# arturxe2/T-DEED

Hardware: AMD Instinct MI355X
Metric: clips/sec (L=100, 224^2, bf16) forward, per-frame logits (higher is better)
Workload: dtype bf16; 1 GPU; rny002_b8: rny002_gsf + ed_sgp_mixer n_layers=2 ks=7, L=100, 224x224, batch 8/GPU, inference forward, random-init weights; clips_per_gpu=8, parallelism=dp1 (clip-sharded, no collective), hip_graph=True, batches_in_flight=3, sub_batches_per_batch=1, dist_backend=none, dist_ranks=1, self_launched=False

## Files before the change

### include/tdeed_hip.h

```cpp
#ifndef TDEED_HIP_H
#define TDEED_HIP_H
#include <stdint.h>
#ifdef __cplusplus
extern "C" {
#endif

enum { TDEED_F32 = 0, TDEED_BF16 = 1 };
enum { TDEED_ACT_NONE = 0, TDEED_ACT_RELU = 1, TDEED_ACT_GELU = 2 };
enum { TDEED_OK = 0, TDEED_ERR_ARG = -1, TDEED_ERR_LAUNCH = -2, TDEED_ERR_RUNTIME = -3 };

const char* tdeed_last_error(void);
int tdeed_abi_version(void);
int tdeed_device_info(int dev, char* name64, int* n_cu, int* is_gfx950);

int tdeed_stem_fwd(const void* frames , int frames_f32,
                   int N, int H, int W, int crop_top, int crop_left,
                   int crop_h, int crop_w, int flip ,
                   const unsigned char* flip_mask ,
                   const float* w ,
                   const float* scale , const float* shift , void* out,
                   int relu , int dtype, void* stream);

int tdeed_stem_mfma_parts(int crop_h, int crop_w);
int tdeed_stem_mfma_fwd(const void* frames, int frames_f32, int N, int H, int W, int crop_top, int crop_left, int crop_h,
                        int crop_w, int flip, const unsigned char* flip_mask, const void* wfrag, void* z, float* colpart,
                        void* stream);
int tdeed_stem_mfma_eval_fwd(const void* frames, int frames_f32, int N, int H, int W, int crop_top, int crop_left, int crop_h,
                             int crop_w, int flip, const unsigned char* flip_mask, const void* wfrag, const float* scale,
                             const float* shift, void* out, void* stream);

int tdeed_s1_front_parts(int crop_h, int crop_w, int C1);
int tdeed_s1_front_fwd(const uint8_t* frames, int N, int H, int W, int crop_top, int crop_left, int crop_h,
                       int crop_w, int flip, const void* stem_wf, const float* stem_sc, const float* stem_sh,
                       int C1, const void* w1f, const float* sc1, const float* sh1, const void* wdf,
                       const float* scd, const float* shd, const void* w2f, const float* sc2,
                       const float* sh2, void* y2, void* shortcut, float* pooled, void* stream);

int tdeed_gemm_fwd(const void* A, long lda, const void* A0, long lda0, int k0,
                   const float* a_scale, int a_scale_rows, int M, int K, int N, const void* W,
                   long ldw, const float* scale, const float* shift, const void* R, long ldr,
                   int act, void* C, long ldc, int gather_stride, int gather_hi, int gather_wi,
                   int gather_ho, int gather_wo, float* colpart, void* C2, long ldc2, int n2, int c2_pre, int dtype,
                   void* stream);

int tdeed_gemm_ws_fits(int K, int N, int dtype);
int tdeed_gemm_ws_fwd(const void* A, long lda, const void* A0, long lda0, int k0,
                      const float* a_scale, int a_scale_rows, int M, int K, int N, const void* Wfrag,
                      const float* scale, const float* shift, const void* R, long ldr, int act,
                      void* C, long ldc, int gather_stride, int gather_hi, int gather_wi,
                      int gather_ho, int gather_wo, void* C2, long ldc2, int n2, int dtype, void* stream);

int tdeed_gemm_ws_sc_fits(int K, int Ks, int N, int dtype);
int tdeed_gemm_ws_sc_fwd(const void* A, long lda, const void* A0, long lda0, int k0, const float* a_scale,
                         int a_scale_rows, int M, int K, int N, const void* Wfrag, const float* scale,
                         const float* shift, const void* As, long ldas, int Ks, const void* Wsfrag,
                         const float* sscale, const float* sshift, int act, void* C, long ldc, int gather_stride,
                         int gather_hi, int gather_wi, int gather_ho, int gather_wo, void* C2, long ldc2, int n2,
                         int dtype, void* stream);

int tdeed_gconv3x3_parts(int Hi, int Wi, int C, int stride, int dtype);
int tdeed_gconv3x3_mfma_fits(int Hi, int Wi, int C, int stride);
int tdeed_gconv3x3_fwd(const void* x, int N, int Hi, int Wi, int C, int gw, int stride,
                       const float* w, const void* wfrag, const float* scale, const float* shift,
                       void* y, float* pooled, float* pooled_sq, const float* in_a, const float* in_b,
                       int relu , int dtype,
                       void* stream);

int tdeed_gemm_splitk_splits(int K);
int tdeed_gemm_splitk_partials(const void* A, long lda, int M, int K, int N, const void* W, long ldw, float* workspace,
                               void* stream);
int tdeed_gemm_splitk_fwd(const void* A, long lda, int M, int K, int N, const void* W, long ldw, const float* scale,
                          const float* shift, const void* R, long ldr, int act, void* C, long ldc,
                          float* workspace, void* stream);

int tdeed_se_gate_mfma_fits(int C, int R);
int tdeed_se_gate_mfma_fwd(const float* pooled, int n_parts, float inv_cnt, int N, int C, int R, const void* w1f,
                           const float* b1, const void* w2f, const float* b2, float* gate, void* stream);

int tdeed_gemm_rs_fits(int M, int K, int N);
int tdeed_gemm_rs_fwd(const void* A, long lda, const void* A0, long lda0, int k0, const float* a_scale, int a_scale_rows,
                      int M, int K, int N, const void* Wfrag, const float* scale, const float* shift, const void* R, long ldr,
                      int act, void* C, long ldc, void* C2, long ldc2, int n2, void* stream);

int tdeed_gemm_rs_grid(int M);
int tdeed_gemm_rs_stats_fwd(const void* A, long lda, const void* A0, long lda0, int k0, int M, int K, int N, const void* Wfrag,
                            void* C, long ldc, float* colpart, void* stream);

int tdeed_c1_gconv_set_debug(void* buf);
int tdeed_c1_gconv_fits(int Hi, int Wi, int Cin, int C, int stride);
int tdeed_c1_gconv_slab_tiles(int Hi, int Wi, int C, int stride);
int tdeed_c1_gconv_fwd(const void* x, const void* G, int Fp, int N, int Hi, int Wi, int Cin, int C, int gw, int stride,
                       const void* w1f, const float* s1, const float* h1, const void* wfrag, const float* scale,
                       const float* shift, void* y, float* pooled, void* stream);
int tdeed_c1_gconv_set_form(int form);
int tdeed_c1_gconv_slab_loop_fits(int Hi, int Wi, int Cin, int C, int stride);
int tdeed_c1_gconv_workgroups(int N, int Hi, int Wi, int Cin, int C, int stride);

int tdeed_c1_gconv_c3in_fits(int Hi, int Wi, int Cp, int C);
int tdeed_c1_gconv_c3in_fwd(const void* y2p, const void* scp, const float* gate, const void* w3f, const float* s3,
                            const float* h3, void* xs2, int N, int Hi, int Wi, int Cp, int C, int gw, const void* w1f,
                            const float* s1, const float* h1, const void* wfrag, const float* scale, const float* shift,
                            void* y, float* pooled, void* stream);
int tdeed_c1_gconv_c3in_set_walk(int walk);
int tdeed_c1_gconv_c3in_walk(int Hi, int Wi, int Cp, int C);
int tdeed_c1_gconv_c3in_workgroups(int N, int Hi, int Wi, int Cp, int C);

int tdeed_bneck_fits(int h, int w, int C, int R);
int tdeed_bneck_set_debug(void* buf);
int tdeed_bneck_fwd(const void* x, const void* G, int Fp, int N, int h, int w, int C, const void* w1f, const float* s1,
                    const float* h1, const void* w2f, const float* s2, const float* h2, const void* se_w1f,
                    const float* se_b1, const void* se_w2f, const float* se_b2, int R, const void* w3f, const float* s3,
                    const float* h3, void* out, void* out2, int n2,
                    int w2_tap_major ,
                    void* stream);
int tdeed_bneck_qtail_fits(int h, int w, int C, int F);
int tdeed_bneck_gs_fwd(const void* x, const void* gx, int ldx, const float* gate, const float* ysum, const float* xsum,
                       const float* cw1, const float* cb1, const float* cw2, const float* cb2, int T, int F, int Fp, int N,
                       int h, int w, int C, const void* w1f, const float* s1, const float* h1, const void* w2f,
                       const float* s2, const float* h2, const void* se_w1f, const float* se_b1, const void* se_w2f,
                       const float* se_b2, int R, const void* w3f, const float* s3, const float* h3, void* out, void* out2,
                       int n2, int w2_tap_major, const void* q_wqf, const float* q_bn, int q_F, float* Q, void* stream);


int tdeed_se_gate_fwd(const float* pooled, int n_parts, float inv_cnt, int N, int C, int R,
                      const float* w1t, const float* b1, const float* w2t, const float* b2,
                      float* gate, void* stream);

int tdeed_se_gate_bf16_fwd(const float* pooled, int n_parts, float inv_cnt, int N, int C, int R,
                           const void* w1p, const float* b1, const void* w2p, const float* b2,
                           float* gate, void* stream);

int tdeed_gsf_gate_fwd(const void* x, int B, int T, int h, int w, int C, int F,
                       const float* bn_scale, const float* bn_shift,
                       const float* wq ,
                       const void* wqf ,
                       const float* b3d ,
                       float* Q , float* gate, float* ysum, float* xsum,
                       int dtype, void* stream);
int tdeed_gsf_gate_sums_fwd(const void* x, int B, int T, int h, int w, int C, int F, const float* b3d, const float* Q,
                            float* gate, float* ysum, float* xsum, void* stream);
int tdeed_gsf_weight_fwd(const float* ysum, const float* xsum, int B, int T, int F, int hw,
                         const float* cw1 , const float* cb1, const float* cw2,
                         const float* cb2, float* fw , void* stream);
int tdeed_gsf_apply_fwd(const void* x, const float* gate, const float* fw , int B,
                        int T, int h, int w, int C, int F, int Fp, void* out, int dtype,
                        void* stream);

int tdeed_gsf_apply_fused_fwd(const void* x, const float* gate, const float* ysum, const float* xsum,
                              const float* cw1, const float* cb1, const float* cw2, const float* cb2, int B,
                              int T, int h, int w, int C, int F, int Fp, void* out, int dtype, void* stream);
int tdeed_gsf_blend_src_fwd(const void* x, const float* gate, const float* ysum, const float* xsum,
                            const float* cw1, const float* cb1, const float* cw2, const float* cb2, int B,
                            int T, int h, int w, int C, int F, int Fp, void* out, int dtype, void* stream);

int tdeed_avgpool_posenc_fwd(const void* x, int B, int T, int hw, int C, const float* temp_enc,
                             void* feat, float* rowstat, int dtype, int dtype_out , void* stream);

int tdeed_layernorm_fwd(const void* x, long ldx, int rows, int C, const float* w, const float* b,
                        float eps, void* y, long ldy, int dtype, void* stream);
int tdeed_sgp_branch_fwd(const void* o, const void* x, int B, int T, int C, int ks, int up,
                         const float* dw, const float* db, void* y, int dtype, void* stream);
int tdeed_mixer_branch_fwd(const void* xn, int B, int T_hi, int T_lo, int C, int ks, int up,
                           const float* dw1, const float* db1, const float* dw2,
                           const float* db2, void* cat, int dtype, void* stream);
int tdeed_sgp_front_set_debug(void* buf);
int tdeed_sgp_front_fwd(const void* x, int B, int T, int C, int ks, int up, const float* ln_w, const float* ln_b, float eps,
                        const float* dw, const float* db, void* y, float* chsum, const float* rowstat, int rowstat_parts,
                        void* y16 ,
                        int dtype, void* stream);
int tdeed_mixer_front_fwd(const void* z, const void* xlo, int B, int T_hi, int T_lo, int C, int ks, int up,
                          const float* ln1_w, const float* ln1_b, const float* ln2_w, const float* ln2_b, float eps,
                          const float* dw1, const float* db1, const float* dw2, const float* db2, void* cat,
                          const float* rowstat_z, int rowstat_z_parts, const float* rowstat_x, int rowstat_x_parts,
                          int dtype, int dtype_cat, void* stream);
int tdeed_groupnorm_fwd(const void* x, int B, int T, int C, int G, const float* w, const float* b,
                        float eps, void* y, int dtype, void* stream);
int tdeed_maxpool_fwd(const void* x, int B, int T_in, int T_out, int C, void* y, int dtype,
                      void* stream);
int tdeed_maxpool_rowstat_fwd(const void* x, int B, int T_in, int T_out, int C, void* y, float* rowstat, float eps, int dtype,
                              void* stream);

int tdeed_heads_fwd(const void* x, int rows, int C, const float* w, const float* b, int n_out,
                    float* out, int dtype, void* stream);

int tdeed_loss_fwd(const float* logits, int rows, int ld, int K1, const int64_t* hard,
                   const float* soft, const float* cls_w, int displ_col, const float* labelD,
                   float* out, void* stream);

int tdeed_loss_bwd(const float* head_out, int rows, int ld, int K1, const int64_t* hard, const float* soft,
                   const float* cls_w, int displ_col, const float* labelD, float grad_scale, float* dhead,
                   void* stream);
int tdeed_loss2(const float* head_out, int B, int T, int ld, int K1a, int K1b, const int64_t* dataset, const int64_t* hard,
                const float* soft, const float* cls_w, int displ_col, const float* labelD, float grad_scale, float* out,
                float* dhead, void* stream);
long tdeed_heads_bwd_workspace(int rows, int C, int n_out);
int tdeed_heads_bwd(const float* dout, const void* x, int rows, int C, const float* w, int n_out, void* dx,
                    float* dw, float* db, void* workspace, int dtype, void* stream);
int tdeed_adamw_step(float* param, const float* grad, float* exp_avg, float* exp_avg_sq, long n, float lr,
                     float beta1, float beta2, float eps, float weight_decay, int step, float grad_scale,
                     void* stream);

long tdeed_grad_guard_ws_bytes(long n);
int tdeed_grad_guard(const float* grad, long n, int skip_nonfinite, void* guard, void* ws, void* stream);
int tdeed_adamw_step_guarded(float* param, const float* grad, float* exp_avg, float* exp_avg_sq, long n, float lr,
                             float beta1, float beta2, float eps, float weight_decay, int step, float grad_scale,
                             const void* guard, int skip_nonfinite, float max_grad_norm, void* stream);

int tdeed_adamw_step_groups(float* param, const float* grad, float* exp_avg, float* exp_avg_sq, long n, float lr,
                            float beta1, float beta2, float eps, float weight_decay, int step, float grad_scale,
                            const void* guard, int skip_nonfinite, float max_grad_norm, const void* runs, int nruns,
                            void* stream);

int tdeed_process_prediction(const float* head_out, int B, int T, int ld, int K1, int displ_col,
                             float* scores, int64_t* cls, void* stream);

int tdeed_cast_f32_to_bf16(const float* src, void* dst, long n, void* stream);
int tdeed_multi_cast_transpose(const void* tab, int n, long tiles, int dtype, void* stream);
int tdeed_gather_cast(const float* src, const int* idx, long n, void* out, int dtype, void* stream);
int tdeed_fill_u8_hash(uint8_t* dst, long n, uint64_t seed, void* stream);

int tdeed_clip_gather_u8(const uint8_t* video, int L, long frame_bytes, const int* starts, int B, int T,
                         uint8_t* clips_out, void* stream);

int tdeed_clip_gather_seg_u8(const uint8_t* video, int L_total, long frame_bytes, const int* starts, const int* clip_base,
                             const int* clip_len_v, int B, int T, uint8_t* clips_out, void* stream);
int tdeed_clip_gather_ring_u8(const uint8_t* ring, int ring_frames, int L_total, long frame_bytes, const int* starts,
                              const int* clip_base, const int* clip_len_v, int B, int T, uint8_t* clips_out, void* stream);
int tdeed_rows_gather(const void* maps, int rows, long row_bytes, int L, int pad_row, const int* starts, int B, int T, void* out,
                      void* stream);
int tdeed_rows_gather_seg(const void* maps, int rows, long row_bytes, int L_total, int pad_row, const int* starts,
                          const int* clip_base, const int* clip_len_v, int B, int T, void* out, void* stream);
int tdeed_stitch_scores_seg(const float* clip_scores, int V, int n, int T, int K1, const int* starts, const int* seg_off,
                            const int* clip_off, int nv, int count_all, int L_total, float* track_sum, int* support,
                            float* mean_out, void* stream);
int tdeed_frame_events_seg(const float* mean, const int* seg_off, int nv, int L_total, int max_len, int K1, float hr_threshold,
                           int* pred, unsigned char* pred_u8, float* pred_score, int* first_frame, int* count, void* stream);
int tdeed_frame_stats_seg(const float* mean, const unsigned char* labels, int L_total, int K1, long* stats, void* stream);
long tdeed_nms_track_seg_workspace(int L_total, int max_len, int K1);
int tdeed_nms_track_seg_threads(int max_len);
int tdeed_nms_track_seg(const float* mean, const int* seg_off, int nv, int L_total, int max_len, int K1, float hr_threshold,
                        double threshold, int soft, const int* windows, int n_windows, const int* first_frame, void* workspace,
                        unsigned char* emitted, double* kept_score, int* st_frame, unsigned char* st_class_u8, double* st_score,
                        int* st_count, int* out_frame, unsigned char* out_class_u8, double* out_score, int* event_off, int* rounds,
                        void* stream);

int tdeed_ap_lds_frames(void);
int tdeed_ap_max_tolerances(void);
int tdeed_ap_max_truth(int n_tol);
int tdeed_ap_match_seg(const float* mean, const unsigned char* emitted, const double* kept_score, const int* seg_off, int nv,
// ... 218 lines not shown
```

### t-deed_amd/_lib.py

```python
import ctypes
import os
from ctypes import c_int, c_long, c_float, c_double, c_void_p, c_char_p, c_uint64, POINTER

import torch

CSRC = os.path.join(os.path.dirname(os.path.abspath(__file__)), "csrc")
LIB_PATH = os.path.join(CSRC, "libtdeed_hip.so")

F32, BF16 = 0, 1
ACT_NONE, ACT_RELU, ACT_GELU = 0, 1, 2


class HipLibraryMissing(RuntimeError):
    pass


class HipCallError(RuntimeError):
    pass


P = c_void_p
_SIGS = {
    "tdeed_abi_version": ([], c_int),
    "tdeed_device_info": ([c_int, c_char_p, POINTER(c_int), POINTER(c_int)], c_int),
    "tdeed_stem_fwd": ([P, c_int, c_int, c_int, c_int, c_int, c_int, c_int, c_int, c_int, P, P, P, P, P, c_int, c_int, P], c_int),
    "tdeed_augment_scratch_floats": ([c_int], c_long),
    "tdeed_augment_clips": ([P, c_int, c_int, c_int, c_int, c_int, c_int, c_int, c_int, c_int, P, P, P, P, P], c_int),
    "tdeed_mix_frames": ([P, P, P, c_int, c_long, P, P], c_int),
    "tdeed_avgpool_posenc_bwd": ([P, c_int, c_int, c_int, c_int, P, P, c_int, P], c_int),
    "tdeed_stem_mfma_parts": ([c_int, c_int], c_int),
    "tdeed_stem_mfma_fwd": ([P, c_int, c_int, c_int, c_int, c_int, c_int, c_int, c_int, c_int, P, P, P, P, P], c_int),
    "tdeed_stem_mfma_eval_fwd": ([P, c_int, c_int, c_int, c_int, c_int, c_int, c_int, c_int, c_int, P, P, P, P, P, P], c_int),
    "tdeed_stem_wgrad": ([P, c_int, c_int, c_int, c_int, c_int, c_int, c_int, c_int, c_int, P, P, P, P, c_int, P], c_int),
    "tdeed_stem_wgrad_bn_fits": ([c_int, c_int, c_int, c_int], c_int),
    "tdeed_stem_wgrad_bn": ([P, c_int, c_int, c_int, c_int, c_int, c_int, c_int, c_int, c_int, P, P, P, P, P, P, P, P, P, P], c_int),
    "tdeed_s1_front_parts": ([c_int, c_int, c_int], c_int),
    "tdeed_s1_front_fwd": ([P, c_int, c_int, c_int, c_int, c_int, c_int, c_int, c_int, P, P, P, c_int, P, P, P, P, P, P,
                            P, P, P, P, P, P, P], c_int),
    "tdeed_gemm_fwd": ([P, c_long, P, c_long, c_int, P, c_int, c_int, c_int, c_int, P, c_long, P, P, P, c_long,
                        c_int, P, c_long, c_int, c_int, c_int, c_int, c_int, P, P, c_long, c_int, c_int, c_int, P], c_int),
    "tdeed_gemm_ws_fits": ([c_int, c_int, c_int], c_int),
    "tdeed_gemm_ws_fwd": ([P, c_long, P, c_long, c_int, P, c_int, c_int, c_int, c_int, P, P, P, P, c_long,
                           c_int, P, c_long, c_int, c_int, c_int, c_int, c_int, P, c_long, c_int, c_int, P], c_int),
    "tdeed_gemm_ws_sc_fits": ([c_int, c_int, c_int, c_int], c_int),
    "tdeed_gemm_ws_sc_fwd": ([P, c_long, P, c_long, c_int, P, c_int, c_int, c_int, c_int, P, P, P, P, c_long, c_int, P, P, P,
                              c_int, P, c_long, c_int, c_int, c_int, c_int, c_int, P, c_long, c_int, c_int, P], c_int),
    "tdeed_gconv3x3_parts": ([c_int, c_int, c_int, c_int, c_int], c_int),
    "tdeed_gconv3x3_mfma_fits": ([c_int, c_int, c_int, c_int], c_int),
    "tdeed_gconv3x3_fwd": ([P, c_int, c_int, c_int, c_int, c_int, c_int, P, P, P, P, P, P, P, P, P, c_int, c_int, P], c_int),
    "tdeed_gemm_splitk_splits": ([c_int], c_int),
    "tdeed_gemm_splitk_fwd": ([P, c_long, c_int, c_int, c_int, P, c_long, P, P, P, c_long, c_int, P, c_long, P, P], c_int),
    "tdeed_se_gate_mfma_fits": ([c_int, c_int], c_int),
    "tdeed_se_gate_mfma_fwd": ([P, c_int, c_float, c_int, c_int, c_int, P, P, P, P, P, P], c_int),
    "tdeed_gemm_rs_fits": ([c_int, c_int, c_int], c_int),
    "tdeed_gemm_rs_grid": ([c_int], c_int),
    "tdeed_gemm_rs_stats_fwd": ([P, c_long, P, c_long, c_int, c_int, c_int, c_int, P, P, c_long, P, P], c_int),
    "tdeed_gemm_rs_fwd": ([P, c_long, P, c_long, c_int, P, c_int, c_int, c_int, c_int, P, P, P, P, c_long, c_int, P, c_long, P,
                           c_long, c_int, P], c_int),
    "tdeed_c1_gconv_set_debug": ([P], c_int),
    "tdeed_c1_gconv_fits": ([c_int, c_int, c_int, c_int, c_int], c_int),
    "tdeed_c1_gconv_slab_tiles": ([c_int, c_int, c_int, c_int], c_int),
    "tdeed_c1_gconv_fwd": ([P, P, c_int, c_int, c_int, c_int, c_int, c_int, c_int, c_int, P, P, P, P, P, P, P, P,
                            P], c_int),
    "tdeed_c1_gconv_set_form": ([c_int], c_int),
    "tdeed_c1_gconv_slab_loop_fits": ([c_int, c_int, c_int, c_int, c_int], c_int),
    "tdeed_c1_gconv_workgroups": ([c_int, c_int, c_int, c_int, c_int, c_int], c_int),
    "tdeed_c1_gconv_c3in_fits": ([c_int, c_int, c_int, c_int], c_int),
    "tdeed_c1_gconv_c3in_fwd": ([P, P, P, P, P, P, P, c_int, c_int, c_int, c_int, c_int, c_int, P, P, P, P, P, P, P, P,
                                 P], c_int),
    "tdeed_c1_gconv_c3in_set_walk": ([c_int], c_int),
    "tdeed_c1_gconv_c3in_walk": ([c_int, c_int, c_int, c_int], c_int),
    "tdeed_c1_gconv_c3in_workgroups": ([c_int, c_int, c_int, c_int, c_int], c_int),
    "tdeed_bneck_fits": ([c_int, c_int, c_int, c_int], c_int),
    "tdeed_bneck_set_debug": ([P], c_int),
    "tdeed_bneck_fwd": ([P, P, c_int, c_int, c_int, c_int, c_int, P, P, P, P, P, P, P, P, P, P, c_int, P, P, P, P, P, c_int,
                         c_int, P], c_int),
    "tdeed_bneck_gs_fwd": ([P, P, c_int, P, P, P, P, P, P, P, c_int, c_int, c_int, c_int, c_int, c_int, c_int, P, P, P, P, P, P, P,
                            P, P, P, c_int, P, P, P, P, P, c_int, c_int, P, P, c_int, P, P], c_int),
    "tdeed_bneck_qtail_fits": ([c_int, c_int, c_int, c_int], c_int),
    "tdeed_gsf_gate_sums_fwd": ([P, c_int, c_int, c_int, c_int, c_int, c_int, P, P, P, P, P, P], c_int),
    "tdeed_bn_slabs": ([c_long], c_int),
    "tdeed_bn_train_stats": ([P, c_long, c_int, P, P, c_float, c_float, P, P, P, P, P, P, P, c_int, P], c_int),
    "tdeed_bn_apply": ([P, c_long, c_int, P, P, P, c_int, P, c_int, P], c_int),
    "tdeed_bn_apply_slice": ([P, c_long, c_int, P, P, P, P, P, c_int, P, P, c_int, c_int, c_int, P], c_int),
    "tdeed_bn_apply2": ([P, c_long, c_int, P, P, P, P, P, c_int, P, c_int, P], c_int),
    "tdeed_bn_train_bwd": ([P, P, P, c_int, c_long, c_int, P, P, P, P, P, P, P, P, P, P, P, c_int, P], c_int),
    "tdeed_fold_rows": ([P, c_long, c_int, c_int, c_int, P, c_long, P], c_int),
    "tdeed_bn_finalize": ([P, P, c_long, c_int, c_long, c_int, P, P, c_float, c_float, P, P, P, P, P, P, P], c_int),
    "tdeed_pool_rows": ([P, P, c_int, c_int, c_int, P, P, c_int, P, c_int, P], c_int),
    "tdeed_se_train_fwd": ([P, c_int, c_int, c_int, P, P, P, P, P, P, P], c_int),
    "tdeed_se_train_bwd": ([P, P, P, c_int, c_int, c_int, P, P, P, P, P, P], c_int),
    "tdeed_scale_rows": ([P, P, P, c_float, c_int, c_int, c_int, P, P, P, c_int, P], c_int),
    "tdeed_gconv3x3_dgrad_stats": ([P, c_int, c_int, c_int, c_int, c_int, P, P, P, P, P, P, P, P, P, P, P], c_int),
    "tdeed_gconv3x3_bwd_stats_bands": ([c_int], c_int),
    "tdeed_gconv3x3_bwd_stats_fits": ([c_int, c_int, c_int, c_int, c_int], c_int),
    "tdeed_gconv3x3_bwd_stats": ([P, P, c_int, c_int, c_int, c_int, c_int, P, P, P, P, P, P, P, P, P, P, P, P, P], c_int),
    "tdeed_bn_bwd_masked_from_parts": ([P, P, c_long, c_int, P, P, P, P, P, P, P, c_long, c_int, P, P, c_int, P], c_int),
    "tdeed_narrow_conv1_bwd_fits": ([c_int, c_int], c_int),
    "tdeed_narrow_conv1_bwd_grid": ([c_long, c_int, c_int], c_int),
    "tdeed_narrow_conv1_bwd": ([P, P, c_long, c_int, c_int, P, P, P, P, P, P, P, P, P, c_long, c_int, c_int, P, c_int, P, P, P, P,
                                P, P, P], c_int),
    "tdeed_bn_sums_from_parts": ([P, P, c_long, c_int, c_int, P, P, P], c_int),
    "tdeed_se_bn_bwd_sums": ([P, P, c_int, c_int, c_int, P, P, P, P, c_int, P], c_int),
    "tdeed_se_bn_bwd_finalize": ([P, P, P, c_int, c_int, c_int, P, P, P], c_int),
    "tdeed_se_bn_bwd_apply": ([P, P, P, P, c_int, c_int, c_int, P, P, P, P, P, P, P, c_int, P], c_int),
    "tdeed_gemm_dgrad": ([P, c_long, c_int, c_int, c_int, P, c_long, P, c_long, c_int, c_int, P, c_long, P, c_long, c_int, P,
                          c_long, P, c_long, P, P, c_long, P, P, c_int, P], c_int),
    "tdeed_gemm_dgrad_rs": ([P, c_long, c_int, c_int, c_int, P, P, c_long, P, c_long, P, c_long, c_int, P, c_long, P, c_long, P, P,
                             P], c_int),
    "tdeed_gsf_add_cols_sink_parts": ([c_long, c_int, c_int], c_int),
    "tdeed_gsf_add_cols_sink": ([P, P, c_long, c_int, c_int, P, P, c_long, P, c_long, P, P, c_long, P, P, c_int, P], c_int),
    "tdeed_bn_bwd_from_parts": ([P, P, c_long, c_int, P, P, P, P, c_int, P, c_int, c_int, c_int, P, P, P, c_int, P], c_int),
    "tdeed_gconv_wgrad_slabs": ([c_long], c_int),
    "tdeed_gconv3x3_bwd": ([P, P, c_int, c_int, c_int, c_int, c_int, c_int, P, P, P, P, P, P, c_int, P], c_int),
    "tdeed_stride2_rows": ([P, P, c_int, c_int, c_int, c_int, c_int, c_int, P], c_int),
    "tdeed_loss2": ([P, c_int, c_int, c_int, c_int, c_int, P, P, P, P, c_int, P, c_float, P, P, P], c_int),
    "tdeed_reduce_strided": ([P, c_int, c_long, c_long, P, P], c_int),
    "tdeed_gsf_slice": ([P, c_long, c_int, c_int, c_int, P, c_int, P], c_int),
    "tdeed_gsf_bwd_scratch_floats": ([c_int, c_int, c_int, c_int], c_long),
    "tdeed_gsf_bwd_part_layout": ([c_int, c_int, c_int, c_int, P], c_int),
    "tdeed_sgp_gemm_ksteps": ([c_int], c_int),
    "tdeed_sgp_gemm_row_tiles": ([c_int, c_int], c_int),
    "tdeed_sgp_gemm_col_tiles": ([c_int, c_int], c_int),
    "tdeed_sgp_gemm_form": ([c_int, c_int, c_int, c_int, c_int], c_int),
    "tdeed_sgp_gemm_gn_gelu": ([P, c_int, c_int, c_int, P, c_int, P, P, c_int, c_float, P, P, c_int, P, c_int, c_int, P], c_int),
    "tdeed_sgp_gemm_residual": ([P, c_int, c_int, c_int, P, P, c_int, P, P, P, P, P, c_int, c_int, c_int, P], c_int),
    "tdeed_sgp_gemm_gelu_chsum": ([P, c_int, c_int, c_int, P, P, c_int, P, P, P, c_int, c_int, P], c_int),
    "tdeed_gsf_bwd": ([P, P, P, P, P, P, c_int, c_int, c_int, c_int, c_int, c_int, c_int, P, P, P, P, P, P, P, P, P, P, P, P,
                       c_int, P], c_int),
    "tdeed_gsf_add_cols": ([P, P, c_long, c_int, c_int, P, c_int, P], c_int),
    "tdeed_gsf_bwd_bn_parts": ([c_int, c_int, c_int, c_int, c_int, c_int], c_int),
    "tdeed_gsf_bwd_stats": ([P, P, P, P, P, P, c_int, c_int, c_int, c_int, c_int, c_int, c_int, P, P, P, P, P, P, P, P, P, P, P, P,
                             P, P, c_int, P], c_int),
    "tdeed_gsf_add_cols_sink_bn": ([P, P, c_long, c_int, c_int, P, P, c_long, P, c_long, P, P, c_long, P, P, P, P, P, P, P, c_int,
                                    P], c_int),
    "tdeed_multi_fold_cw": ([c_int, c_long], c_int),
    "tdeed_multi_fold": ([P, c_int, c_long, P, c_float, c_int, P], c_int),
    "tdeed_multi_copy": ([P, c_int, c_long, P, c_float, c_int, P], c_int),
    "tdeed_reduce_partials": ([P, c_int, c_long, P, c_int, P], c_int),
    "tdeed_eltwise": ([P, P, P, c_long, c_int, c_int, P], c_int),
    "tdeed_transpose": ([P, c_int, c_int, P, c_int, P], c_int),
    "tdeed_wgrad_slices": ([c_int, c_int, c_int], c_int),
    "tdeed_wgrad": ([P, c_long, P, c_long, P, c_long, c_int, c_int, c_int, c_int, P, P, P, P, c_int, c_int, P], c_int),
    "tdeed_layernorm_bwd_blocks": ([c_int], c_int),
    "tdeed_layernorm_bwd": ([P, c_long, P, c_long, c_int, c_int, P, c_float, P, c_int, P, P, P, c_int, P], c_int),
    "tdeed_groupnorm_bwd": ([P, P, c_int, c_int, c_int, c_int, P, c_float, P, c_int, P, P, P, c_int, P], c_int),
    "tdeed_sgp_branch_bwd": ([P, c_long, P, P, P, c_long, c_int, c_int, c_int, c_int, c_int, P, P, P, c_long, P, P, P, P,
                              c_int, P], c_int),
    "tdeed_upsample_bwd": ([P, c_long, c_int, c_int, c_int, c_int, P, c_int, P], c_int),
    "tdeed_maxpool_bwd": ([P, P, c_int, c_int, c_int, c_int, P, c_int, P], c_int),
    "tdeed_se_gate_fwd": ([P, c_int, c_float, c_int, c_int, c_int, P, P, P, P, P, P], c_int),
    "tdeed_se_gate_bf16_fwd": ([P, c_int, c_float, c_int, c_int, c_int, P, P, P, P, P, P], c_int),
    "tdeed_gsf_gate_fwd": ([P, c_int, c_int, c_int, c_int, c_int, c_int, P, P, P, P, P, P, P, P, P, c_int, P], c_int),
    "tdeed_gsf_weight_fwd": ([P, P, c_int, c_int, c_int, c_int, P, P, P, P, P, P], c_int),
    "tdeed_gsf_apply_fwd": ([P, P, P, c_int, c_int, c_int, c_int, c_int, c_int, c_int, P, c_int, P], c_int),
    "tdeed_gsf_apply_fused_fwd": ([P, P, P, P, P, P, P, P, c_int, c_int, c_int, c_int, c_int, c_int, c_int, P, c_int, P], c_int),
    "tdeed_gsf_blend_src_fwd": ([P, P, P, P, P, P, P, P, c_int, c_int, c_int, c_int, c_int, c_int, c_int, P, c_int, P], c_int),
    "tdeed_avgpool_posenc_fwd": ([P, c_int, c_int, c_int, c_int, P, P, P, c_int, c_int, P], c_int),
    "tdeed_layernorm_fwd": ([P, c_long, c_int, c_int, P, P, c_float, P, c_long, c_int, P], c_int),
    "tdeed_sgp_branch_fwd": ([P, P, c_int, c_int, c_int, c_int, c_int, P, P, P, c_int, P], c_int),
    "tdeed_mixer_branch_fwd": ([P, c_int, c_int, c_int, c_int, c_int, c_int, P, P, P, P, P, c_int, P], c_int),
    "tdeed_sgp_front_set_debug": ([P], c_int),
    "tdeed_sgp_front_fwd": ([P, c_int, c_int, c_int, c_int, c_int, P, P, c_float, P, P, P, P, P, c_int, P, c_int, P], c_int),
    "tdeed_mixer_front_fwd": ([P, P, c_int, c_int, c_int, c_int, c_int, c_int, P, P, P, P, c_float, P, P, P, P, P, P, c_int, P,
                               c_int, c_int, c_int, P], c_int),
    "tdeed_gemm_splitk_partials": ([P, c_long, c_int, c_int, c_int, P, c_long, P, P], c_int),
    "tdeed_groupnorm_fwd": ([P, c_int, c_int, c_int, c_int, P, P, c_float, P, c_int, P], c_int),
    "tdeed_maxpool_fwd": ([P, c_int, c_int, c_int, c_int, P, c_int, P], c_int),
    "tdeed_maxpool_rowstat_fwd": ([P, c_int, c_int, c_int, c_int, P, P, c_float, c_int, P], c_int),
    "tdeed_heads_fwd": ([P, c_int, c_int, P, P, c_int, P, c_int, P], c_int),
    "tdeed_loss_fwd": ([P, c_int, c_int, c_int, P, P, P, c_int, P, P, P], c_int),
    "tdeed_loss_bwd": ([P, c_int, c_int, c_int, P, P, P, c_int, P, c_float, P, P], c_int),
    "tdeed_heads_bwd_workspace": ([c_int, c_int, c_int], c_long),
    "tdeed_heads_bwd": ([P, P, c_int, c_int, P, c_int, P, P, P, P, c_int, P], c_int),
    "tdeed_adamw_step": ([P, P, P, P, c_long, c_float, c_float, c_float, c_float, c_float, c_int, c_float, P], c_int),
    "tdeed_grad_guard_ws_bytes": ([c_long], c_long),
    "tdeed_grad_guard": ([P, c_long, c_int, P, P, P], c_int),
    "tdeed_adamw_step_guarded": ([P, P, P, P, c_long, c_float, c_float, c_float, c_float, c_float, c_int, c_float, P, c_int,
                                  c_float, P], c_int),
    "tdeed_adamw_step_groups": ([P, P, P, P, c_long, c_float, c_float, c_float, c_float, c_float, c_int, c_float, P, c_int,
                                 c_float, P, c_int, P], c_int),
    "tdeed_process_prediction": ([P, c_int, c_int, c_int, c_int, c_int, P, P, P], c_int),
    "tdeed_gather_cast": ([P, P, c_long, P, c_int, P], c_int),
    "tdeed_cast_f32_to_bf16": ([P, P, c_long, P], c_int),
    "tdeed_multi_cast_transpose": ([P, c_int, c_long, c_int, P], c_int),
    "tdeed_fill_u8_hash": ([P, c_long, c_uint64, P], c_int),
    "tdeed_clip_gather_u8": ([P, c_int, c_long, P, c_int, c_int, P, P], c_int),
    "tdeed_clip_gather_seg_u8": ([P, c_int, c_long, P, P, P, c_int, c_int, P, P], c_int),
    "tdeed_clip_gather_ring_u8": ([P, c_int, c_int, c_long, P, P, P, c_int, c_int, P, P], c_int),
    "tdeed_rows_gather": ([P, c_int, c_long, c_int, c_int, P, c_int, c_int, P, P], c_int),
    "tdeed_rows_gather_seg": ([P, c_int, c_long, c_int, c_int, P, P, P, c_int, c_int, P, P], c_int),
    "tdeed_stitch_scores_seg": ([P, c_int, c_int, c_int, c_int, P, P, P, c_int, c_int, c_int, P, P, P, P], c_int),
    "tdeed_frame_events_seg": ([P, P, c_int, c_int, c_int, c_int, c_float, P, P, P, P, P, P], c_int),
    "tdeed_nms_track_seg_workspace": ([c_int, c_int, c_int], c_long),
    "tdeed_nms_track_seg_threads": ([c_int], c_int),
    "tdeed_nms_track_seg": ([P, P, c_int, c_int, c_int, c_int, c_float, c_double, c_int, P, c_int, P, P, P, P, P, P, P, P, P, P, P,
                             P, P, P], c_int),
    "tdeed_ap_lds_frames": ([], c_int),
    "tdeed_ap_max_tolerances": ([], c_int),
    "tdeed_ap_max_truth": ([c_int], c_int),
    "tdeed_ap_match_seg": ([P, P, P, P, c_int, c_int, c_int, c_int, c_float, P, c_int, P, c_long, P, P, c_int, c_int, P, c_int, P, P,
                            P, P, P, P], c_int),
    "tdeed_ap_rank": ([P, P, P, c_int, c_long, P, c_int, c_int, c_int, c_int, P, P, P, P, P, P, P, P], c_int),
    "tdeed_ap_state_pack": ([P, P, P, P, P, P, c_long, c_long, P, P, P, c_int, c_int, c_int, c_int, c_long, c_int, P], c_int),
    "tdeed_ap_state_unpack": ([P, P, P, P, P, P, c_long, c_long, P, P, P, c_int, c_int, c_int, c_int, c_long, c_int, P], c_int),
    "tdeed_frame_stats_seg": ([P, P, c_int, c_int, P, P], c_int),
    "tdeed_train_clip_gather_u8": ([P, c_long, c_long, P, P, P, c_int, c_int, c_int, P, P], c_int),
    "tdeed_train_clip_gather_mix_f32": ([P, c_long, c_long, P, P, P, P, P, P, P, c_int, c_int, c_int, P, P], c_int),
    "tdeed_clip_labels": ([P, P, c_int, c_int, c_int, c_int, P, P, P, c_int, c_int, P, P, P], c_int),
    "tdeed_train_clip_gather_u8_ps": ([P, c_long, c_long, P, P, P, c_int, c_int, P, P, P], c_int),
    "tdeed_train_clip_gather_mix_f32_ps": ([P, c_long, c_long, P, P, P, P, P, P, P, c_int, c_int, P, P, P], c_int),
    "tdeed_clip_labels_ps": ([P, P, c_int, c_int, P, c_int, P, P, P, c_int, c_int, P, P, P], c_int),
    "tdeed_jpeg_frame_coeffs": ([c_int, c_int, c_int], c_long),
    "tdeed_jpeg_entropy": ([P, c_long, P, c_int, P, c_int, P, c_int, c_int, c_int, c_int, c_int, c_int, P, P, P], c_int),
    "tdeed_jpeg_pixels": ([P, P, P, c_int, P, c_int, c_int, c_int, c_int, c_int, P], c_int),
    "tdeed_jpeg_pixels_rows": ([P, P, P, c_int, P, c_long, P, c_int, c_int, c_int, c_int, c_int, P], c_int),
    "tdeed_jpeg_pixels_window": ([P, P, P, c_int, P, c_long, P, c_int, c_int, c_int, c_int, c_int, c_int, c_int, c_int, c_int, P],
                                 c_int),
    "tdeed_jpeg_window_blocks": ([c_int, c_int, c_int, c_int, c_int, c_int, c_int, P], c_int),
# ... 118 lines not shown
```

### t-deed_amd/build.py

```python
import os
import subprocess
import sys
from concurrent.futures import ThreadPoolExecutor

CSRC = os.path.join(os.path.dirname(os.path.abspath(__file__)), "csrc")
LIB = os.path.join(CSRC, "libtdeed_hip.so")
SOURCES = ["gemm.hip", "conv.hip", "front.hip", "gsf.hip", "sgp.hip", "sgp_fused.hip", "sgp_gemm.hip", "bneck.hip", "sgp_bwd.hip", "trunk_bwd.hip", "trunk_bwd2.hip", "trunk_bwd3.hip", "gsf_bwd.hip", "train.hip", "misc.hip", "augment.hip", "comm.hip", "video.hip", "spot.hip", "ap.hip", "trainclips.hip", "jpeg.hip"]
FLAGS = ["--offload-arch=gfx950", "-O3", "-fPIC", "-std=c++17", "-ffp-contract=fast", "-Wall",
         "-Wno-unused-function"]
VGPR_MFMA = set(filter(None, os.environ.get("TDEED_VGPR_MFMA", "front.hip").split(",")))
EXTRA = {s: ["-mllvm", "-amdgpu-mfma-vgpr-form"] for s in VGPR_MFMA}


def _hipcc():
    for p in ("/opt/rocm/bin/hipcc", "hipcc"):
        if os.path.exists(p) or p == "hipcc":
            return p


def _stale(obj, deps):
    if not os.path.exists(obj):
        return True
    t = os.path.getmtime(obj)
    return any(os.path.getmtime(d) > t for d in deps)


DEBUG_FLAGS = ["--offload-arch=gfx950", "-O1", "-g", "-DTDEED_DEBUG=1", "-fPIC", "-std=c++17", "-ffp-contract=fast", "-Wall",
               "-Wno-unused-function"]
LIB_DEBUG = os.path.join(CSRC, "libtdeed_hip_dbg.so")


def build(force=False, verbose=True, flavour="release", only=None):
    debug = flavour == "debug"
    flags, lib, osuf = (DEBUG_FLAGS, LIB_DEBUG, ".dbg.o") if debug else (FLAGS, LIB, ".o")
    hdrs = [os.path.join(CSRC, "common.h"), os.path.join(CSRC, "sgp_tile.h"), os.path.join(CSRC, "se_excite.h"), os.path.join(CSRC, "jpeg_core.h"),
            os.path.join(os.path.dirname(os.path.dirname(CSRC)), "include", "tdeed_hip.h")]
    jobs = []
    objs = []
    for s in (only or SOURCES):
        src = os.path.join(CSRC, s)
        obj = os.path.join(CSRC, s.replace(".hip", osuf))
        objs.append(obj)
        if force or _stale(obj, [src] + hdrs):
            jobs.append([_hipcc(), *flags, *([] if debug else EXTRA.get(s, [])), "-c", src, "-o", obj])

    def run(cmd):
        if verbose:
            print(" ".join(cmd), flush=True)
        r = subprocess.run(cmd, capture_output=True, text=True)
        if r.returncode != 0:
            raise RuntimeError(f"hipcc failed:\n{r.stdout}\n{r.stderr}")
        if verbose and r.stderr.strip():
            print(r.stderr, file=sys.stderr)
    with ThreadPoolExecutor(max_workers=4) as ex:
        list(ex.map(run, jobs))
    if only:
        return objs
    if jobs or not os.path.exists(lib):
        run([_hipcc(), "--offload-arch=gfx950", "-shared", "-fPIC", "-o", lib, *objs, "-ldl"])
    return lib


if __name__ == "__main__":
    print(build(force="--force" in sys.argv, flavour="debug" if "--debug" in sys.argv else "release"))
```

### t-deed_amd/csrc/conv.hip

```cpp
#include "common.h"

template <typename T, typename IN>
__global__ __launch_bounds__(256) void stem_kernel(const IN* __restrict__ frames, int H, int W,
                                                   int top, int left, int ch, int cw, int flip_all,
                                                   const unsigned char* __restrict__ flip_mask,
                                                   const float* __restrict__ w,
                                                   const float* __restrict__ scale,
                                                   const float* __restrict__ shift, T* __restrict__ out,
                                                   int Ho, int Wo, int relu) {
  __shared__ float tile[3][33][34];
  const int n = blockIdx.z;
  const int oy0 = blockIdx.y * 16, ox0 = blockIdx.x * 16;
  const int iy0 = oy0 * 2 - 1, ix0 = ox0 * 2 - 1;
  const float mean[3] = {0.485f, 0.456f, 0.406f};
  const float stdv[3] = {0.229f, 0.224f, 0.225f};
  const IN* src = frames + (long)n * 3 * H * W;
  const int flip = flip_mask ? (int)flip_mask[n] : flip_all;
  for (int i = threadIdx.x; i < 3 * 33 * 33; i += 256) {
    int c = i / (33 * 33);
    int r = i - c * 33 * 33;
    int y = r / 33, x = r - y * 33;
    int iy = iy0 + y, ix = ix0 + x;
    float v = 0.f;
    if (iy >= 0 && iy < ch && ix >= 0 && ix < cw) {
// ... 413 lines not shown
        o[r] = (bf16_t)v;
        if (zin) {
          const float zv = (float)z4[r];
          const float g = fmaf(zv, bfa[r], bfb[r]) > 0.f ? (float)o[r] : 0.f;
          psum[r] += g;
          psq[r] = fmaf(g, zv - bmu[r], psq[r]);
        } else {
          psum[r] += (float)o[r];
          psq[r] = fmaf((float)o[r], (float)o[r], psq[r]);
        }
      }
      *reinterpret_cast<bf16x4*>(yout + (long)pc * C + ch0) = o;
    }
  }
#pragma unroll
  for (int r = 0; r < 4; ++r) {
    const float v = td_row16_sum(psum[r]);
    if (pl == 0) red[wv][q * 4 + r] = v;
    if (pooled_sq) {
      const float w = td_row16_sum(psq[r]);
      if (pl == 0) redq[wv][q * 4 + r] = w;
    }
  }
  __syncthreads();
  if (threadIdx.x < units * 16) {
    const int u = threadIdx.x >> 4, cc = threadIdx.x & 15;
    float sres = 0.f, qres = 0.f;
    for (int w2 = u; w2 < 4; w2 += units) {
      sres += red[w2][cc];
      if (pooled_sq) qres += redq[w2][cc];
    }
    const int ch = cs0 + u * 16 + cc;
    if (ch < C) {
      pooled[((long)n * nbands + bnd) * C + ch] = sres;
      if (pooled_sq) pooled_sq[((long)n * nbands + bnd) * C + ch] = qres;
    }
  }
}

template <int STRIDE, bool AFF>
__global__ __launch_bounds__(256) void gconv3x3_mfma_kernel(const bf16_t* __restrict__ x, int Hi, int Wi, int C,
                                                            const float* __restrict__ in_a, const float* __restrict__ in_b,
                                                            const bf16x8* __restrict__ wfrag,
                                                            const float* __restrict__ scale,
                                                            const float* __restrict__ shift,
                                                            bf16_t* __restrict__ y, float* __restrict__ pooled,
                                                            float* __restrict__ pooled_sq,
                                                            int Ho, int Wo, int band, int nbands, int CSP, int PS,
                                                            int rows_in, int relu, const GcStat bst) {
  extern __shared__ __attribute__((aligned(16))) unsigned char tile[];
  __shared__ float red[4][32];
  __shared__ float redq[4][32];
  const long lid = xcd_logical_id(blockIdx.x, gridDim.x);
  const int nslabs_ = (C + CSP - 1) >> (CSP == 64 ? 6 : (CSP == 32 ? 5 : 4));
  int slab, bnd, n, t_;
  td_split(lid, nslabs_, t_, slab);
  td_split(t_, nbands, n, bnd);
  const int cs0 = slab * CSP;
  const GcW gw_ = gconv_load_w(wfrag, slab, CSP);
  const int oy0 = bnd * band;
  const int nrows_out = min(band, Ho - oy0);
  const int WP = Wi + 2;
  const int iy0 = oy0 * STRIDE - 1;
  const int cpp = CSP >> 3;
  const int nrow_used = (nrows_out - 1) * STRIDE + 3;
  const bf16_t* xin = x + (long)n * Hi * Wi * C;
  const int total = nrow_used * WP * cpp;
  const IDiv dcpp(cpp), dwp(WP);
  float ia[8], ib[8];
  if constexpr (AFF) {
    const int jt = threadIdx.x % cpp;
#pragma unroll
    for (int e = 0; e < 8; ++e) {
      const int c = min(cs0 + jt * 8 + e, C - 1);
      ia[e] = in_a[c];
      ib[e] = in_b[c];
    }
  }
  for (int i0 = threadIdx.x; i0 < total; i0 += 256 * 8) {
    u32x4 v[8];
    bool ok[8];
#pragma unroll
    for (int b8 = 0; b8 < 8; ++b8) {
      const int i = min(i0 + b8 * 256, total - 1);
      int j, pix, r, xx;
      dcpp.divmod(i, pix, j);
      dwp.divmod(pix, r, xx);
      const int iy = iy0 + r, ix = xx - 1, c = cs0 + j * 8;
      ok[b8] = iy >= 0 && iy < Hi && ix >= 0 && ix < Wi && c < C;
      v[b8] = *reinterpret_cast<const u32x4*>(ok[b8] ? xin + ((long)iy * Wi + ix) * C + c : xin);
    }
    TD_ISSUE_FENCE();
#pragma unroll
    for (int b8 = 0; b8 < 8; ++b8) {
      const int i = i0 + b8 * 256;
      if (i < total) {
        int j, pix;
        dcpp.divmod(i, pix, j);
        if constexpr (AFF) {
          const bf16x8 t8 = *reinterpret_cast<const bf16x8*>(&v[b8]);
          bf16x8 o8;
#pragma unroll
          for (int e = 0; e < 8; ++e) o8[e] = (bf16_t)fmaxf(fmaf((float)t8[e], ia[e], ib[e]), 0.f);
          v[b8] = *reinterpret_cast<const u32x4*>(&o8);
        }
        *reinterpret_cast<u32x4*>(tile + (long)pix * PS + j * 16) = ok[b8] ? v[b8] : (u32x4){0u, 0u, 0u, 0u};
      }
    }
  }
  __syncthreads();
  gconv_band_mma<STRIDE>(gw_, tile, red, redq, Wi, C, scale, shift, y, pooled, pooled_sq, Ho, Wo, nbands, CSP, PS, relu, n, bnd,
                         slab, oy0, nrows_out, bst);
}

__device__ __forceinline__ void c1g_zero_halo(unsigned char* tile, int nrow_used, int Hi, int Wi, int PS, int iy0) {
  const int tid = threadIdx.x, WP = Wi + 2;
  const int cpp = PS >> 4;
  for (int i = tid; i < nrow_used * 2 * cpp; i += 256) {
    const int j = i % cpp, rc = i / cpp;
    const int rr = rc >> 1, col = (rc & 1) ? (Wi + 1) : 0;
    *reinterpret_cast<u32x4*>(tile + ((long)rr * WP + col) * PS + j * 16) = (u32x4){0u, 0u, 0u, 0u};
  }
  for (int rr = 0; rr < nrow_used; ++rr) {
    const int r = iy0 + rr;
    if (r >= 0 && r < Hi) continue;
    for (int i = tid; i < WP * cpp; i += 256)
      *reinterpret_cast<u32x4*>(tile + (long)rr * WP * PS + (long)i * 16) = (u32x4){0u, 0u, 0u, 0u};
  }
}
__device__ __forceinline__ bool c1g_tile_px(int ntl, int npx, IDiv dwi, int t0, int pl, int& rr, int& cc) {
  const int p = t0 * 16 + pl;
  const bool ok = t0 < ntl && p < npx;
  dwi.divmod(ok ? p : 0, rr, cc);
  return ok;
}
template <int KS1, typename F4>
__device__ __forceinline__ void c1g_conv1_tile(const bf16x8 (&w1r)[4][KS1], const bf16x8 (&xf)[KS1], const F4 (&a1)[4],
                                               const F4 (&b1)[4], int nts, bool pok, unsigned char* dst) {
#pragma unroll
  for (int t = 0; t < 4; ++t) {
    if (t < nts) {
      f32x4 acc = {0.f, 0.f, 0.f, 0.f};
#pragma unroll
      for (int ks = 0; ks < KS1; ++ks) acc = __builtin_amdgcn_mfma_f32_16x16x32_bf16(w1r[t][ks], xf[ks], acc, 0, 0, 0);
      if (pok) {
        bf16x4 o;
#pragma unroll
        for (int e = 0; e < 4; ++e) o[e] = (bf16_t)fmaxf(acc[e] * a1[t][e] + b1[t][e], 0.f);
        *reinterpret_cast<bf16x4*>(dst + t * 32) = o;
      }
    }
  }
}
template <int STRIDE, int KS1>
__global__ __launch_bounds__(256, KS1 == 4 ? 3 : 1) void c1_gconv_mfma_kernel(const bf16_t* __restrict__ x, const bf16_t* __restrict__ G, int Fp,
                                                            int Hi, int Wi, int Cin, int C, const bf16x8* __restrict__ w1f,
                                                            const float* __restrict__ s1, const float* __restrict__ h1,
                                                            const bf16x8* __restrict__ wfrag, const float* __restrict__ scale,
                                                            const float* __restrict__ shift, bf16_t* __restrict__ y,
                                                            float* __restrict__ pooled, int Ho, int Wo, int band, int nbands,
                                                            int CSP, int PS, int rows_in, int relu, long long* dbg) {
  extern __shared__ __attribute__((aligned(16))) unsigned char tile[];
  __shared__ float red[4][32];
  __shared__ float redq[4][32];
  GC_STAMP(0);
  const long lid = xcd_logical_id(blockIdx.x, gridDim.x);
  const int nslabs_ = (C + CSP - 1) >> (CSP == 64 ? 6 : (CSP == 32 ? 5 : 4));
  int slab, bnd, n, t_;
  td_split(lid, nslabs_, t_, slab);
  td_split(t_, nbands, n, bnd);
  const int oy0 = bnd * band;
  const int nrows_out = min(band, Ho - oy0);
  const int WP = Wi + 2;
  const int iy0 = oy0 * STRIDE - 1;
  const int nrow_used = (nrows_out - 1) * STRIDE + 3;
  const int tid = threadIdx.x, lane = tid & 63, wv = __builtin_amdgcn_readfirstlane(tid >> 6);
  const int pl = lane & 15, q = lane >> 4;
  const int nts = CSP >> 4;
  constexpr bool GW_EARLY = KS1 <= 2;
  GcW gw_;
  if constexpr (GW_EARLY) gw_ = gconv_load_w(wfrag, slab, CSP);
  bf16x8 w1r[4][KS1];
  float a1[4][4], b1[4][4];
#pragma unroll
  for (int t = 0; t < 4; ++t) {
    const int tt = slab * nts + min(t, nts - 1);
#pragma unroll
    for (int ks = 0; ks < KS1; ++ks) w1r[t][ks] = w1f[((long)tt * KS1 + ks) * 64 + lane];
    const int c4 = slab * CSP + t * 16 + 4 * q;
    const bool ok = t < nts && c4 < C;
    const int cc4 = min(c4, C - 4);
    const f32x4 av = *reinterpret_cast<const f32x4*>(s1 + cc4), bv = *reinterpret_cast<const f32x4*>(h1 + cc4);
#pragma unroll
    for (int e = 0; e < 4; ++e) {
      a1[t][e] = ok ? av[e] : 0.f;
      b1[t][e] = ok ? bv[e] : 0.f;
    }
  }
  c1g_zero_halo(tile, nrow_used, Hi, Wi, PS, iy0);
  GC_STAMP(1);
  {
    const int r_lo = max(iy0, 0), r_hi = min(iy0 + nrow_used, Hi);
    const int npx = (r_hi - r_lo) * Wi;
    const int ntl = (npx + 15) >> 4;
    const IDiv dwi(Wi);
    const bf16_t* xn = x + (long)n * Hi * Wi * Cin;
    const bf16_t* gn = G ? G + (long)n * Hi * Wi * Fp : nullptr;
    constexpr int NPF = KS1 <= 2 ? 4 : 1;
    if constexpr (KS1 == 4) {
      auto tile_px = [&](int t0, int& rr, int& cc) {
        const int p = min(t0, ntl - 1) * 16 + pl;
        const bool ok = t0 < ntl && p < npx;
        dwi.divmod(p < npx ? p : 0, rr, cc);
        return ok;
      };
      auto tile_load = [&](int rr, int cc, bf16x8 (&xfo)[KS1]) {
        const long pix = (long)(r_lo + rr) * Wi + cc;
#pragma unroll
        for (int ks = 0; ks < KS1; ++ks) {
          const int k = 32 * ks + 8 * q;
          const bf16_t* src = (gn && k < Fp) ? gn + pix * Fp + k : xn + pix * Cin + k;
          xfo[ks] = *reinterpret_cast<const bf16x8*>(src);
        }
      };
      auto tile_mma = [&](bool pok_, int rr, int cc, const bf16x8 (&xfi)[KS1]) {
        unsigned char* dst = tile + ((long)(r_lo + rr - iy0) * WP + cc + 1) * PS + 8 * q;
        c1g_conv1_tile(w1r, xfi, a1, b1, nts, pok_, dst);
      };
      bf16x8 xa[KS1], xb[KS1];
      int ra, ca, rb, cb;
      bool pa = tile_px(wv, ra, ca), pb;
      tile_load(ra, ca, xa);
      for (int tb = wv; tb < ntl; tb += 8) {
        pb = tile_px(tb + 4, rb, cb);
        tile_load(rb, cb, xb);
        tile_mma(pa, ra, ca, xa);
        pa = tile_px(tb + 8, ra, ca);
        tile_load(ra, ca, xa);
        tile_mma(pb, rb, cb, xb);
      }
    } else
    for (int tb = wv; tb < ntl; tb += 4 * NPF) {
      bf16x8 xf[NPF][KS1];
      int rrs[NPF], ccs[NPF];
      bool poks[NPF];
#pragma unroll
      for (int g = 0; g < NPF; ++g) {
        poks[g] = c1g_tile_px(ntl, npx, dwi, tb + 4 * g, pl, rrs[g], ccs[g]);
        const long pix = (long)(r_lo + rrs[g]) * Wi + ccs[g];
#pragma unroll
        for (int ks = 0; ks < KS1; ++ks) {
          const int k = 32 * ks + 8 * q;
          const bool ok = poks[g] && k < Cin;
          const bf16_t* src = (gn && k < Fp) ? gn + pix * Fp + k : xn + pix * Cin + k;
          const u32x4 v = *reinterpret_cast<const u32x4*>(ok ? src : xn);
          const u32x4 z = {0u, 0u, 0u, 0u};
          const u32x4 w = ok ? v : z;
          xf[g][ks] = *reinterpret_cast<const bf16x8*>(&w);
        }
      }
#pragma unroll
      for (int g = 0; g < NPF; ++g) {
        if (tb + 4 * g >= ntl) break;
        unsigned char* dst = tile + ((long)(r_lo + rrs[g] - iy0) * WP + ccs[g] + 1) * PS + 8 * q;
        c1g_conv1_tile(w1r, xf[g], a1, b1, nts, poks[g], dst);
      }
    }
  }
  GC_STAMP(2);
  if constexpr (!GW_EARLY) gw_ = gconv_load_w(wfrag, slab, CSP);
  __syncthreads();
  GC_STAMP(3);
  gconv_band_mma<STRIDE>(gw_, tile, red, redq, Wi, C, scale, shift, y, pooled, nullptr, Ho, Wo, nbands, CSP, PS, relu, n, bnd,
                         slab, oy0, nrows_out, GcStat{nullptr, nullptr, nullptr, nullptr}, dbg);
}

#define C1G_SLAB_TILES(KS1v) ((KS1v) <= 2 ? 5 : 4)
#define C1G_SLAB_MAXC 512
template <int STRIDE, int KS1>
__global__ __launch_bounds__(256, KS1 == 2 ? 3 : 2) void c1_gconv_slab_loop_kernel(const bf16_t* __restrict__ x, const bf16_t* __restrict__ G, int Fp,
                                                            int Hi, int Wi, int Cin, int C, const bf16x8* __restrict__ w1f,
                                                            const float* __restrict__ s1, const float* __restrict__ h1,
                                                            const bf16x8* __restrict__ wfrag, const float* __restrict__ scale,
                                                            const float* __restrict__ shift, bf16_t* __restrict__ y,
                                                            float* __restrict__ pooled, int Ho, int Wo, int band, int nbands,
                                                            int CSP, int PS, int rows_in, int relu, long long* dbg) {
  extern __shared__ __attribute__((aligned(16))) unsigned char tile[];
  __shared__ float red[4][32];
  __shared__ float redq[4][32];
  GC_STAMP(0);
  const long lid = xcd_logical_id(blockIdx.x, gridDim.x);
  const int nslabs_ = (C + CSP - 1) >> 6;
  int bnd, n;
  td_split(lid, nbands, n, bnd);
  const int oy0 = bnd * band;
  const int nrows_out = min(band, Ho - oy0);
  const int WP = Wi + 2;
  const int iy0 = oy0 * STRIDE - 1;
  const int nrow_used = (nrows_out - 1) * STRIDE + 3;
  const int tid = threadIdx.x, lane = tid & 63, wv = __builtin_amdgcn_readfirstlane(tid >> 6);
  const int pl = lane & 15, q = lane >> 4;
  static_assert(STRIDE == 2 && (KS1 == 2 || KS1 == 5), "the slab loop exists for the stride-2 multi-slab blocks");
  constexpr int NT = C1G_SLAB_TILES(KS1);
  constexpr int SCSP = 64;
  const int r_lo = max(iy0, 0), r_hi = min(iy0 + nrow_used, Hi);
  const int npx = (r_hi - r_lo) * Wi;
  const int ntl = (npx + 15) >> 4;
  const IDiv dwi(Wi);
  const bf16_t* xn = x + (long)n * Hi * Wi * Cin;
  const bf16_t* gn = G ? G + (long)n * Hi * Wi * Fp : nullptr;
  __shared__ __attribute__((aligned(16))) float fold[2][C1G_SLAB_MAXC];
  float fa[C1G_SLAB_MAXC / 256], fb[C1G_SLAB_MAXC / 256];
#pragma unroll
  for (int j = 0; j < C1G_SLAB_MAXC / 256; ++j) {
    const int c = min(tid + 256 * j, C - 1);
    fa[j] = s1[c];
    fb[j] = h1[c];
  }
  u32x4 xv[NT][KS1];
  int dsto[NT];
  bool poks[NT];
#pragma unroll
  for (int g = 0; g < NT; ++g) {
    int rr, cc;
    poks[g] = c1g_tile_px(ntl, npx, dwi, wv + 4 * g, pl, rr, cc);
    const long pix = (long)(r_lo + rr) * Wi + cc;
    dsto[g] = ((r_lo + rr - iy0) * WP + cc + 1) * PS + 8 * q;
#pragma unroll
    for (int ks = 0; ks < KS1; ++ks) {
      const int k = 32 * ks + 8 * q;
      const bool ok = poks[g] && k < Cin;
      const bf16_t* src = (gn && k < Fp) ? gn + pix * Fp + k : xn + pix * Cin + k;
      xv[g][ks] = *reinterpret_cast<const u32x4*>(ok ? src : xn);
    }
  }
  bf16x8 w1r[4][KS1];
  auto load_w1 = [&](int sl, int tlo) {
#pragma unroll
    for (int t = tlo; t < tlo + 2; ++t)
#pragma unroll
      for (int ks = 0; ks < KS1; ++ks) w1r[t][ks] = w1f[((long)(sl * 4 + t) * KS1 + ks) * 64 + lane];
  };
  load_w1(0, 0);
  load_w1(0, 2);
  GcW gw_ = gconv_load_w(wfrag, 0, SCSP);
  c1g_zero_halo(tile, nrow_used, Hi, Wi, PS, iy0);
#pragma unroll
  for (int j = 0; j < C1G_SLAB_MAXC / 256; ++j) {
    const int c = tid + 256 * j;
    fold[0][c] = c < C ? fa[j] : 0.f;
    fold[1][c] = c < C ? fb[j] : 0.f;
  }
  __syncthreads();
  GC_STAMP(1);
  bf16x8 xf[NT][KS1];
#pragma unroll
  for (int g = 0; g < NT; ++g)
#pragma unroll
    for (int ks = 0; ks < KS1; ++ks) {
      const u32x4 z = {0u, 0u, 0u, 0u};
      const u32x4 w = (poks[g] && 32 * ks + 8 * q < Cin) ? xv[g][ks] : z;
      xf[g][ks] = *reinterpret_cast<const bf16x8*>(&w);
    }
  auto conv1_pair = [&](int sl, int tlo) {
#pragma unroll
    for (int t = tlo; t < tlo + 2; ++t) {
      const f32x4 av = *reinterpret_cast<const f32x4*>(&fold[0][sl * 64 + t * 16 + 4 * q]);
      const f32x4 bv = *reinterpret_cast<const f32x4*>(&fold[1][sl * 64 + t * 16 + 4 * q]);
#pragma unroll
      for (int g = 0; g < NT; ++g) {
        if (wv + 4 * g >= ntl) break;
        f32x4 acc = {0.f, 0.f, 0.f, 0.f};
#pragma unroll
        for (int ks = 0; ks < KS1; ++ks) acc = __builtin_amdgcn_mfma_f32_16x16x32_bf16(w1r[t][ks], xf[g][ks], acc, 0, 0, 0);
        if (poks[g]) {
          bf16x4 o;
#pragma unroll
          for (int e = 0; e < 4; ++e) o[e] = (bf16_t)fmaxf(acc[e] * av[e] + bv[e], 0.f);
          *reinterpret_cast<bf16x4*>(tile + dsto[g] + t * 32) = o;
        }
      }
    }
  };
  for (int s = 0; s < nslabs_; ++s) {
    const int sn = min(s + 1, nslabs_ - 1);
    conv1_pair(s, 0);
    load_w1(sn, 0);
    conv1_pair(s, 2);
    if (s == 0) GC_STAMP(2);
    __syncthreads();
    if (s == 0) GC_STAMP(3);
    gconv_band_mma<STRIDE>(gw_, tile, red, redq, Wi, C, scale, shift, y, pooled, nullptr, Ho, Wo, nbands, SCSP, PS, relu, n,
                           bnd, s, oy0, nrows_out);
    if (s == 0) GC_STAMP(4);
    load_w1(sn, 2);
    gw_ = gconv_load_w(wfrag, sn, SCSP);
    __syncthreads();
  }
  GC_STAMP(5);
  GC_STAMP(6);
}

struct C3In {
  const bf16_t* y2p; const bf16_t* scp; const float* gate;
  const bf16x8* w3f; const float* s3; const float* h3;
  bf16_t* xs2;
};
#define C3W_NPF 4
template <int CSP>
__global__ __launch_bounds__(256, 3) void c1_gconv_c3in_walk_kernel(int Hi, int Wi, int Cin, int C, const bf16x8* __restrict__ w1f,
                                                            const float* __restrict__ s1, const float* __restrict__ h1,
                                                            const bf16x8* __restrict__ wfrag, const float* __restrict__ scale,
                                                            const float* __restrict__ shift, bf16_t* __restrict__ y,
                                                            float* __restrict__ pooled, int Ho, int Wo, int band, int nbands,
                                                            int walk, long long* dbg, const C3In c3) {
  constexpr int PS = CSP * 2 + 16;
  extern __shared__ __attribute__((aligned(16))) unsigned char tile[];
  __shared__ float red[4][32];
  __shared__ float redq[4][32];
  __shared__ __attribute__((aligned(16))) float f1[2][64];
  __shared__ __attribute__((aligned(16))) float f2[2][64];
  __shared__ __attribute__((aligned(16))) float f3[3][32];
  __shared__ __attribute__((aligned(16))) bf16x8 wl[6][64];
  GC_STAMP(0);
  const long lid = xcd_logical_id(blockIdx.x, gridDim.x);
  const int nruns = (nbands + walk - 1) / walk;
  int n, run;
  td_split(lid, nruns, n, run);
  const int b0 = run * walk, b1 = min(b0 + walk, nbands);
  const int WP = Wi + 2;
  const int tid = threadIdx.x, lane = tid & 63, wv = __builtin_amdgcn_readfirstlane(tid >> 6);
  const int pl = lane & 15, q = lane >> 4;
  const int nts = CSP >> 4;
  const int k8 = 8 * q;
  const bool kok = k8 < Cin;
  const int kc = min(k8, Cin - 8);
  const bf16_t* yn = c3.y2p + (long)n * Hi * Wi * Cin;
  const bf16_t* rn = c3.scp + (long)n * Hi * Wi * Cin;
  bf16_t* xsn = c3.xs2 ? c3.xs2 + (long)n * Ho * Wo * Cin : nullptr;
  const IDiv dwi(Wi);
  struct Bg { int oy0, nrows_out, iy0, nrow_used, r_lo, npx, ntl; };
  auto geom = [&](int b, bool first) {
    Bg g;
    g.oy0 = b * band;
    g.nrows_out = min(band, Ho - g.oy0);
    g.iy0 = g.oy0 * 2 - 1;
    g.nrow_used = (g.nrows_out - 1) * 2 + 3;
    g.r_lo = first ? max(g.iy0, 0) : g.iy0 + 1;
    g.npx = (min(g.iy0 + g.nrow_used, Hi) - g.r_lo) * Wi;
    g.ntl = (g.npx + 15) >> 4;
    return g;
  };
  auto request = [&](const Bg& g, int tb, u32x4 (&yf)[C3W_NPF], u32x4 (&rf)[C3W_NPF]) {
#pragma unroll
    for (int i = 0; i < C3W_NPF; ++i) {
      const int t0 = tb + 4 * i;
      const int p = t0 * 16 + pl;
      int rr, cc;
      dwi.divmod((t0 < g.ntl && p < g.npx) ? p : 0, rr, cc);
      const unsigned o = (unsigned)(((g.r_lo + rr) * Wi + cc) * Cin + kc) * 2u;
      yf[i] = *reinterpret_cast<const u32x4*>(reinterpret_cast<const unsigned char*>(yn) + o);
      rf[i] = *reinterpret_cast<const u32x4*>(reinterpret_cast<const unsigned char*>(rn) + o);
    }
  };
  Bg cur = geom(b0, true);
  u32x4 yf[C3W_NPF], rf[C3W_NPF];
  request(cur, wv, yf, rf);
  auto load_gw = [&]() {
    constexpr int pairs = CSP >= 32 ? CSP >> 5 : 1;
    const unsigned char* wu = reinterpret_cast<const unsigned char*>(wfrag + (CSP >= 32 ? (wv % pairs) * 2 * 5 * 64 : 0));
    unsigned lo = (unsigned)lane * 16u;
    asm volatile("" : "+v"(lo));
    GcW w;
#pragma unroll
    for (int ks = 0; ks < 5; ++ks) {
      w.a[ks] = *reinterpret_cast<const bf16x8*>(wu + ks * 1024 + lo);
      w.b[ks] = CSP >= 32 ? *reinterpret_cast<const bf16x8*>(wu + (5 + ks) * 1024 + lo) : w.a[ks];
    }
    return w;
  };
  GcW gw_;
  {
    const int i0 = tid, i1 = min(tid + 256, 6 * 64 - 1);
    const bf16x8 wv0 = w1f[(long)min(i0 >> 6, nts - 1) * 64 + (i0 & 63)];
    const bf16x8 wv1 = c3.w3f[i1 - 256];
    const int c = tid & 63, cc = min(c, C - 1), c3c = min(tid & 31, Cin - 1);
    const bool ok = c < C, ok3 = (tid & 31) < Cin;
    const float v1a = s1[cc], v1b = h1[cc], v2a = scale[cc], v2b = shift[cc];
    const float v3g = c3.gate[(long)n * Cin + c3c], v3a = c3.s3[c3c], v3b = c3.h3[c3c];
    c1g_zero_halo(tile, cur.nrow_used, Hi, Wi, PS, cur.iy0);
    if (tid < 64) {
      f1[0][c] = ok ? v1a : 0.f;
      f1[1][c] = ok ? v1b : 0.f;
      f2[0][c] = ok ? v2a : 0.f;
      f2[1][c] = ok ? v2b : 0.f;
    } else if (tid < 96) {
      f3[0][tid & 31] = v3g;
      f3[1][tid & 31] = ok3 ? v3a : 1.f;
      f3[2][tid & 31] = ok3 ? v3b : 0.f;
    }
    wl[i0 >> 6][i0 & 63] = wv0;
    if (tid < 128) wl[4 + (tid >> 6)][tid & 63] = wv1;
  }
  __syncthreads();
  GC_STAMP(1);
  auto compute = [&](const Bg& g, int tb, const u32x4 (&yfi)[C3W_NPF], const u32x4 (&rfi)[C3W_NPF]) {
    float g8[8], sc3[8], sh3[8];
#pragma unroll
    for (int e4 = 0; e4 < 8; e4 += 4) {
      const f32x4 gv = *reinterpret_cast<const f32x4*>(&f3[0][kc + e4]);
      const f32x4 sv = *reinterpret_cast<const f32x4*>(&f3[1][k8 + e4]), hv = *reinterpret_cast<const f32x4*>(&f3[2][k8 + e4]);
#pragma unroll
      for (int e = 0; e < 4; ++e) {
        g8[e4 + e] = gv[e];
        sc3[e4 + e] = sv[e];
        sh3[e4 + e] = hv[e];
      }
    }
    f32x4 a1[4], b1[4];
    bf16x8 w1r[4][1];
    const bf16x8 w3a = wl[4][lane], w3b = wl[5][lane];
#pragma unroll
    for (int t = 0; t < 4; ++t) {
      w1r[t][0] = wl[t][lane];
      a1[t] = *reinterpret_cast<const f32x4*>(&f1[0][t * 16 + 4 * q]);
      b1[t] = *reinterpret_cast<const f32x4*>(&f1[1][t * 16 + 4 * q]);
    }
#pragma unroll
    for (int i = 0; i < C3W_NPF; ++i) {
      const int t0 = tb + 4 * i;
      if (t0 >= g.ntl) break;
      int rr, col;
      const bool pok = c1g_tile_px(g.ntl, g.npx, dwi, t0, pl, rr, col);
      const bf16x8 y8 = *reinterpret_cast<const bf16x8*>(&yfi[i]), r8 = *reinterpret_cast<const bf16x8*>(&rfi[i]);
      bf16x8 a8;
#pragma unroll
      for (int e = 0; e < 8; ++e) {
        float f = (float)y8[e];
        f *= g8[e];
        a8[e] = (bf16_t)f;
      }
      const u32x4 zero4 = {0u, 0u, 0u, 0u};
      const u32x4 am = (pok && kok) ? *reinterpret_cast<const u32x4*>(&a8) : zero4;
      const f32x4 z4 = {0.f, 0.f, 0.f, 0.f};
      const f32x4 c0 = __builtin_amdgcn_mfma_f32_16x16x32_bf16(w3a, *reinterpret_cast<const bf16x8*>(&am), z4, 0, 0, 0);
      const f32x4 c1 = __builtin_amdgcn_mfma_f32_16x16x32_bf16(w3b, *reinterpret_cast<const bf16x8*>(&am), z4, 0, 0, 0);
      float v[8];
#pragma unroll
      for (int r = 0; r < 4; ++r) {
        v[r] = c0[r] * sc3[r] + sh3[r];
        v[4 + r] = c1[r] * sc3[4 + r] + sh3[4 + r];
      }
      bf16x8 o8;
#pragma unroll
      for (int e = 0; e < 8; ++e) {
        v[e] += (float)r8[e];
        v[e] = fmaxf(v[e], 0.f);
        o8[e] = (bf16_t)v[e];
      }
      const u32x4 xm = kok ? *reinterpret_cast<const u32x4*>(&o8) : zero4;
      const bf16x8 xf[1] = {*reinterpret_cast<const bf16x8*>(&xm)};
      const int row = g.r_lo + rr;
      if (xsn && pok && kok && !((row | col) & 1) && (row >> 1) >= g.oy0 && (row >> 1) < g.oy0 + g.nrows_out)
        *reinterpret_cast<u32x4*>(xsn + ((long)(row >> 1) * Wo + (col >> 1)) * Cin + k8) = xm;
      unsigned char* dst = tile + ((long)(row - g.iy0) * WP + col + 1) * PS + 8 * q;
      c1g_conv1_tile(w1r, xf, a1, b1, nts, pok, dst);
    }
  };
  const int rowchunks = (WP * PS) >> 4;
  for (int b = b0; b < b1; ++b) {
    TD_ISSUE_FENCE();
    const int rz = Hi - cur.iy0;
    if (b != b0 && rz < cur.nrow_used)
      for (int i = tid; i < rowchunks; i += 256)
        *reinterpret_cast<u32x4*>(tile + rz * (WP * PS) + i * 16) = (u32x4){0u, 0u, 0u, 0u};
    compute(cur, wv, yf, rf);
    for (int tb = wv + 4 * C3W_NPF; tb < cur.ntl; tb += 4 * C3W_NPF) {
      request(cur, tb, yf, rf);
      compute(cur, tb, yf, rf);
    }
    const Bg nxt = geom(min(b + 1, b1 - 1), false);
    gw_ = load_gw();
    request(nxt, wv, yf, rf);
    if (b == b0) GC_STAMP(2);
    if (b == b0 + 1) GC_STAMP(4);
    __syncthreads();
    __builtin_amdgcn_s_waitcnt(0x0F70 | (2 * C3W_NPF));
    gconv_band_mma<2>(gw_, tile, red, redq, Wi, C, f2[0], f2[1], y, pooled, nullptr, Ho, Wo, nbands, CSP, PS, 1, n, b, 0,
                      cur.oy0, cur.nrows_out);
    for (int i = tid; i < rowchunks; i += 256)
      *reinterpret_cast<u32x4*>(tile + i * 16) = *reinterpret_cast<const u32x4*>(tile + (cur.nrow_used - 1) * (WP * PS) + i * 16);
    __syncthreads();
    if (b == b0) GC_STAMP(3);
    if (b == b0 + 1) GC_STAMP(5);
    cur = nxt;
  }
  GC_STAMP(6);
}

static long long* g_c1g_dbg = nullptr;
extern "C" int tdeed_c1_gconv_set_debug(void* buf) { g_c1g_dbg = (long long*)buf; return TDEED_OK; }

extern "C" int tdeed_gconv3x3_mfma_fits(int Hi, int Wi, int C, int stride) {
  return gc_geom(Hi, Wi, C, stride).band > 0 ? 1 : 0;
}

extern "C" int tdeed_gconv3x3_parts(int Hi, int Wi, int C, int stride, int dtype) {
  if (dtype != TDEED_BF16) return 1;
  GcGeom g = gc_geom(Hi, Wi, C, stride);
  return g.band > 0 ? g.nbands : 1;
}

static int gconv3x3_launch(const void* x, int N, int Hi, int Wi, int C, int gw, int stride, const float* w, const void* wfrag,
                           const float* scale, const float* shift, void* y, float* pooled, float* pooled_sq, const float* in_a,
                           const float* in_b, int relu, int dtype, void* stream, const GcStat bst);
extern "C" int tdeed_gconv3x3_fwd(const void* x, int N, int Hi, int Wi, int C, int gw, int stride,
                                  const float* w, const void* wfrag, const float* scale, const float* shift,
                                  void* y, float* pooled, float* pooled_sq, const float* in_a, const float* in_b, int relu,
                                  int dtype, void* stream) {
  return gconv3x3_launch(x, N, Hi, Wi, C, gw, stride, w, wfrag, scale, shift, y, pooled, pooled_sq, in_a, in_b, relu, dtype,
                         stream, GcStat{nullptr, nullptr, nullptr, nullptr});
}
extern "C" int tdeed_gconv3x3_dgrad_stats(const void* dy, int N, int Hi, int Wi, int C, int gw, const void* wfrag_t,
                                          const float* one, const float* zero, void* dx, const void* bz, const float* bfa,
                                          const float* bfb, const float* bmean, float* part_s, float* part_q, void* stream) {
  TD_CHECK(bz && bfa && bfb && bmean && part_s && part_q && wfrag_t && one && zero, "gconv3x3_dgrad_stats: null pointer");
  TD_CHECK(tdeed_gconv3x3_mfma_fits(Hi, Wi, C, 1), "gconv3x3_dgrad_stats: %dx%dx%d is not served by the MFMA kernel", Hi, Wi, C);
  return gconv3x3_launch(dy, N, Hi, Wi, C, gw, 1, nullptr, wfrag_t, one, zero, dx, part_s, part_q, nullptr, nullptr, 0,
                         TDEED_BF16, stream, GcStat{(const bf16_t*)bz, bfa, bfb, bmean});
}
static int gconv3x3_launch(const void* x, int N, int Hi, int Wi, int C, int gw, int stride, const float* w, const void* wfrag,
                           const float* scale, const float* shift, void* y, float* pooled, float* pooled_sq, const float* in_a,
                           const float* in_b, int relu, int dtype, void* stream, const GcStat bst) {
  TD_CHECK(x && scale && shift && y && pooled, "gconv3x3: null pointer");
  TD_CHECK(!in_a == !in_b, "gconv3x3: in_a and in_b come together");
  TD_CHECK(!in_a || (dtype == TDEED_BF16 && wfrag), "gconv3x3: the on-load input affine exists in the bf16 MFMA kernel only");
  TD_CHECK(!pooled_sq || (dtype == TDEED_BF16 && wfrag), "gconv3x3: sums of squares come from the bf16 MFMA kernel only");
  TD_CHECK((gw == 8 || gw == 16) && C % gw == 0, "gconv3x3: group width %d / C %d unsupported", gw, C);
  TD_CHECK(stride == 1 || stride == 2, "gconv3x3: stride %d", stride);
  TD_CHECK(N > 0 && N <= 65535 && Hi > 0 && Wi > 0, "gconv3x3: bad sizes");
  hipStream_t st = (hipStream_t)stream;
  if (dtype == TDEED_F32) {
    TD_CHECK(w, "gconv3x3: fp32 path needs the packed fp32 weights");
    return gw == 8 ? launch_gconv<float, 8>(x, N, Hi, Wi, C, stride, w, scale, shift, y, pooled, relu, st)
                   : launch_gconv<float, 16>(x, N, Hi, Wi, C, stride, w, scale, shift, y, pooled, relu, st);
  }
  if (dtype == TDEED_BF16) {
    GcGeom g = gc_geom(Hi, Wi, C, stride);
    if (!wfrag || g.band <= 0) {
      TD_CHECK(w, "gconv3x3: no weights");
      TD_CHECK(!in_a, "gconv3x3: a row of %d px x %d ch does not fit LDS; no on-load input affine on the VALU path", Wi, C);
      return gw == 8 ? launch_gconv<bf16_t, 8>(x, N, Hi, Wi, C, stride, w, scale, shift, y, pooled, relu, st)
                     : launch_gconv<bf16_t, 16>(x, N, Hi, Wi, C, stride, w, scale, shift, y, pooled, relu, st);
    }
    const int Ho = (Hi - 1) / stride + 1, Wo = (Wi - 1) / stride + 1;
    dim3 grid((unsigned)((long)g.nbands * g.nslabs * N));
    size_t smem = (size_t)g.rows_in * (Wi + 2) * g.PS;
#define TD_GCF(Sv, Av)                                                                                                   \
  hipLaunchKernelGGL((gconv3x3_mfma_kernel<Sv, Av>), grid, dim3(256), smem, st, (const bf16_t*)x, Hi, Wi, C, in_a, in_b,      \
                     (const bf16x8*)wfrag, scale, shift, (bf16_t*)y, pooled, pooled_sq, Ho, Wo, g.band, g.nbands, g.CSP, g.PS, \
                     g.rows_in, relu, bst)
    if (stride == 1) { if (in_a) TD_GCF(1, true); else TD_GCF(1, false); }
    else { if (in_a) TD_GCF(2, true); else TD_GCF(2, false); }
#undef TD_GCF
    TD_LAUNCH_CHECK("gconv3x3_mfma");
    return TDEED_OK;
  }
  tdeed_set_error("gconv3x3: bad dtype %d", dtype);
  return TDEED_ERR_ARG;
}

extern "C" int tdeed_c1_gconv_fits(int Hi, int Wi, int Cin, int C, int stride) {
  const int ks1 = (Cin + 31) / 32;
  if (Cin % 8 != 0 || Cin < 8 || !(ks1 == 1 || ks1 == 2 || ks1 == 4 || ks1 == 5) || C % 8 != 0) return 0;
  return gc_geom(Hi, Wi, C, stride).band > 0 ? 1 : 0;
}
extern "C" int tdeed_c1_gconv_slab_tiles(int Hi, int Wi, int C, int stride) {
  const GcGeom g = gc_geom(Hi, Wi, C, stride);
  return g.nslabs * (g.CSP >> 4);
}
static int g_c1g_form = -1;
extern "C" int tdeed_c1_gconv_set_form(int form) {
  TD_CHECK(form >= -1 && form <= 1, "c1_gconv_set_form: %d (-1 routed, 0 per slab, 1 slab loop)", form);
  g_c1g_form = form;
  return TDEED_OK;
}
extern "C" int tdeed_c1_gconv_slab_loop_fits(int Hi, int Wi, int Cin, int C, int stride) {
  if (stride != 2 || !tdeed_c1_gconv_fits(Hi, Wi, Cin, C, stride)) return 0;
  const int ks1 = (Cin + 31) / 32;
  if (ks1 != 2 && ks1 != 5) return 0;
  const GcGeom g = gc_geom(Hi, Wi, C, stride);
  if (g.nslabs < 2 || g.nslabs * g.CSP > C1G_SLAB_MAXC) return 0;
  const int rows = g.rows_in < Hi ? g.rows_in : Hi;
  const int tiles = (rows * Wi + 15) / 16;
  return (tiles + 3) / 4 <= C1G_SLAB_TILES(ks1) ? 1 : 0;
}
static bool c1g_slab_loop(int Hi, int Wi, int Cin, int C, int stride) {
  return g_c1g_form != 0 && tdeed_c1_gconv_slab_loop_fits(Hi, Wi, Cin, C, stride);
}
extern "C" int tdeed_c1_gconv_workgroups(int N, int Hi, int Wi, int Cin, int C, int stride) {
  if (N <= 0 || !tdeed_c1_gconv_fits(Hi, Wi, Cin, C, stride)) return 0;
  const GcGeom g = gc_geom(Hi, Wi, C, stride);
  return N * g.nbands * (c1g_slab_loop(Hi, Wi, Cin, C, stride) ? 1 : g.nslabs);
}
extern "C" int tdeed_c1_gconv_fwd(const void* x, const void* G, int Fp, int N, int Hi, int Wi, int Cin, int C, int gw,
                                  int stride, const void* w1f, const float* s1, const float* h1, const void* wfrag,
                                  const float* scale, const float* shift, void* y, float* pooled, void* stream) {
  TD_CHECK(x && w1f && s1 && h1 && wfrag && scale && shift && y && pooled, "c1_gconv: null pointer");
  TD_CHECK((gw == 8 || gw == 16) && C % gw == 0, "c1_gconv: group width %d / C %d unsupported", gw, C);
  TD_CHECK(stride == 1 || stride == 2, "c1_gconv: stride %d", stride);
  TD_CHECK(N > 0 && N <= 65535 && tdeed_c1_gconv_fits(Hi, Wi, Cin, C, stride), "c1_gconv: Hi=%d Wi=%d Cin=%d C=%d unsupported",
           Hi, Wi, Cin, C);
  TD_CHECK(!G || (Fp % 8 == 0 && Fp > 0 && Fp <= Cin), "c1_gconv: bad splice width %d", Fp);
  const GcGeom g = gc_geom(Hi, Wi, C, stride);
  const int Ho = (Hi - 1) / stride + 1, Wo = (Wi - 1) / stride + 1;
  const bool slabs = c1g_slab_loop(Hi, Wi, Cin, C, stride);
  dim3 grid((unsigned)((long)g.nbands * (slabs ? 1 : g.nslabs) * N));
  const size_t smem = (size_t)g.rows_in * (Wi + 2) * g.PS;
  hipStream_t st = (hipStream_t)stream;
  const int KS1 = (Cin + 31) / 32;
#define TD_C1G(Sv, Kv)                                                                                                       \
  hipLaunchKernelGGL((c1_gconv_mfma_kernel<Sv, Kv>), grid, dim3(256), smem, st, (const bf16_t*)x, (const bf16_t*)G,           \
                     G ? Fp : 0, Hi, Wi, Cin, C, (const bf16x8*)w1f, s1, h1, (const bf16x8*)wfrag, scale, shift, (bf16_t*)y,  \
                     pooled, Ho, Wo, g.band, g.nbands, g.CSP, g.PS, g.rows_in, 1, g_c1g_dbg)
#define TD_C1G_K(Sv)                                                                                                       \
  do {                                                                                                                     \
    if (KS1 == 1) TD_C1G(Sv, 1); else if (KS1 == 2) TD_C1G(Sv, 2); else if (KS1 == 4) TD_C1G(Sv, 4);                      \
    else TD_C1G(Sv, 5);                                                                                                    \
  } while (0)
  if (slabs) {
#define TD_C1G_SL(Kv)                                                                                                       \
  hipLaunchKernelGGL((c1_gconv_slab_loop_kernel<2, Kv>), grid, dim3(256), smem, st, (const bf16_t*)x, (const bf16_t*)G,        \
                     G ? Fp : 0, Hi, Wi, Cin, C, (const bf16x8*)w1f, s1, h1, (const bf16x8*)wfrag, scale, shift, (bf16_t*)y,  \
                     pooled, Ho, Wo, g.band, g.nbands, g.CSP, g.PS, g.rows_in, 1, g_c1g_dbg)
    if (KS1 == 2) TD_C1G_SL(2); else TD_C1G_SL(5);
#undef TD_C1G_SL
  } else if (stride == 2) TD_C1G_K(2); else TD_C1G_K(1);
#undef TD_C1G_K
#undef TD_C1G
  TD_LAUNCH_CHECK("c1_gconv");
  return TDEED_OK;
}

extern "C" int tdeed_c1_gconv_c3in_fits(int Hi, int Wi, int Cp, int C) {
  if (Cp < 8 || Cp > 32 || Cp % 8 != 0 || C > 64 || !tdeed_c1_gconv_fits(Hi, Wi, Cp, C, 2)) return 0;
  if ((long)Hi * Wi * Cp * 2 >= (1L << 31)) return 0;
  return gc_geom(Hi, Wi, C, 2).nslabs == 1 ? 1 : 0;
}
#define C3IN_WALK_ROUTED 5
static int g_c3in_walk = 0;
extern "C" int tdeed_c1_gconv_c3in_set_walk(int walk) {
  TD_CHECK(walk >= 0 && walk <= 65535, "c1_gconv_c3in_set_walk: %d (0 routed, k >= 1 runs of k bands)", walk);
  g_c3in_walk = walk;
  return TDEED_OK;
}
static int c3in_walk(int forced, int Hi, int Wi, int C) {
  const int nb = gc_geom(Hi, Wi, C, 2).nbands, walk = forced ? forced : C3IN_WALK_ROUTED;
  return walk < nb ? walk : nb;
}
extern "C" int tdeed_c1_gconv_c3in_walk(int Hi, int Wi, int Cp, int C) {
  return tdeed_c1_gconv_c3in_fits(Hi, Wi, Cp, C) ? c3in_walk(0, Hi, Wi, C) : 0;
}
extern "C" int tdeed_c1_gconv_c3in_workgroups(int N, int Hi, int Wi, int Cp, int C) {
  if (N <= 0 || !tdeed_c1_gconv_c3in_fits(Hi, Wi, Cp, C)) return 0;
  const int nb = gc_geom(Hi, Wi, C, 2).nbands, walk = c3in_walk(g_c3in_walk, Hi, Wi, C);
  return N * ((nb + walk - 1) / walk);
}
extern "C" int tdeed_c1_gconv_c3in_fwd(const void* y2p, const void* scp, const float* gate, const void* w3f, const float* s3,
                                       const float* h3, void* xs2, int N, int Hi, int Wi, int Cp, int C, int gw,
                                       const void* w1f, const float* s1, const float* h1, const void* wfrag,
                                       const float* scale, const float* shift, void* y, float* pooled, void* stream) {
  TD_CHECK(y2p && scp && gate && w3f && s3 && h3, "c1_gconv_c3in: null pointer (the producer's operands)");
  TD_CHECK(w1f && s1 && h1 && wfrag && scale && shift && y && pooled, "c1_gconv_c3in: null pointer");
  TD_CHECK((gw == 8 || gw == 16) && C % gw == 0, "c1_gconv_c3in: group width %d / C %d unsupported", gw, C);
  TD_CHECK(N > 0 && N <= 65535 && tdeed_c1_gconv_c3in_fits(Hi, Wi, Cp, C), "c1_gconv_c3in: Hi=%d Wi=%d Cp=%d C=%d unsupported",
           Hi, Wi, Cp, C);
  const GcGeom g = gc_geom(Hi, Wi, C, 2);
  const int Ho = (Hi - 1) / 2 + 1, Wo = (Wi - 1) / 2 + 1;
  const size_t smem = (size_t)g.rows_in * (Wi + 2) * g.PS;
  const C3In c3{(const bf16_t*)y2p, (const bf16_t*)scp, gate, (const bf16x8*)w3f, s3, h3, (bf16_t*)xs2};
  const int walk = c3in_walk(g_c3in_walk, Hi, Wi, C);
  dim3 grid((unsigned)((long)((g.nbands + walk - 1) / walk) * N));
#define TD_C3W(CSPv)                                                                                                        \
  hipLaunchKernelGGL((c1_gconv_c3in_walk_kernel<CSPv>), grid, dim3(256), smem, (hipStream_t)stream, Hi, Wi,  \
                     Cp, C, (const bf16x8*)w1f, s1, h1, (const bf16x8*)wfrag, scale, shift, (bf16_t*)y, pooled, Ho, Wo,       \
                     g.band, g.nbands, walk, g_c1g_dbg, c3)
  if (g.CSP == 64) TD_C3W(64); else if (g.CSP == 32) TD_C3W(32); else TD_C3W(16);
#undef TD_C3W
  TD_LAUNCH_CHECK("c1_gconv_c3in");
  return TDEED_OK;
}

#define SE_FPB 4
__global__ __launch_bounds__(256) void se_gate_kernel(const float* __restrict__ pooled, int n_parts, float inv_cnt,
                                                      int N, int C, int R, const float* __restrict__ w1t,
                                                      const float* __restrict__ b1,
                                                      const float* __restrict__ w2t,
                                                      const float* __restrict__ b2, float* __restrict__ gate) {
  extern __shared__ float sm[];
  float* sp = sm;
  float* shid = sm + SE_FPB * C;
  const int f0 = blockIdx.x * SE_FPB;
  for (int i = threadIdx.x; i < SE_FPB * C; i += 256) {
    const int f = i / C, c = i - f * C;
    float v = 0.f;
    if (f0 + f < N) {
      const float* src = pooled + ((long)(f0 + f) * n_parts) * C + c;
      for (int q = 0; q < n_parts; ++q) v += src[(long)q * C];
    }
    sp[i] = v * inv_cnt;
  }
  __syncthreads();
  {
    const int RP = R <= 32 ? 32 : (R <= 64 ? 64 : (R <= 128 ? 128 : 256));
    const int nsl = 256 / RP;
    const int j = threadIdx.x % RP, sl = threadIdx.x / RP;
    float a[SE_FPB];
#pragma unroll
    for (int f = 0; f < SE_FPB; ++f) a[f] = 0.f;
    if (j < R) {
      const int cper = (C + nsl - 1) / nsl;
      const int c0 = sl * cper, c1 = min(C, c0 + cper);
#pragma unroll 8
      for (int c = c0; c < c1; ++c) {
        const float wv_ = w1t[(long)c * R + j];
#pragma unroll
        for (int f = 0; f < SE_FPB; ++f) a[f] = fmaf(sp[f * C + c], wv_, a[f]);
      }
    }
    float* part = shid + SE_FPB * R;
    if (j < R) {
#pragma unroll
      for (int f = 0; f < SE_FPB; ++f) part[(sl * SE_FPB + f) * R + j] = a[f];
    }
    __syncthreads();
    for (int i = threadIdx.x; i < SE_FPB * R; i += 256) {
      float v = 0.f;
      for (int q = 0; q < nsl; ++q) v += part[q * SE_FPB * R + i];
      shid[i] = fmaxf(v + b1[i % R], 0.f);
    }
  }
  __syncthreads();
  for (int c = threadIdx.x; c < C; c += 256) {
    float a[SE_FPB];
#pragma unroll
    for (int f = 0; f < SE_FPB; ++f) a[f] = 0.f;
#pragma unroll 8
    for (int j = 0; j < R; ++j) {
      const float wv_ = w2t[(long)j * C + c];
#pragma unroll
      for (int f = 0; f < SE_FPB; ++f) a[f] = fmaf(shid[f * R + j], wv_, a[f]);
    }
#pragma unroll
    for (int f = 0; f < SE_FPB; ++f)
      if (f0 + f < N) gate[(long)(f0 + f) * C + c] = sigmoidf_(a[f] + b2[c]);
  }
}

extern "C" int tdeed_se_gate_fwd(const float* pooled, int n_parts, float inv_cnt, int N, int C, int R,
                                 const float* w1t, const float* b1, const float* w2t, const float* b2, float* gate,
                                 void* stream) {
  TD_CHECK(pooled && w1t && b1 && w2t && b2 && gate, "se_gate: null pointer");
  TD_CHECK(N > 0 && C > 0 && R > 0 && R <= 256 && n_parts > 0, "se_gate: bad sizes");
  const int RP = R <= 32 ? 32 : (R <= 64 ? 64 : (R <= 128 ? 128 : 256));
  size_t smem = (size_t)SE_FPB * (C + R + (256 / RP) * R) * sizeof(float);
  hipLaunchKernelGGL(se_gate_kernel, dim3(cdiv(N, SE_FPB)), dim3(256), smem, (hipStream_t)stream, pooled, n_parts,
                     inv_cnt, N, C, R, w1t, b1, w2t, b2, gate);
  TD_LAUNCH_CHECK("se_gate");
  return TDEED_OK;
}

__global__ __launch_bounds__(256) void se_gate_bf16_kernel(const float* __restrict__ pooled, int n_parts, float inv_cnt,
                                                           int N, int C, int R, const bf16_t* __restrict__ w1p,
// ... 447 lines not shown
```

### t-deed_amd/engine.py

```python
import os
from collections import namedtuple
from types import SimpleNamespace

import numpy as np
import torch

from . import ops, _lib
from .streams import new_stream
from .regnet_spec import regnet_spec, sgp_up_size, pyramid_lengths, first_site_block
from .packing import (_np, _f32, _dense, pack_ws_weights, pack_se_bf16, pack_mfma_frags, pack_se_mfma,
                      pack_front_weights, _stem_frags_np, gs_source_order_columns, _gsf_q_frags_np, pack_gsf_q_frags,
                      _gsf_p_frags_np, pack_gsf_p_frags, pack_gconv_frags, _gconv_frags_np, stem_frags_on_device,
                      gsf_q_frags_on_device, gconv_frag_index, gconv_frags_on_device)

BN_EPS = 1e-5


class _Pool:

    def __init__(self, device):
        self.device = device
        self.free = []
        self.all = []

    def take(self, shape, dtype):
        n = int(np.prod(shape)) * torch.empty((), dtype=dtype).element_size()
        n = (n + 255) // 256 * 256
        best = None
        for i, b in enumerate(self.free):
            if b.numel() >= n and (best is None or b.numel() < self.free[best].numel()):
                best = i
        if best is not None and self.free[best].numel() <= 2 * n + (1 << 20):
            raw = self.free.pop(best)
        else:
            raw = torch.empty(n, dtype=torch.uint8, device=self.device)
            self.all.append(raw)
        t = raw[:int(np.prod(shape)) * torch.empty((), dtype=dtype).element_size()].view(dtype).view(*shape)
        t._td_raw = raw
        return t

    def give(self, t):
        self.free.append(t._td_raw)

    def total_bytes(self):
        return sum(b.numel() for b in self.all)


def _dwpack(sd, pre, names, C, device):
    ws = [_np(sd[f"{pre}.{n}.weight"]).reshape(C, -1) for n in names]
    bs = [_np(sd[f"{pre}.{n}.bias"]).reshape(C) for n in names]
    return _f32(np.concatenate(ws, axis=1), device), _f32(np.stack(bs, axis=0), device)


SGP_GEMM = os.environ.get("TDEED_SGP_GEMM", "1") == "1"
SGP_F32_STREAM = os.environ.get("TDEED_SGP_F32_STREAM", "1") == "1"
SGP_BF16_OPERAND_MIN_C = int(os.environ.get("TDEED_SGP_BF16_OPERAND_MIN_C", "384"))


def sgp_stream_dtype(act_dtype, device):
    if SGP_GEMM and SGP_F32_STREAM and act_dtype == torch.bfloat16 and str(device) != "cpu":
        return torch.float32
    return act_dtype


def _pack_mlp(sd, pre, C, o, act_dtype, device):
    o.w_fc1 = _dense(_np(sd[pre + ".mlp.0.weight"]).reshape(4 * C, C), act_dtype, device)
    o.b_fc1 = _f32(_np(sd[pre + ".mlp.0.bias"]), device)
    o.w_fc2 = _dense(_np(sd[pre + ".mlp.2.weight"]).reshape(C, 4 * C), act_dtype, device)
    o.b_fc2 = _f32(_np(sd[pre + ".mlp.2.bias"]), device)
    o.gn_w, o.gn_b = _f32(_np(sd[pre + ".gn.weight"]), device), _f32(_np(sd[pre + ".gn.bias"]), device)
    o.w1g = o.w2g = None
    if act_dtype == torch.bfloat16 and str(device) != "cpu" and C % 16 == 0 and SGP_GEMM:
        o.w1g = pack_mfma_frags(_np(sd[pre + ".mlp.0.weight"]).reshape(4 * C, C), device, ks_mult=12)
        o.w2g = pack_mfma_frags(_np(sd[pre + ".mlp.2.weight"]).reshape(C, 4 * C), device, ks_mult=12)


GS_SRC_ORDER = os.environ.get("TDEED_GS_SRC_ORDER", "1") == "1"
WS_WIDE_MIN_ROWS = 250000
RS_MIN_ROWS = int(os.environ.get("TDEED_RS_MIN_ROWS", "60000"))


class DenseW:

    def __init__(self, W, act_dtype, device, gated=False):
        W = _np(W)
        self.N, self.K = W.shape
        mode = ops.gemm_ws_fits_mode(self.K, self.N, act_dtype) if str(device) != "cpu" else 0
        self.ws = mode == 1
        if self.ws and ((self.K == 64 and self.N == 64) or (gated and self.K >= 64 and self.K % 64 == 0)):
            self.ws = False
        self.w = pack_ws_weights(W, act_dtype, device) if self.ws else _dense(W, act_dtype, device)
        self.wide = (not self.ws) and mode == 2 and WS_WIDE_MIN_ROWS > 0
        self.w_wide = pack_ws_weights(W, act_dtype, device) if self.wide else None
        self.kernel = "gemm_ws" if self.ws else "gemm"

    def _use_wide(self, M):
        return self.wide and M is not None and M >= WS_WIDE_MIN_ROWS

    def _use_rs(self, M, kw):
        return (RS_MIN_ROWS > 0 and self.wide and M is not None and M >= RS_MIN_ROWS
                and (kw.get("a_scale") is None or kw.get("a_scale_rows", 0) >= 64)
                and kw.get("gather") is None and kw.get("lda") is None and kw.get("ldc") is None
                and ops.gemm_rs_fits(M, self.K, self.N))

    def kern(self, M):
        return "gemm_ws" if (self.ws or self._use_wide(M)) else "gemm"

    def run(self, A, scale, shift, act, **kw):
        if self.ws:
            return ops.gemm_ws(A, self.w, self.K, self.N, scale, shift, act, **kw)
        if act in (ops.ACT_NONE, ops.ACT_RELU) and self._use_rs(kw.get("M"), kw):
            return ops.gemm_rs(A, self.w_wide, self.K, self.N, scale, shift, act,
                               **{k: v for k, v in kw.items() if k in ("A0", "k0", "out", "M", "out2", "residual", "a_scale",
                                                                       "a_scale_rows")})
        if self._use_wide(kw.get("M")):
            return ops.gemm_ws(A, self.w_wide, self.K, self.N, scale, shift, act, **kw)
        return ops.gemm(A, self.w, scale, shift, act, **kw)


def pack_sgp_block(sd, pre, C, act_dtype, device):
    o = SimpleNamespace(C=C)
    o.ln_w = _f32(_np(sd[pre + ".ln.weight"]).reshape(C), device)
    o.ln_b = _f32(_np(sd[pre + ".ln.bias"]).reshape(C), device)
    o.dw, o.db = _dwpack(sd, pre, ["psi", "convw", "convkw", "fc", "global_fc"], C, device)
    o.ks = _np(sd[pre + ".psi.weight"]).shape[-1]
    o.up = _np(sd[pre + ".convkw.weight"]).shape[-1]
    _pack_mlp(sd, pre, C, o, act_dtype, device)
    return o


def pack_sgp_mixer(sd, pre, C, act_dtype, device):
    o = SimpleNamespace(C=C)
    for n in ("ln1", "ln2"):
        setattr(o, n + "_w", _f32(_np(sd[f"{pre}.{n}.weight"]).reshape(C), device))
        setattr(o, n + "_b", _f32(_np(sd[f"{pre}.{n}.bias"]).reshape(C), device))
    o.dw1, o.db1 = _dwpack(sd, pre, ["psi1", "convw1", "convkw1", "fc1", "global_fc1"], C, device)
    o.dw2, o.db2 = _dwpack(sd, pre, ["psi2", "convw2", "convkw2", "fc2", "global_fc2"], C, device)
    o.ks = _np(sd[pre + ".psi1.weight"]).shape[-1]
    o.up = _np(sd[pre + ".convkw1.weight"]).shape[-1]
    o.w_cat = _dense(_np(sd[pre + ".concat_fc.weight"]).reshape(C, 6 * C), act_dtype, device)
    o.b_cat = _f32(_np(sd[pre + ".concat_fc.bias"]), device)
    o.wcg = (pack_mfma_frags(_np(sd[pre + ".concat_fc.weight"]).reshape(C, 6 * C), device, ks_mult=12)
             if act_dtype == torch.bfloat16 and str(device) != "cpu" and C % 16 == 0 and SGP_GEMM else None)
    _pack_mlp(sd, pre, C, o, act_dtype, device)
    return o


def _se(pooled, inv_cnt, bw, gate):
    if bw.se_mf is not None:
        return ops.se_gate_mfma(pooled, inv_cnt, bw.se_mf.w1f, bw.se_b1, bw.se_mf.w2f, bw.se_b2, bw.spec.se_rd, out=gate)
    if bw.se_bf is not None:
        return ops.se_gate_bf16(pooled, inv_cnt, bw.se_bf.se_w1p, bw.se_b1, bw.se_bf.se_w2p, bw.se_b2, bw.spec.se_rd, out=gate)
    return ops.se_gate(pooled, inv_cnt, bw.se_w1t, bw.se_b1, bw.se_w2t, bw.se_b2, out=gate)


BNECK_ONE_LAUNCH = os.environ.get("TDEED_BNECK", "1") == "1"
BNECK_BLEND = True
BNECK_QTAIL = True
C1_GCONV = os.environ.get("TDEED_C1_GCONV", "1") == "1"
C1_GCONV_MAX_CIN = 160
SC_IN_CONV3 = True
S1_CONV3_IN_C1G = True


BlockForm = namedtuple("BlockForm",
                       "h w h2 w2 one_launch c1g site Fp slice_in q_given blend_in qtail slice_next sc_in_conv3 conv3_in")


def block_forms(blocks, h, w, act_dtype, taps, last_out_is_slice, pending=None):
    forms = []
    for bi, bw in enumerate(blocks):
        blk = bw.spec
        nbw = blocks[bi + 1] if bi + 1 < len(blocks) else None
        one_launch = bool(BNECK_ONE_LAUNCH and getattr(bw, "fused", None) is not None and bw.se_mf is not None
                          and blk.stride == 1 and not blk.has_downsample and blk.cin == blk.cout
                          and not (last_out_is_slice and nbw is None) and ops.bneck_fits(h, w, blk.cout, blk.se_rd))
        c1g = bool(C1_GCONV and not one_launch and act_dtype == torch.bfloat16 and bw.w2frag is not None
                   and blk.cin <= C1_GCONV_MAX_CIN and ops.c1_gconv_fits(h, w, blk.cin, blk.cout, blk.stride))
        site = blk.gsf_fold > 0
        Fp = (blk.gsf_fold + 7) // 8 * 8 if site else 0
        blend_in = bool(site and one_launch and BNECK_BLEND and bw.gs_src and bw.gs_cw1 is not None and h * w >= 14
                        and 2 * Fp <= blk.cin and ("_features." + blk.name + ".gs_out") not in taps)
        slice_next = (nbw.spec.gsf_fold + 7) // 8 * 8 if (nbw is not None and nbw.spec.gsf_fold) else 0
        qtail = bool(blend_in and BNECK_QTAIL and slice_next and getattr(nbw, "gs_wqf", None) is not None
                     and ops.bneck_qtail_fits(h, w, blk.cout, nbw.spec.gsf_fold))
        sc_in_conv3 = bool(SC_IN_CONV3 and blk.has_downsample and act_dtype == torch.bfloat16 and bw.w3.ws and bw.wd.ws
                           and ops.gemm_ws_sc_fits(blk.cout, blk.cin, blk.cout, act_dtype))
        h2, w2 = (h - 1) // blk.stride + 1, (w - 1) // blk.stride + 1
        slice_in, q_given = bool(site and forms and forms[-1].slice_next == Fp), bool(forms and forms[-1].qtail)
        conv3_in = bool(S1_CONV3_IN_C1G and pending is not None and bi == 0 and c1g and not site and blk.stride == 2
                        and blk.has_downsample and act_dtype == torch.bfloat16 and pending.w3.ws
                        and pending.spec.cout == blk.cin and ("_features." + pending.spec.name) not in taps
                        and ops.c1_gconv_c3in_fits(h, w, blk.cin, blk.cout))
        forms.append(BlockForm(h, w, h2, w2, one_launch, c1g, site, Fp, slice_in, q_given, blend_in, qtail, slice_next, sc_in_conv3,
                               conv3_in))
        h, w = h2, w2
    return forms


class Step:
    __slots__ = ("name", "kernel", "fn", "bytes", "flops")

    def __init__(self, name, kernel, fn, nbytes=0, flops=0):
        self.name, self.kernel, self.fn, self.bytes, self.flops = name, kernel, fn, int(nbytes), int(flops)


def _esz(dt):
    return 2 if dt == torch.bfloat16 else 4


def gemm_cost(M, K, N, es, residual=False, extra=0):
    return (M * K + N * K + M * N * (2 if residual else 1)) * es + extra, 2 * M * K * N


class SgpBuilder:

    def __init__(self, pool, steps, keep, taps, B, act_dtype):
        self.pool, self.steps, self.keep, self.taps, self.B, self.dt = pool, steps, keep, taps, B, act_dtype
        self.splitk_rows = 4096
        self.fused = os.environ.get("TDEED_SGP_FUSED", "1") == "1"
        self.gemm = SGP_GEMM and act_dtype == torch.bfloat16

    def _mlp_gemm(self, name, y, o, Tn, chsum, pool_to=None, y16=None):
        pool, steps, B, C = self.pool, self.steps, self.B, o.C
        R, adt = B * Tn, y.dtype
        es = _esz(adt)
        ya = y if y16 is None else y16
        f1 = ops.sgp_gemm_form(0 if ya.dtype == torch.bfloat16 else 3, B, Tn, 4 * C, C)
        f2 = ops.sgp_gemm_form(1, B, Tn, C, 4 * C)
        nct = ops.sgp_gemm_tiles(Tn, C, f2)[1]
        H = pool.take((B, Tn, 4 * C), torch.bfloat16)
        outb = pool.take((B, Tn, C), adt)
        rsp = torch.empty((nct, R, 2), dtype=torch.float32, device=y.device)
        pooled = rpp = None
        if pool_to is not None and 2 * pool_to == Tn:
            pooled = pool.take((B, pool_to, C), adt)
            rpp = torch.empty((nct, B * pool_to, 2), dtype=torch.float32, device=y.device)
            pooled._td_rowstat = rpp
        self.last_pooled = pooled
        steps.append(Step(name + ".fc1", "sgp_gemm", lambda: ops.sgp_gemm_gn_gelu(ya, chsum, o.gn_w, o.gn_b, o.w1g, o.b_fc1, 4 * C,
                                                                                out=H, form=f1),
                          R * C * _esz(ya.dtype) + 4 * C * C * 2 + R * 4 * C * 2, 2 * R * 4 * C * C))
        steps.append(Step(name + ".fc2", "sgp_gemm", lambda: ops.sgp_gemm_residual(H, o.w2g, o.b_fc2, y, out=outb, rowstat_part=rsp,
                                                                                 pooled=pooled, rowstat_pool_part=rpp, form=f2),
                          R * 4 * C * 2 + 4 * C * C * 2 + 2 * R * C * es + (0 if pooled is None else B * pool_to * C * es),
                          2 * R * 4 * C * C))
        pool.give(H)
        outb._td_rowstat = rsp
        return outb

    def dense(self, name, A, Wt, bias, act, out, R, residual=None):
        N, K = Wt.shape
        es = _esz(self.dt)
        if (self.dt == torch.bfloat16 and R <= self.splitk_rows
                and ops.gemm_splitk_splits(K) >= 4):
            ws = self.pool.take((ops.gemm_splitk_splits(K), R, N), torch.float32)
            self.steps.append(Step(name, "gemm_splitk", lambda: ops.gemm_splitk(A, Wt, None, bias, act, residual=residual,
                                                                                 out=out, M=R, workspace=ws),
                                   *gemm_cost(R, K, N, es, residual is not None)))
            self.pool.give(ws)
        else:
            self.steps.append(Step(name, "gemm", lambda: ops.gemm(A, Wt, None, bias, act, residual=residual, out=out, M=R),
                                   *gemm_cost(R, K, N, es, residual is not None)))

    def _mlp(self, name, y, o, outb, Tn):
        pool, steps, B, C, dt = self.pool, self.steps, self.B, o.C, self.dt
        es, R = _esz(dt), B * Tn
        self.last_pooled = None
        gn = pool.take((B, Tn, C), dt)
        hid = pool.take((B, Tn, 4 * C), dt)
        steps.append(Step(name + ".gn", "groupnorm", lambda: ops.groupnorm(y, 16, o.gn_w, o.gn_b, out=gn), 2 * R * C * es))
        self.dense(name + ".fc1", gn, o.w_fc1, o.b_fc1, ops.ACT_GELU, hid, R)
        self.dense(name + ".fc2", hid, o.w_fc2, o.b_fc2, ops.ACT_NONE, outb, R, residual=y)
        pool.give(gn)
        pool.give(hid)

    def _tap(self, name, outb):
        if name in self.taps:
            self.keep[name] = outb
        return outb

    def block(self, xin, Tn, o, name, pool_to=None):
        pool, steps, B, C, dt = self.pool, self.steps, self.B, o.C, self.dt
        self.last_pooled = None
        R, wl = B * Tn, 2 * o.ks + o.up + 2
        if self.fused:
            gemm = self.gemm and getattr(o, "w1g", None) is not None
            adt = xin.dtype if gemm else dt
            es = _esz(adt)
            y = pool.take((B, Tn, C), adt)
            y16 = pool.take((B, Tn, C), torch.bfloat16) if (gemm and adt == torch.float32 and C > SGP_BF16_OPERAND_MIN_C) else None
            chs = pool.take((B, C, 2), torch.float32) if gemm else None
            outb = None if gemm else pool.take((B, Tn, C), dt)
            rs_in = getattr(xin, "_td_rowstat", None)
            steps.append(Step(name + ".front", "sgp_front", lambda: ops.sgp_front(xin, o.ks, o.up, o.ln_w, o.ln_b, o.dw, o.db,
                                                                                 out=y, chsum=chs, rowstat=rs_in, out16=y16),
                              2 * R * C * es + C * (wl + 7) * 4 + (0 if y16 is None else R * C * 2), 2 * R * C * (wl + 3)))
            if gemm:
                outb = self._mlp_gemm(name, y, o, Tn, chs, pool_to=pool_to, y16=y16)
            else:
                self._mlp(name, y, o, outb, Tn)
            for t_ in (y, y16, chs):
                if t_ is not None:
                    pool.give(t_)
            return self._tap(name, outb)
        ln = pool.take((B, Tn, C), dt)
        y = pool.take((B, Tn, C), dt)
        gn = pool.take((B, Tn, C), dt)
        hid = pool.take((B, Tn, 4 * C), dt)
        outb = pool.take((B, Tn, C), dt)
        es = _esz(dt)
        steps.append(Step(name + ".ln", "layernorm", lambda: ops.layernorm(xin, o.ln_w, o.ln_b, out=ln), 2 * R * C * es))
        steps.append(Step(name + ".branch", "sgp_branch", lambda: ops.sgp_branch(ln, xin, o.ks, o.up, o.dw, o.db, out=y),
                          3 * R * C * es + C * (wl + 5) * 4, 2 * R * C * (wl + 3)))
        steps.append(Step(name + ".gn", "groupnorm", lambda: ops.groupnorm(y, 16, o.gn_w, o.gn_b, out=gn), 2 * R * C * es))
        self.dense(name + ".fc1", gn, o.w_fc1, o.b_fc1, ops.ACT_GELU, hid, R)
        self.dense(name + ".fc2", hid, o.w_fc2, o.b_fc2, ops.ACT_NONE, outb, R, residual=y)
        for t_ in (ln, y, gn, hid):
            pool.give(t_)
        return self._tap(name, outb)

    def mixer(self, xlo, T_lo, z, T_hi, o, name):
        pool, steps, B, C, dt = self.pool, self.steps, self.B, o.C, self.dt
        R, Rl, wl = B * T_hi, B * T_lo, 2 * o.ks + o.up + 2
        if self.fused:
            gemm = self.gemm and getattr(o, "wcg", None) is not None
            adt = z.dtype if gemm else dt
            if gemm and xlo.dtype != adt:
                raise TypeError("SgpBuilder.mixer: z and x_lo must share the residual stream's type")
            es = _esz(adt)
            cat = pool.take((B, T_hi, 6 * C), torch.bfloat16 if gemm else dt)
            if not gemm:
                mo = pool.take((B, T_hi, C), dt)
                outb = pool.take((B, T_hi, C), dt)
            rs_z, rs_x = getattr(z, "_td_rowstat", None), getattr(xlo, "_td_rowstat", None)
            steps.append(Step(name + ".front", "mixer_front",
                              lambda: ops.mixer_front(z, xlo, cat, o.ks, o.up, o.ln1_w, o.ln1_b, o.ln2_w, o.ln2_b, o.dw1,
                                                      o.db1, o.dw2, o.db2, rowstat_z=rs_z, rowstat_x=rs_x),
                              (R + Rl) * C * es + 6 * R * C * _esz(cat.dtype) + 2 * C * (wl + 7) * 4, 4 * R * C * (wl + 3)))
            if not gemm:
                self.dense(name + ".cat", cat, o.w_cat, o.b_cat, ops.ACT_GELU, mo, R)
                self._mlp(name, mo, o, outb, T_hi)
                pool.give(cat)
                pool.give(mo)
                return self._tap(name, outb)
            fc = ops.sgp_gemm_form(2, B, T_hi, C, 6 * C)
            NJ = ops.sgp_gemm_tiles(T_hi, C, fc)[0]
            mo = pool.take((B, T_hi, C), adt)
            mo16 = pool.take((B, T_hi, C), torch.bfloat16) if (adt == torch.float32 and C > SGP_BF16_OPERAND_MIN_C) else None
            chs = pool.take((NJ, B, C, 2), torch.float32)
            steps.append(Step(name + ".cat", "sgp_gemm", lambda: ops.sgp_gemm_gelu_chsum(cat, o.wcg, o.b_cat, C, mo, chs, form=fc,
                                                                                       out16=mo16),
                              R * 6 * C * 2 + 6 * C * C * 2 + R * C * es + (0 if mo16 is None else R * C * 2), 2 * R * 6 * C * C))
            pool.give(cat)
            outb = self._mlp_gemm(name, mo, o, T_hi, chs, y16=mo16)
            pool.give(mo)
            if mo16 is not None:
                pool.give(mo16)
            pool.give(chs)
            return self._tap(name, outb)
        cat = pool.take((B, T_hi, 6 * C), dt)
        xn = pool.take((B, T_lo, C), dt)
        mo = pool.take((B, T_hi, C), dt)
        gn = pool.take((B, T_hi, C), dt)
        hid = pool.take((B, T_hi, 4 * C), dt)
        outb = pool.take((B, T_hi, C), dt)
        zslab = cat.view(-1)[4 * C:]
        es = _esz(dt)
        steps.append(Step(name + ".ln1", "layernorm", lambda: ops.layernorm(z, o.ln1_w, o.ln1_b, out=zslab, ldy=6 * C,
                                                                            rows=R, C=C), 2 * R * C * es))
        steps.append(Step(name + ".ln2", "layernorm", lambda: ops.layernorm(xlo, o.ln2_w, o.ln2_b, out=xn), 2 * Rl * C * es))
        steps.append(Step(name + ".branch", "mixer_branch",
                          lambda: ops.mixer_branch(xn, cat, T_hi, o.ks, o.up, o.dw1, o.db1, o.dw2, o.db2),
                          (6 * R + Rl) * C * es + 2 * C * (wl + 5) * 4, 4 * R * C * (wl + 3)))
        self.dense(name + ".cat", cat, o.w_cat, o.b_cat, ops.ACT_GELU, mo, R)
        steps.append(Step(name + ".gn", "groupnorm", lambda: ops.groupnorm(mo, 16, o.gn_w, o.gn_b, out=gn), 2 * R * C * es))
        self.dense(name + ".fc1", gn, o.w_fc1, o.b_fc1, ops.ACT_GELU, hid, R)
        self.dense(name + ".fc2", hid, o.w_fc2, o.b_fc2, ops.ACT_NONE, outb, R, residual=mo)
        for t_ in (cat, xn, mo, gn, hid):
            pool.give(t_)
        return self._tap(name, outb)

    def pyramid(self, feat, T, n, sgp, mixers, pre="_temp_fine."):
        pool, steps, B, dt = self.pool, self.steps, self.B, self.dt
        C = sgp[0].C
        lens = pyramid_lengths(T, n)
        cur = feat
        stash = []
        for i in range(n):
            cur = self.block(cur, lens[i], sgp[i], f"{pre}_sgp.{i}", pool_to=lens[i + 1])
            stash.append(cur)
            pooled = self.last_pooled
            if pooled is None:
                pooled = pool.take((B, lens[i + 1], C), cur.dtype)
                if self.gemm and self.fused:
                    prs = torch.empty((B * lens[i + 1], 2), dtype=torch.float32, device=cur.device)
                    pooled._td_rowstat = prs
                    steps.append(Step(f"{pre}pool{i}", "maxpool", lambda a=cur, b=pooled, L=lens[i + 1], r=prs:
                                      ops.maxpool_rowstat(a, L, out=b, rowstat=r), B * (lens[i] + lens[i + 1]) * C * _esz(cur.dtype)))
                else:
                    steps.append(Step(f"{pre}pool{i}", "maxpool", lambda a=cur, b=pooled, L=lens[i + 1]: ops.maxpool(a, L, out=b),
                                      B * (lens[i] + lens[i + 1]) * C * _esz(cur.dtype)))
            cur = pooled
        cur = self.block(cur, lens[n], sgp[n], f"{pre}_sgp.{n}")
        for i in range(n):
            lvl = n - 1 - i
            cur = self.mixer(cur, lens[lvl + 1], stash[lvl], lens[lvl], mixers[lvl], f"{pre}_sgpMixer.{lvl}")
            cur = self.block(cur, lens[lvl], sgp[n + 1 + i], f"{pre}_sgp.{n + 1 + i}")
        return cur


TrunkGeometry = namedtuple("TrunkGeometry", "crop ch cw maps")


def centre_window(H, W, ch, cw):
    return (int(round((H - ch) / 2.0)), int(round((W - cw) / 2.0)), ch, cw)


def trunk_geometry(blocks, crop, H, W):
    ch, cw, rect = H, W, None
    if crop is not None and crop > 0 and (crop != H or crop != W):
        ch = cw = crop
        rect = centre_window(H, W, ch, cw)
    h, w = (ch + 1) // 2, (cw + 1) // 2
    maps = [(h, w, blocks[0].cin)]
    for blk in blocks:
        h, w = (h - 1) // blk.stride + 1, (w - 1) // blk.stride + 1
        maps.append((h, w, blk.cout))
    return TrunkGeometry(rect, ch, cw, maps)


class SubPlan:
    __slots__ = ("frames", "steps", "keep", "head_out", "pool_bytes", "B", "T", "h", "w", "sgp_out")

    def __init__(self, frames, steps, keep, head_out, pool_bytes, B, T, h=None, w=None):
        self.frames, self.steps, self.keep, self.head_out, self.pool_bytes = frames, steps, keep, head_out, pool_bytes
        self.B, self.T, self.h, self.w, self.sgp_out = B, T, h, w, keep.get("sgp_out")


class Plan:
    __slots__ = ("subs", "streams", "tail", "steps", "head_out", "keep", "graph", "pool_bytes", "B", "T", "trunk_map", "out", "h",
                 "w", "trunk_in", "flip_buf")

    def __init__(self, subs, head_out, B, T, streams=None, tail=None, trunk_map=None, out=None, h=None, w=None, trunk_in=None,
                 flip_buf=None):
        self.subs, self.streams, self.tail = subs, streams or [None] * len(subs), tail
        chains = subs + ([] if tail is None else [tail])
        self.steps = [st for c in chains for st in c.steps]
        self.pool_bytes = sum(c.pool_bytes for c in chains)
        self.head_out, self.keep, self.graph, self.B, self.T = head_out, (subs[0].keep if subs else {}), None, B, T
        self.trunk_map, self.out, self.h, self.w, self.trunk_in, self.flip_buf = trunk_map, out, h, w, trunk_in, flip_buf


_Front = namedtuple("_Front", "bw y2 sc pooled gate")


class TrunkBuilder:

    def __init__(self, pw, act_dtype, device, taps, B, fuse_front=True):
        self.pw, self.act_dtype, self.device, self.taps, self.B, self.fuse_front = pw, act_dtype, device, taps, B, fuse_front
        self.pool, self.steps, self.keep = _Pool(device), [], {}
        self.N = B * pw.clip_len
        self.frames = self.head_out = None
        self.front = None
        self.stem_wf = None

    def _se_conv3(self, bw, h2, w2, y2, pooled, gate, sc, out, out2=None, sc_from=None):
        blk, es, N, M2 = bw.spec, _esz(self.act_dtype), self.N, self.N * h2 * w2
        se = Step(blk.name + ".se", "se_gate", lambda: _se(pooled, 1.0 / (h2 * w2), bw, gate),
                  2 * N * blk.cout * 4 + 2 * blk.cout * blk.se_rd * 4, 4 * N * blk.cout * blk.se_rd)
        if sc_from is not None:
            x, gather = sc_from
            return (se, Step(blk.name + ".conv3", "gemm_ws", lambda: ops.gemm_ws_sc(
                y2, bw.w3.w, blk.cout, blk.cout, bw.s3, bw.h3, x, bw.wd.w, blk.cin, bw.sd, bw.hd, ops.ACT_RELU, a_scale=gate,
                a_scale_rows=h2 * w2, gather=gather, out=out, M=M2, out2=out2),
                (M2 * (2 * blk.cout + blk.cin) + blk.cout * (blk.cout + blk.cin)) * es,
                2 * M2 * blk.cout * (blk.cout + blk.cin)))
        return (se, Step(blk.name + ".conv3", bw.w3.kern(M2), lambda: bw.w3.run(
            y2, bw.s3, bw.h3, ops.ACT_RELU, residual=sc, a_scale=gate, a_scale_rows=h2 * w2, out=out, M=M2, out2=out2),
            *gemm_cost(M2, blk.cout, blk.cout, es, True)))

    def _block_done(self, blk, dead, x, x_kept, out):
        for t_ in dead:
            self.pool.give(t_)
        if not x_kept and hasattr(x, "_td_raw"):
            self.pool.give(x)
        tapname = "_features." + blk.name
        if tapname in self.taps:
            self.keep[tapname] = out
        return tapname in self.taps

    def _gs_site(self, bw, f, xg, q):
        pool, B, blk, T = self.pool, self.B, bw.spec, self.pw.clip_len
        N, F, Fp = self.N, blk.gsf_fold, f.Fp
        M = N * f.h * f.w
        gb = dict(gate=pool.take((N, f.h, f.w, 2), torch.float32),
                  q=(q if f.q_given else pool.take((N, f.h, f.w, 6), torch.float32)),
                  ysum=pool.take((N, F), torch.float32),
                  xsum=pool.take((N, F), torch.float32))
        if not f.blend_in:
            gb["out"] = pool.take((M, Fp), self.act_dtype)
            if bw.gs_cw1 is not None:
                gb["fw"] = pool.take((B, F, T), torch.float32)
        self.steps.append(Step(blk.name + ".gate_shift", "gate_shift", lambda: ops.gate_shift(
            xg, B, T, F, Fp, bw.gs_scale, bw.gs_shift, bw.gs_wq, bw.gs_b3d, bw.gs_cw1, bw.gs_cb1,
            bw.gs_cw2, bw.gs_cb2, bufs=gb, wqf=bw.gs_wqf, src_order=bw.gs_src, gates_only=f.blend_in, q_given=f.q_given),
            M * ((1 if f.blend_in else 2) * F + (0 if f.blend_in else Fp)) * _esz(self.act_dtype) + M * 16, 2 * M * F * 27))
        tap = "_features." + blk.name + ".gs_out"
        if tap in self.taps:
            if bw.gs_src:
                raise ValueError("the gs_out tap is in module channel order: build the engine with TDEED_GS_SRC_ORDER=0")
            self.keep[tap] = gb["out"]
        return gb

    def _one_launch(self, bw, f, x, xg, gb, nbw):
        pool, blk, T, dt = self.pool, bw.spec, self.pw.clip_len, self.act_dtype
        N, es = self.N, _esz(dt)
        M = N * f.h * f.w
        out = pool.take((N, f.h, f.w, blk.cout), dt)
        xs_next = pool.take((N, f.h, f.w, f.slice_next), dt) if f.slice_next else None
        o2 = xs_next.view(-1, f.slice_next) if f.slice_next else None
        q_next = None
        if f.blend_in:
            qt = None
            if f.qtail:
                q_next = pool.take((N, f.h, f.w, 6), torch.float32)
                qt = (nbw.gs_wpf, nbw.gs_bnq, nbw.spec.gsf_fold, q_next)
            run = lambda: ops.bneck_gs(
                x, xg, gb["gate"], gb["ysum"], gb["xsum"], bw.gs_cw1, bw.gs_cb1, bw.gs_cw2, bw.gs_cb2, T, blk.gsf_fold, f.Fp,
                bw.fused.w1f, bw.s1, bw.h1, bw.fused.w2f, bw.s2, bw.h2, bw.se_mf.w1f, bw.se_b1, bw.se_mf.w2f, bw.se_b2,
                blk.se_rd, bw.fused.w3f, bw.s3, bw.h3, out=out, out2=o2, w2_tap_major=bw.fused.w2_tap_major, qtail=qt)
        else:
            G = gb.get("out")
            run = lambda: ops.bneck(
                x, bw.fused.w1f, bw.s1, bw.h1, bw.fused.w2f, bw.s2, bw.h2, bw.se_mf.w1f, bw.se_b1, bw.se_mf.w2f, bw.se_b2,
                blk.se_rd, bw.fused.w3f, bw.s3, bw.h3, G=G, out=out, out2=o2, w2_tap_major=bw.fused.w2_tap_major)
        self.steps.append(Step(blk.name + ".bneck", "bneck", run,
                               (2 * M * blk.cout + (M * f.Fp if f.blend_in else 0)) * es + (8 * M if f.blend_in else 0)
                               + (24 * M if f.qtail else 0)
                               + (2 * blk.cout * blk.cout + blk.cout * blk.gw * 9) * es,
                               2 * M * blk.cout * (2 * blk.cout + blk.gw * 9)))
        return out, xs_next, q_next

    def _chain(self, bw, f, x, y1, G, out, dead_site):
        pool, steps, blk, dt = self.pool, self.steps, bw.spec, self.act_dtype
        N, es, s = self.N, _esz(dt), blk.stride
        h, w, h2, w2 = f.h, f.w, f.h2, f.w2
        M, M2 = N * h * w, N * h2 * w2
        if y1 is not None:
            splice = dict(A0=G, k0=f.Fp) if f.site else {}
            steps.append(Step(blk.name + ".conv1", bw.w1.kern(M), lambda: bw.w1.run(
                x, bw.s1, bw.h1, ops.ACT_RELU, out=y1, M=M, **splice), *gemm_cost(M, blk.cin, blk.cout, es)))
        y2 = pool.take((N, h2, w2, blk.cout), dt)
        parts = ops.gconv3x3_parts(h, w, blk.cout, s, dt) if bw.w2frag is not None else 1
        pooled = pool.take((N, parts, blk.cout), torch.float32)
        gate = pool.take((N, blk.cout), torch.float32)
        if f.c1g and bw.c1g_w1f is None:
            bw.c1g_w1f = pack_mfma_frags(bw.w1_raw, self.device, rows=16 * ops.c1_gconv_slab_tiles(h, w, blk.cout, s))
        xs2 = None
        if f.conv3_in:
            front, self.front = self.front, None
            pbw = front.bw
            xs2 = pool.take((N, h2, w2, blk.cin), dt)
            steps.append(Step(blk.name + ".conv1_conv2", "c1_gconv", lambda: ops.c1_gconv_c3in(
                front.y2, front.sc, front.gate, pbw.w3.w, pbw.s3, pbw.h3, bw.c1g_w1f, bw.s1, bw.h1, bw.w2frag, bw.s2, bw.h2,
                blk.gw, blk.cout, xs2=xs2, out=y2, pooled=pooled),
                (2 * M * blk.cin + M2 * blk.cout + M2 * blk.cin) * es + (blk.cin * blk.cin + blk.cout * (blk.cin + blk.gw * 9)) * es,
                2 * M * blk.cin * blk.cin + 2 * M * blk.cin * blk.cout + 2 * M2 * blk.cout * blk.gw * 9))
            for t_ in front[1:]:
                pool.give(t_)
            x = xs2
        elif f.c1g:
            steps.append(Step(blk.name + ".conv1_conv2", "c1_gconv", lambda: ops.c1_gconv(
                x, bw.c1g_w1f, bw.s1, bw.h1, bw.w2frag, bw.s2, bw.h2, blk.gw, s, blk.cout, G=G, out=y2, pooled=pooled),
                (M * blk.cin + M2 * blk.cout) * es + blk.cout * (blk.cin + blk.gw * 9) * es,
                2 * M * blk.cin * blk.cout + 2 * M2 * blk.cout * blk.gw * 9))
        else:
            steps.append(Step(blk.name + ".conv2", "gconv3x3", lambda: ops.gconv3x3(
                y1, bw.w2, bw.s2, bw.h2, blk.gw, s, wfrag=bw.w2frag, out=y2, pooled=pooled),
                (M + M2) * blk.cout * es + blk.cout * blk.gw * 9 * 4, 2 * M2 * blk.cout * blk.gw * 9))
        sc, shortcut, sc_from = x, [], None
        gather = (s, h, w, h2, w2) if (s > 1 and xs2 is None) else None
        if f.sc_in_conv3:
            sc, sc_from = None, (x, gather)
        elif blk.has_downsample:
            sc = pool.take((N, h2, w2, blk.cout), dt)
            shortcut = [Step(blk.name + ".downsample", bw.wd.kern(M2), lambda: bw.wd.run(
                x, bw.sd, bw.hd, ops.ACT_NONE, gather=gather, out=sc, M=M2), *gemm_cost(M2, blk.cin, blk.cout, es))]
        if out is None:
            out = pool.take((N, h2, w2, blk.cout), dt)
        xs_next = pool.take((N, h2, w2, f.slice_next), dt) if f.slice_next else None
        se, conv3 = self._se_conv3(bw, h2, w2, y2, pooled, gate, sc, out, out2=xs_next, sc_from=sc_from)
        steps += [se, *shortcut, conv3]
        return out, xs_next, (([y1] if y1 is not None else []) + [y2, pooled, gate] + dead_site + ([sc] if shortcut else [])
                              + ([xs2] if xs2 is not None else []))

    def _blocks(self, x, h, w, blocks, x_kept, out_last=None):
        pool, N, dt, fr = self.pool, self.N, self.act_dtype, self.front
        xs = q = None
        forms = block_forms(blocks, h, w, dt, self.taps, out_last is not None, *(() if fr is None else (fr.bw,)))
        if fr is not None:
            if forms and forms[0].conv3_in:
                self.steps.append(self._se_conv3(fr.bw, h, w, fr.y2, fr.pooled, fr.gate, fr.sc, None)[0])
            else:
                x = pool.take((N, h, w, fr.bw.spec.cout), dt)
                self.steps += self._se_conv3(fr.bw, h, w, fr.y2, fr.pooled, fr.gate, fr.sc, x)
                x_kept = self._block_done(fr.bw.spec, fr[1:], None, True, x)
                self.front = None
        for bi, f in enumerate(forms):
            bw, last = blocks[bi], bi + 1 == len(blocks)
            y1 = None if (f.one_launch or f.c1g) else pool.take((N, f.h, f.w, bw.spec.cout), dt)
            xg = xs if f.slice_in else x
            gb = self._gs_site(bw, f, xg, q) if f.site else {}
            dead = list(gb.values()) + ([xs] if f.slice_in else [])
            if f.one_launch:
                out, xs, q = self._one_launch(bw, f, x, xg, gb, None if last else blocks[bi + 1])
            else:
                out, xs, dead = self._chain(bw, f, x, y1, gb.get("out"), out_last if last else None, dead)
                q = None
            x_kept = self._block_done(bw.spec, dead, x, x_kept, out)
            x, h, w = out, f.h2, f.w2
        return x, h, w, x_kept

    def trunk(self, H, W, crop, flip, frames_dtype=torch.uint8, stop=None, out_last=None, rect=None, frames=None):
        Wt, pool, steps, N, dt, es = self.pw.W, self.pool, self.steps, self.N, self.act_dtype, _esz(self.act_dtype)
        if rect is not None:
            geo = trunk_geometry(self.pw.spec.blocks, None, rect[2], rect[3])
            win = lambda: tuple(rect)
        else:
            geo = trunk_geometry(self.pw.spec.blocks, crop, H, W)
            win = lambda: geo.crop
        ch, cw, (Ho, Wo, c0) = geo.ch, geo.cw, geo.maps[0]
        if frames is None:
            frames = torch.empty((N, 3, H, W), dtype=frames_dtype, device=self.device)
        self.frames = frames
        blocks = list(Wt.blocks[:stop])
        if (Wt.front is not None and "_features.stem" not in self.taps and self.fuse_front and frames_dtype == torch.uint8
                and blocks and not isinstance(flip, torch.Tensor) and ops.s1_front_parts(ch, cw, Wt.blocks[0].spec.cout) > 0):
            bw = blocks.pop(0)
            blk, (h, w, _) = bw.spec, geo.maps[1]
            parts, M2 = ops.s1_front_parts(ch, cw, blk.cout), N * h * w
            y2 = pool.take((N, h, w, blk.cout), dt)
            sc = pool.take((N, h, w, blk.cout), dt)
            pooled = pool.take((N, parts, blk.cout), torch.float32)
            gate = pool.take((N, blk.cout), torch.float32)
            steps.append(Step("s1_front", "s1_front", lambda: ops.s1_front(
                frames, Wt.front, win(), flip, y2=y2, shortcut=sc, pooled=pooled),
                              N * 3 * ch * cw + 2 * M2 * blk.cout * es,
                              2 * N * Ho * Wo * 32 * (27 + 2 * blk.cout) // 1 + 2 * M2 * blk.cout * blk.gw * 9))
            self.front = _Front(bw, y2, sc, pooled, gate)
            x, x_kept = None, True
        else:
            x, h, w = pool.take((N, Ho, Wo, c0), dt), Ho, Wo
            if self.stem_wf is not None and dt == torch.bfloat16 and ops.stem_mfma_parts(ch, cw) > 0:
                wf = self.stem_wf
                steps.append(Step("stem", "stem_mfma", lambda: ops.stem_mfma_eval(frames, wf, Wt.stem_scale, Wt.stem_shift, win(),
                                                                                flip, out=x),
                                  N * 3 * ch * cw * (4 if frames_dtype == torch.float32 else 1) + N * Ho * Wo * 32 * es,
                                  2 * N * Ho * Wo * 32 * 27))
            else:
                steps.append(Step("stem", "stem", lambda: ops.stem(frames, Wt.stem_w, Wt.stem_scale, Wt.stem_shift, dt, win(),
                                                                   flip, out=x),
                                  N * 3 * ch * cw + N * Ho * Wo * 32 * es, 2 * N * Ho * Wo * 32 * 27))
            x_kept = "_features.stem" in self.taps
            if x_kept:
                self.keep["_features.stem"] = x
        if out_last is not None and not blocks:
            raise ValueError("join_at must leave at least one un-fused bottleneck in the sub-batch plans")
        return self._blocks(x, h, w, blocks, x_kept, out_last=out_last)

    def avgpool(self, x, h, w, x_kept, feat=None, frs=None):
        pw, Wt, B, C = self.pw, self.pw.W, self.B, self.pw.spec.feat_dim
        if feat is None:
            feat = self.pool.take((B, pw.clip_len, C), sgp_stream_dtype(self.act_dtype, self.device))
        if frs is None:
            frs = torch.empty((self.N, 2), dtype=torch.float32, device=self.device)
        feat._td_rowstat = frs
        self.steps.append(Step("avgpool", "avgpool_posenc", lambda: ops.avgpool_posenc(x, B, pw.clip_len, Wt.temp_enc, out=feat,
                                                                                      rowstat=frs),
                               (self.N * h * w + self.N) * C * _esz(self.act_dtype)))
        self.keep["feat"] = feat
        if not x_kept:
            self.pool.give(x)
        return feat

    def sgp_heads(self, feat, head_out=None):
        pw, Wt, N, C = self.pw, self.pw.W, self.N, self.pw.spec.feat_dim
        if head_out is None:
            head_out = torch.empty((N, pw.n_out), dtype=torch.float32, device=self.device)
        self.head_out = head_out
        cur = SgpBuilder(self.pool, self.steps, self.keep, self.taps, self.B, self.act_dtype).pyramid(
            feat, pw.clip_len, pw.n_layers, Wt.sgp, Wt.mixer)
        self.steps.append(Step("heads", "heads", lambda: ops.heads(cur, Wt.head_w, Wt.head_b, out=head_out),
                               N * C * _esz(self.act_dtype) + N * pw.n_out * 4, 2 * N * C * pw.n_out))
        self.keep["sgp_out"] = cur

    def sub_plan(self, h=None, w=None):
        return SubPlan(self.frames, self.steps, self.keep, self.head_out, self.pool.total_bytes(), self.B, self.pw.clip_len, h, w)


class PackedWeights:

    def __init__(self, cfg, state, act_dtype, device):
        g = (lambda k: cfg[k]) if isinstance(cfg, dict) else (lambda k: getattr(cfg, k))
        self.arch = g("feature_arch")
        self.spec = regnet_spec(self.arch)
        self.mode = "gsm" if self.arch.endswith("_gsm") else ("gsf" if self.arch.endswith("_gsf") else None)
        self.clip_len = g("clip_len")
        self.n_layers = g("n_layers")
        self.ks = g("sgp_ks")
        self.up = sgp_up_size(self.ks, g("sgp_r"))
        self.radi = g("radi_displacement")
        self.act_dtype = act_dtype
        self.device = device
        sd = {k: _np(v) for k, v in state.items()}
        self.double_head = "_pred_fine._fc1._fc_out.weight" in sd
        f32 = lambda a: _f32(a, device)
        bf16_gpu = act_dtype == torch.bfloat16 and str(device) != "cpu"

        def bn_fold(pre):
            w, b = sd[pre + ".weight"].astype(np.float64), sd[pre + ".bias"].astype(np.float64)
            m, v = sd[pre + ".running_mean"].astype(np.float64), sd[pre + ".running_var"].astype(np.float64)
            s = w / np.sqrt(v + BN_EPS)
            return f32(s), f32(b - m * s)

        W = SimpleNamespace()
        p = "_features."
        W.stem_w = f32(sd[p + "stem.conv.weight"].reshape(32, 27))
        W.stem_scale, W.stem_shift = bn_fold(p + "stem.bn")
        W.blocks = []
        for blk in self.spec.blocks:
            bp = p + blk.name
            bw = SimpleNamespace(spec=blk)
            c1 = bp + (".conv1.net" if blk.gsf_fold else ".conv1")
            w1_mat = _np(sd[c1 + ".conv.weight"]).reshape(blk.cout, blk.cin)
            bw.gs_src = bool(blk.gsf_fold and GS_SRC_ORDER and self.mode == "gsf" and bf16_gpu)
            if bw.gs_src:
                w1_mat = gs_source_order_columns(w1_mat, blk.gsf_fold)
            bw.w1 = DenseW(w1_mat, act_dtype, device)
            bw.w1_raw = w1_mat
            bw.wd_raw = _np(sd[bp + ".downsample.conv.weight"]).reshape(blk.cout, blk.cin) if blk.has_downsample else None
            bw.c1g_w1f = None
            bw.s1, bw.h1 = bn_fold(c1 + ".bn")
            w2 = sd[bp + ".conv2.conv.weight"]
            G, gw = blk.groups, blk.gw
            w2 = w2.reshape(G, gw, gw, 3, 3).transpose(0, 3, 4, 2, 1)
            bw.w2 = f32(w2.reshape(G, 9, gw, gw))
            bw.s2, bw.h2 = bn_fold(bp + ".conv2.bn")
            bw.w2frag = pack_gconv_frags(sd[bp + ".conv2.conv.weight"], gw, device) if act_dtype == torch.bfloat16 else None
            bw.se_w1t = f32(sd[bp + ".se.fc1.weight"].reshape(blk.se_rd, blk.cout).T)
            bw.se_b1 = f32(sd[bp + ".se.fc1.bias"])
            bw.se_w2t = f32(sd[bp + ".se.fc2.weight"].reshape(blk.cout, blk.se_rd).T)
            bw.se_b2 = f32(sd[bp + ".se.fc2.bias"])
            bw.se_bf = (SimpleNamespace(**pack_se_bf16(sd[bp + ".se.fc1.weight"], sd[bp + ".se.fc2.weight"], device))
                        if bf16_gpu else None)
            bw.se_mf = (SimpleNamespace(**pack_se_mfma(sd[bp + ".se.fc1.weight"], sd[bp + ".se.fc2.weight"], device))
                        if (bf16_gpu and ops.se_gate_mfma_fits(blk.cout, blk.se_rd)) else None)
            bw.w3 = DenseW(sd[bp + ".conv3.conv.weight"].reshape(blk.cout, blk.cout), act_dtype, device, gated=True)
            bw.fused = (SimpleNamespace(w1f=pack_mfma_frags(w1_mat, device),
                                        w2f=pack_gconv_frags(sd[bp + ".conv2.conv.weight"], gw, device, tap_major=(gw == 8)),
                                        w2_tap_major=(gw == 8),
                                        w3f=pack_mfma_frags(sd[bp + ".conv3.conv.weight"].reshape(blk.cout, blk.cout), device))
                        if (bw.se_mf is not None and blk.stride == 1 and not blk.has_downsample and blk.cin == blk.cout
                            and blk.cout <= 384) else None)
            bw.s3, bw.h3 = bn_fold(bp + ".conv3.bn")
            if blk.has_downsample:
                bw.wd = DenseW(sd[bp + ".downsample.conv.weight"].reshape(blk.cout, blk.cin), act_dtype, device)
                bw.sd, bw.hd = bn_fold(bp + ".downsample.bn")
            if blk.gsf_fold:
                gp = bp + ".conv1.gs"
                F = blk.gsf_fold
# ... 338 lines not shown
```

### t-deed_amd/ops.py

```python
import ctypes

import numpy as np
import torch

from . import _lib
from ._lib import call, ptr, stream_ptr, dtype_code, ACT_NONE, ACT_RELU, ACT_GELU


def _chk(t, name, dtype=None):
    if t is None:
        return
    if not t.is_cuda:
        raise RuntimeError(f"{name} must be a GPU tensor (tdeed_amd has no CPU path)")
    if not t.is_contiguous():
        raise RuntimeError(f"{name} must be contiguous")
    if dtype is not None and t.dtype != dtype:
        raise TypeError(f"{name}: expected {dtype}, got {t.dtype}")


def _flip_args(flip, N):
    if isinstance(flip, torch.Tensor):
        m = flip.to(torch.uint8).contiguous()
        if m.numel() != N or not m.is_cuda:
            raise ValueError(f"flip mask must hold one flag per frame on the GPU ({m.numel()} vs {N})")
        return 0, m
    return int(bool(flip)), None


def stem(frames_u8, w, scale, shift, act_dtype, crop=None, flip=False, out=None, relu=True):
    _chk(frames_u8, "frames", torch.float32 if frames_u8.dtype == torch.float32 else torch.uint8)
    N, _, H, W = frames_u8.shape
    top, left, ch, cw = crop if crop is not None else (0, 0, H, W)
    Ho, Wo = (ch + 1) // 2, (cw + 1) // 2
    if out is None:
        out = torch.empty((N, Ho, Wo, 32), dtype=act_dtype, device=frames_u8.device)
    fl, fmask = _flip_args(flip, N)
    call("tdeed_stem_fwd", ptr(frames_u8), int(frames_u8.dtype == torch.float32), N, H, W, top, left, ch, cw, fl,
         ptr(fmask), ptr(w), ptr(scale), ptr(shift),
         ptr(out), int(relu), dtype_code(act_dtype), stream_ptr())
    return out


def stem_mfma_parts(ch, cw):
    return _lib.load().tdeed_stem_mfma_parts(ch, cw)


def stem_mfma(frames, wfrag, crop=None, flip=False):
    _chk(frames, "frames", torch.float32 if frames.dtype == torch.float32 else torch.uint8)
    _chk(wfrag, "wfrag", torch.float32)
    N, _, H, W = frames.shape
    top, left, ch, cw = crop if crop is not None else (0, 0, H, W)
    parts = stem_mfma_parts(ch, cw)
    if parts <= 0:
        raise RuntimeError(f"stem_mfma: a {cw}-pixel row band does not fit LDS")
    z = torch.empty((N, (ch + 1) // 2, (cw + 1) // 2, 32), dtype=torch.bfloat16, device=frames.device)
    colpart = torch.empty((N * parts, 2, 32), dtype=torch.float32, device=frames.device)
    fl, fmask = _flip_args(flip, N)
    call("tdeed_stem_mfma_fwd", ptr(frames), int(frames.dtype == torch.float32), N, H, W, top, left, ch, cw, fl, ptr(fmask),
         ptr(wfrag), ptr(z), ptr(colpart), stream_ptr())
    return z, colpart


def stem_mfma_eval(frames, wfrag, scale, shift, crop=None, flip=False, out=None):
    _chk(frames, "frames", torch.float32 if frames.dtype == torch.float32 else torch.uint8)
    _chk(wfrag, "wfrag", torch.float32)
    _chk(scale, "scale", torch.float32)
    _chk(shift, "shift", torch.float32)
    if scale.numel() != 32 or shift.numel() != 32:
        raise ValueError("stem_mfma_eval: scale and shift hold one value per stem channel (32)")
    N, _, H, W = frames.shape
    top, left, ch, cw = crop if crop is not None else (0, 0, H, W)
    if stem_mfma_parts(ch, cw) <= 0:
        raise RuntimeError(f"stem_mfma_eval: a {cw}-pixel row band does not fit LDS")
    shape = (N, (ch + 1) // 2, (cw + 1) // 2, 32)
    if out is None:
        out = torch.empty(shape, dtype=torch.bfloat16, device=frames.device)
    _chk(out, "out", torch.bfloat16)
    if tuple(out.shape) != shape:
        raise ValueError(f"stem_mfma_eval: out {tuple(out.shape)}, expected {shape}")
    fl, fmask = _flip_args(flip, N)
    call("tdeed_stem_mfma_eval_fwd", ptr(frames), int(frames.dtype == torch.float32), N, H, W, top, left, ch, cw, fl, ptr(fmask),
         ptr(wfrag), ptr(scale), ptr(shift), ptr(out), stream_ptr())
    return out


def s1_front_parts(ch, cw, C1):
    return _lib.load().tdeed_s1_front_parts(ch, cw, C1)


def s1_front(frames_u8, fw, crop=None, flip=False, y2=None, shortcut=None, pooled=None):
    _chk(frames_u8, "frames", torch.uint8)
    N, _, H, W = frames_u8.shape
    top, left, ch, cw = crop if crop is not None else (0, 0, H, W)
    Hs, Ws = (ch + 1) // 2, (cw + 1) // 2
    Ho, Wo = (Hs + 1) // 2, (Ws + 1) // 2
    C1 = fw.C1
    dev = frames_u8.device
    if y2 is None:
        y2 = torch.empty((N, Ho, Wo, C1), dtype=torch.bfloat16, device=dev)
    if shortcut is None:
        shortcut = torch.empty((N, Ho, Wo, C1), dtype=torch.bfloat16, device=dev)
    if pooled is None:
        pooled = torch.empty((N, s1_front_parts(ch, cw, C1), C1), dtype=torch.float32, device=dev)
    call("tdeed_s1_front_fwd", ptr(frames_u8), N, H, W, top, left, ch, cw, int(flip), ptr(fw.stem_wf), ptr(fw.stem_sc),
         ptr(fw.stem_sh), C1, ptr(fw.w1f), ptr(fw.sc1), ptr(fw.sh1), ptr(fw.wdf), ptr(fw.scd), ptr(fw.shd),
         ptr(fw.w2f), ptr(fw.sc2), ptr(fw.sh2), ptr(y2), ptr(shortcut), ptr(pooled), stream_ptr())
    return y2, shortcut, pooled


def gemm_colpart_rows(M):
    return (M + 127) // 128


def _out2(out2, A):
    if out2 is None:
        return None, 0, 0
    _chk(out2, "out2", A.dtype)
    return ptr(out2), out2.shape[-1], out2.shape[-1]


def gemm(A, W, scale=None, shift=None, act=ACT_NONE, residual=None, a_scale=None, a_scale_rows=0,
         A0=None, k0=0, gather=None, out=None, M=None, lda=None, ldc=None, colpart=None, out2=None, out2_pre=False):
    _chk(A, "A"); _chk(W, "W", A.dtype)
    K = W.shape[1]
    N = W.shape[0]
    if M is None:
        M = A.numel() // A.shape[-1]
        if gather is not None:
            s, hi, wi, ho, wo = gather
            M = (M // (hi * wi)) * ho * wo
    lda = A.shape[-1] if lda is None else lda
    if out is None:
        out = torch.empty((M, N), dtype=A.dtype, device=A.device)
    ldc = N if ldc is None else ldc
    g = gather if gather is not None else (1, 0, 0, 0, 0)
    call("tdeed_gemm_fwd", ptr(A), lda, ptr(A0), (A0.shape[-1] if A0 is not None else 0), k0,
         ptr(a_scale), a_scale_rows, M, K, N, ptr(W), W.shape[1], ptr(scale), ptr(shift),
         ptr(residual), (residual.shape[-1] if residual is not None else 0), act, ptr(out), ldc,
         g[0], g[1], g[2], g[3], g[4], ptr(colpart), *_out2(out2, A), int(bool(out2_pre)), dtype_code(A.dtype), stream_ptr())
    return out


def c1_gconv_fits(Hi, Wi, Cin, C, stride):
    return _lib.load().tdeed_c1_gconv_fits(Hi, Wi, Cin, C, stride) != 0


def c1_gconv_slab_loop_fits(Hi, Wi, Cin, C, stride):
    lib = _lib.load()
    if not hasattr(lib, "tdeed_c1_gconv_slab_loop_fits"):
        return False
    return lib.tdeed_c1_gconv_slab_loop_fits(Hi, Wi, Cin, C, stride) != 0


def c1_gconv_set_form(form):
    call("tdeed_c1_gconv_set_form", form)


def c1_gconv_workgroups(N, Hi, Wi, Cin, C, stride):
    return _lib.load().tdeed_c1_gconv_workgroups(N, Hi, Wi, Cin, C, stride)


def c1_gconv_slab_tiles(Hi, Wi, C, stride):
    return _lib.load().tdeed_c1_gconv_slab_tiles(Hi, Wi, C, stride)


def c1_gconv(x, w1f, s1, h1, wfrag, scale, shift, gw, stride, C, G=None, out=None, pooled=None):
    _chk(x, "x", torch.bfloat16); _chk(G, "G", torch.bfloat16)
    N, Hi, Wi, Cin = x.shape
    Ho, Wo = (Hi - 1) // stride + 1, (Wi - 1) // stride + 1
    if out is None:
        out = torch.empty((N, Ho, Wo, C), dtype=x.dtype, device=x.device)
    if pooled is None:
        pooled = torch.empty((N, gconv3x3_parts(Hi, Wi, C, stride, x.dtype), C), dtype=torch.float32, device=x.device)
    call("tdeed_c1_gconv_fwd", ptr(x), ptr(G), (G.shape[-1] if G is not None else 0), N, Hi, Wi, Cin, C, gw, stride, ptr(w1f),
         ptr(s1), ptr(h1), ptr(wfrag), ptr(scale), ptr(shift), ptr(out), ptr(pooled), stream_ptr())
    return out, pooled


def c1_gconv_c3in_fits(Hi, Wi, Cp, C):
    lib = _lib.load()
    if not hasattr(lib, "tdeed_c1_gconv_c3in_fits"):
        return False
    return lib.tdeed_c1_gconv_c3in_fits(Hi, Wi, Cp, C) != 0


def c1_gconv_c3in_set_walk(walk):
    call("tdeed_c1_gconv_c3in_set_walk", walk)


def c1_gconv_c3in_walk(Hi, Wi, Cp, C):
    return _lib.load().tdeed_c1_gconv_c3in_walk(Hi, Wi, Cp, C)


def c1_gconv_c3in_workgroups(N, Hi, Wi, Cp, C):
    return _lib.load().tdeed_c1_gconv_c3in_workgroups(N, Hi, Wi, Cp, C)


def c1_gconv_c3in(y2p, scp, gate, w3frag, s3, h3, w1f, s1, h1, wfrag, scale, shift, gw, C, xs2=None, out=None, pooled=None):
    _chk(y2p, "y2p", torch.bfloat16); _chk(scp, "scp", torch.bfloat16); _chk(gate, "gate", torch.float32)
    _chk(xs2, "xs2", torch.bfloat16)
    N, Hi, Wi, Cp = y2p.shape
    Ho, Wo = (Hi - 1) // 2 + 1, (Wi - 1) // 2 + 1
    if tuple(scp.shape) != (N, Hi, Wi, Cp) or gate.numel() != N * Cp or (xs2 is not None and xs2.numel() != N * Ho * Wo * Cp):
        raise ValueError(f"c1_gconv_c3in: y2p {tuple(y2p.shape)}, scp {tuple(scp.shape)}, gate {tuple(gate.shape)}, "
                         f"xs2 {None if xs2 is None else tuple(xs2.shape)} do not belong together")
    if out is None:
        out = torch.empty((N, Ho, Wo, C), dtype=y2p.dtype, device=y2p.device)
    if pooled is None:
        pooled = torch.empty((N, gconv3x3_parts(Hi, Wi, C, 2, y2p.dtype), C), dtype=torch.float32, device=y2p.device)
    call("tdeed_c1_gconv_c3in_fwd", ptr(y2p), ptr(scp), ptr(gate), ptr(w3frag), ptr(s3), ptr(h3), ptr(xs2), N, Hi, Wi, Cp, C, gw,
         ptr(w1f), ptr(s1), ptr(h1), ptr(wfrag), ptr(scale), ptr(shift), ptr(out), ptr(pooled), stream_ptr())
    return out, pooled


def bneck_fits(h, w, C, R):
    return _lib.load().tdeed_bneck_fits(h, w, C, R) != 0


def bneck(x, w1f, s1, h1, w2f, s2, h2, se_w1f, se_b1, se_w2f, se_b2, R, w3f, s3, h3, G=None, out=None, out2=None,
          w2_tap_major=True):
    _chk(x, "x", torch.bfloat16); _chk(G, "G", torch.bfloat16); _chk(out2, "out2", torch.bfloat16)
    N, h, w, C = x.shape
    if out is None:
        out = torch.empty_like(x)
    call("tdeed_bneck_fwd", ptr(x), ptr(G), (G.shape[-1] if G is not None else 0), N, h, w, C, ptr(w1f), ptr(s1),
         ptr(h1), ptr(w2f), ptr(s2), ptr(h2), ptr(se_w1f), ptr(se_b1), ptr(se_w2f), ptr(se_b2), R, ptr(w3f), ptr(s3), ptr(h3),
         ptr(out), ptr(out2), (out2.shape[-1] if out2 is not None else 0), int(bool(w2_tap_major)), stream_ptr())
    return out


def bneck_gs(x, gx, gate, ysum, xsum, cw1, cb1, cw2, cb2, T, F, Fp, w1f, s1, h1, w2f, s2, h2, se_w1f, se_b1, se_w2f, se_b2, R,
             w3f, s3, h3, out=None, out2=None, w2_tap_major=True, qtail=None):
    _chk(x, "x", torch.bfloat16); _chk(gx, "gx", torch.bfloat16); _chk(out2, "out2", torch.bfloat16)
    N, h, w, C = x.shape
    if out is None:
        out = torch.empty_like(x)
    call("tdeed_bneck_gs_fwd", ptr(x), ptr(gx), gx.shape[-1], ptr(gate), ptr(ysum), ptr(xsum), ptr(cw1), ptr(cb1), ptr(cw2),
         ptr(cb2), T, F, Fp, N, h, w, C, ptr(w1f), ptr(s1), ptr(h1), ptr(w2f), ptr(s2), ptr(h2), ptr(se_w1f), ptr(se_b1),
         ptr(se_w2f), ptr(se_b2), R, ptr(w3f), ptr(s3), ptr(h3), ptr(out), ptr(out2),
         (out2.shape[-1] if out2 is not None else 0), int(bool(w2_tap_major)),
         *((ptr(qtail[0]), ptr(qtail[1]), int(qtail[2]), ptr(qtail[3])) if qtail is not None else (None, None, 0, None)),
         stream_ptr())
    return out


def bneck_qtail_fits(h, w, C, F):
    return _lib.load().tdeed_bneck_qtail_fits(h, w, C, F) != 0


def gsq_bn_table(bn_scale, bn_shift):
    F = bn_scale.numel()
    t = torch.zeros((2, (F + 7) // 8 * 8), dtype=torch.float32, device=bn_scale.device)
    t[0, :F] = bn_scale
    t[1, :F] = bn_shift
    return t


def gemm_ws_fits_mode(K, N, act_dtype):
    return _lib.load().tdeed_gemm_ws_fits(K, N, dtype_code(act_dtype))


def gemm_ws_fits(K, N, act_dtype):
    return gemm_ws_fits_mode(K, N, act_dtype) != 0


def gemm_ws(A, Wfrag, K, N, scale=None, shift=None, act=ACT_NONE, residual=None, a_scale=None, a_scale_rows=0,
            A0=None, k0=0, gather=None, out=None, M=None, lda=None, ldc=None, out2=None):
    _chk(A, "A")
    if M is None:
        M = A.numel() // A.shape[-1]
        if gather is not None:
            s, hi, wi, ho, wo = gather
            M = (M // (hi * wi)) * ho * wo
    lda = A.shape[-1] if lda is None else lda
    if out is None:
        out = torch.empty((M, N), dtype=A.dtype, device=A.device)
    ldc = N if ldc is None else ldc
    g = gather if gather is not None else (1, 0, 0, 0, 0)
    call("tdeed_gemm_ws_fwd", ptr(A), lda, ptr(A0), (A0.shape[-1] if A0 is not None else 0), k0,
         ptr(a_scale), a_scale_rows, M, K, N, ptr(Wfrag), ptr(scale), ptr(shift),
         ptr(residual), (residual.shape[-1] if residual is not None else 0), act, ptr(out), ldc,
         g[0], g[1], g[2], g[3], g[4], *_out2(out2, A), dtype_code(A.dtype), stream_ptr())
    return out


def gemm_ws_sc_fits(K, Ks, N, act_dtype):
    lib = _lib.load()
    if not hasattr(lib, "tdeed_gemm_ws_sc_fits"):
        return False
    return lib.tdeed_gemm_ws_sc_fits(K, Ks, N, dtype_code(act_dtype)) != 0


def gemm_ws_sc(A, Wfrag, K, N, scale, shift, As, Wsfrag, Ks, sscale, sshift, act=ACT_NONE, a_scale=None, a_scale_rows=0,
               A0=None, k0=0, gather=None, out=None, M=None, out2=None):
    _chk(A, "A", torch.bfloat16); _chk(As, "As", torch.bfloat16)
    if M is None:
        M = A.numel() // A.shape[-1]
    rows_s = As.numel() // As.shape[-1]
    g = gather if gather is not None else (1, 0, 0, 0, 0)
    need = (M // (g[3] * g[4])) * g[1] * g[2] if gather is not None else M
    if rows_s < need or A.numel() // A.shape[-1] < M:
        raise ValueError(f"gemm_ws_sc: operands hold {A.numel() // A.shape[-1]} / {rows_s} rows, {M} / {need} needed")
    if out is None:
        out = torch.empty((M, N), dtype=A.dtype, device=A.device)
    call("tdeed_gemm_ws_sc_fwd", ptr(A), A.shape[-1], ptr(A0), (A0.shape[-1] if A0 is not None else 0), k0,
         ptr(a_scale), a_scale_rows, M, K, N, ptr(Wfrag), ptr(scale), ptr(shift), ptr(As), As.shape[-1], Ks, ptr(Wsfrag),
         ptr(sscale), ptr(sshift), act, ptr(out), N, g[0], g[1], g[2], g[3], g[4], *_out2(out2, A), dtype_code(A.dtype),
         stream_ptr())
    return out


def gemm_rs_fits(M, K, N):
    return _lib.load().tdeed_gemm_rs_fits(M, K, N) != 0


def gemm_rs(A, Wfrag, K, N, scale=None, shift=None, act=ACT_NONE, residual=None, a_scale=None, a_scale_rows=0, A0=None, k0=0,
            out=None, M=None, out2=None):
    _chk(A, "A", torch.bfloat16)
    if M is None:
        M = A.numel() // A.shape[-1]
    if out is None:
        out = torch.empty((M, N), dtype=A.dtype, device=A.device)
    call("tdeed_gemm_rs_fwd", ptr(A), A.shape[-1], ptr(A0), (A0.shape[-1] if A0 is not None else 0), k0, ptr(a_scale),
         a_scale_rows, M, K, N, ptr(Wfrag), ptr(scale), ptr(shift), ptr(residual),
         (residual.shape[-1] if residual is not None else 0), act, ptr(out), N, *_out2(out2, A), stream_ptr())
    return out


def gemm_rs_stats(A, Wfrag, K, N, M=None, A0=None, k0=0):
# ... 1214 lines not shown
```

Baseline: 5934 clips/s.

## Fuse gate-shift temporal blend into the conv1+grouped-conv kernel

Adds blend variants of the fused conv1+grouped 3x3 conv kernels. They read the block input and the neighbouring-frame features directly and apply the GSF gate-shift blend while loading tiles, instead of reading a gate-shift output tensor written beforehand. The gate-shift step then runs in gates-only mode, so the full shifted activation is no longer written to and re-read from global memory. In exchange the kernels do more loads and arithmetic per tile and gain register pressure, and the path is routed only for shapes the new routing check accepts.

Result: no change. 5975 clips/s (median of 3 runs) (+0.7%).

```diff
diff --git a/include/tdeed_hip.h b/include/tdeed_hip.h
--- a/include/tdeed_hip.h
+++ b/include/tdeed_hip.h
@@ -95,6 +95,13 @@
 int tdeed_c1_gconv_set_form(int form);
 int tdeed_c1_gconv_slab_loop_fits(int Hi, int Wi, int Cin, int C, int stride);
 int tdeed_c1_gconv_workgroups(int N, int Hi, int Wi, int Cin, int C, int stride);
+int tdeed_c1_gconv_gs_fits(int Hi, int Wi, int Cin, int C, int stride, int F, int Fp);
+int tdeed_c1_gconv_gs_routed(int Hi, int Wi, int Cin, int C, int stride, int F, int Fp);
+int tdeed_c1_gconv_gs_fwd(const void* x, const void* gx, int ldx, const float* gate, const float* ysum, const float* xsum,
+                          const float* cw1, const float* cb1, const float* cw2, const float* cb2, int T_len, int F, int Fp,
+                          int N, int Hi, int Wi, int Cin, int C, int gw, int stride, const void* w1f, const float* s1,
+                          const float* h1, const void* wfrag, const float* scale, const float* shift, void* y, float* pooled,
+                          void* stream);
 
 int tdeed_c1_gconv_c3in_fits(int Hi, int Wi, int Cp, int C);
 int tdeed_c1_gconv_c3in_fwd(const void* y2p, const void* scp, const float* gate, const void* w3f, const float* s3,
diff --git a/t-deed_amd/_lib.py b/t-deed_amd/_lib.py
--- a/t-deed_amd/_lib.py
+++ b/t-deed_amd/_lib.py
@@ -65,6 +65,10 @@
     "tdeed_c1_gconv_set_form": ([c_int], c_int),
     "tdeed_c1_gconv_slab_loop_fits": ([c_int, c_int, c_int, c_int, c_int], c_int),
     "tdeed_c1_gconv_workgroups": ([c_int, c_int, c_int, c_int, c_int, c_int], c_int),
+    "tdeed_c1_gconv_gs_fits": ([c_int, c_int, c_int, c_int, c_int, c_int, c_int], c_int),
+    "tdeed_c1_gconv_gs_routed": ([c_int, c_int, c_int, c_int, c_int, c_int, c_int], c_int),
+    "tdeed_c1_gconv_gs_fwd": ([P, P, c_int, P, P, P, P, P, P, P, c_int, c_int, c_int, c_int, c_int, c_int, c_int, c_int, c_int,
+                               c_int, P, P, P, P, P, P, P, P, P], c_int),
     "tdeed_c1_gconv_c3in_fits": ([c_int, c_int, c_int, c_int], c_int),
     "tdeed_c1_gconv_c3in_fwd": ([P, P, P, P, P, P, P, c_int, c_int, c_int, c_int, c_int, c_int, P, P, P, P, P, P, P, P,
                                  P], c_int),
diff --git a/t-deed_amd/build.py b/t-deed_amd/build.py
--- a/t-deed_amd/build.py
+++ b/t-deed_amd/build.py
@@ -33,7 +33,7 @@
 def build(force=False, verbose=True, flavour="release", only=None):
     debug = flavour == "debug"
     flags, lib, osuf = (DEBUG_FLAGS, LIB_DEBUG, ".dbg.o") if debug else (FLAGS, LIB, ".o")
-    hdrs = [os.path.join(CSRC, "common.h"), os.path.join(CSRC, "sgp_tile.h"), os.path.join(CSRC, "se_excite.h"), os.path.join(CSRC, "jpeg_core.h"),
+    hdrs = [os.path.join(CSRC, "common.h"), os.path.join(CSRC, "sgp_tile.h"), os.path.join(CSRC, "se_excite.h"), os.path.join(CSRC, "jpeg_core.h"), os.path.join(CSRC, "c1g_kernels.h"),
             os.path.join(os.path.dirname(os.path.dirname(CSRC)), "include", "tdeed_hip.h")]
     jobs = []
     objs = []
diff --git a/t-deed_amd/csrc/c1g_kernels.h b/t-deed_amd/csrc/c1g_kernels.h
--- /dev/null
+++ b/t-deed_amd/csrc/c1g_kernels.h
@@ -0,0 +1,350 @@
+template <int STRIDE, int KS1>
+__global__ __launch_bounds__(256, KS1 == 4 ? 3 : 1) void C1G_MFMA_KERNEL(const bf16_t* __restrict__ x, const bf16_t* __restrict__ G, int Fp,
+                                                            int Hi, int Wi, int Cin, int C, const bf16x8* __restrict__ w1f,
+                                                            const float* __restrict__ s1, const float* __restrict__ h1,
+                                                            const bf16x8* __restrict__ wfrag, const float* __restrict__ scale,
+                                                            const float* __restrict__ shift, bf16_t* __restrict__ y,
+                                                            float* __restrict__ pooled, int Ho, int Wo, int band, int nbands,
+                                                            int CSP, int PS, int rows_in, int relu, long long* dbg C1G_GS_PARAM) {
+  constexpr bool BLEND = C1G_BLEND;
+  C1G_GS_LOCAL
+  extern __shared__ __attribute__((aligned(16))) unsigned char tile[];
+  __shared__ float red[4][32];
+  __shared__ float redq[4][32];
+  GC_STAMP(0);
+  const long lid = xcd_logical_id(blockIdx.x, gridDim.x);
+  const int nslabs_ = (C + CSP - 1) >> (CSP == 64 ? 6 : (CSP == 32 ? 5 : 4));
+  int slab, bnd, n, t_;
+  td_split(lid, nslabs_, t_, slab);
+  td_split(t_, nbands, n, bnd);
+  const int oy0 = bnd * band;
+  const int nrows_out = min(band, Ho - oy0);
+  const int WP = Wi + 2;
+  const int iy0 = oy0 * STRIDE - 1;
+  const int nrow_used = (nrows_out - 1) * STRIDE + 3;
+  const int tid = threadIdx.x, lane = tid & 63, wv = __builtin_amdgcn_readfirstlane(tid >> 6);
+  const int pl = lane & 15, q = lane >> 4;
+  const int nts = CSP >> 4;
+  static_assert(!BLEND || (STRIDE == 2 && (KS1 == 2 || KS1 == 5)), "the blend exists where the slab loop does");
+  constexpr int KB = KS1 == 2 ? 1 : 2;
+  __shared__ __attribute__((aligned(16))) float bfw[BLEND ? 2 : 1][64];
+  [[maybe_unused]] int bt = 0;
+  [[maybe_unused]] float bsv[10], bcw = 0.f;
+  if constexpr (BLEND) {
+    int bb;
+    td_split(n, gs.T_len, bb, bt);
+    c1g_blend_sums(gs, n, bt, bsv, bcw);
+  }
+  constexpr bool GW_EARLY = KS1 <= 2;
+  GcW gw_;
+  if constexpr (GW_EARLY) gw_ = gconv_load_w(wfrag, slab, CSP);
+  bf16x8 w1r[4][KS1];
+  float a1[4][4], b1[4][4];
+#pragma unroll
+  for (int t = 0; t < 4; ++t) {
+    const int tt = slab * nts + min(t, nts - 1);
+#pragma unroll
+    for (int ks = 0; ks < KS1; ++ks) w1r[t][ks] = w1f[((long)tt * KS1 + ks) * 64 + lane];
+    const int c4 = slab * CSP + t * 16 + 4 * q;
+    const bool ok = t < nts && c4 < C;
+    const int cc4 = min(c4, C - 4);
+    const f32x4 av = *reinterpret_cast<const f32x4*>(s1 + cc4), bv = *reinterpret_cast<const f32x4*>(h1 + cc4);
+#pragma unroll
+    for (int e = 0; e < 4; ++e) {
+      a1[t][e] = ok ? av[e] : 0.f;
+      b1[t][e] = ok ? bv[e] : 0.f;
+    }
+  }
+  c1g_zero_halo(tile, nrow_used, Hi, Wi, PS, iy0);
+  [[maybe_unused]] C1gBl bl;
+  if constexpr (BLEND) {
+    const float wgt = c1g_blend_weight(gs, bt, bsv, bcw);
+    if (wv == 0) {
+      bfw[0][lane] = wgt;
+      bfw[1][lane] = 1.0f - wgt;
+    }
+    bl = c1g_blend_frame(gs, n, bt, Hi * Wi, Fp);
+    __syncthreads();
+  }
+  GC_STAMP(1);
+  {
+    const int r_lo = max(iy0, 0), r_hi = min(iy0 + nrow_used, Hi);
+    const int npx = (r_hi - r_lo) * Wi;
+    const int ntl = (npx + 15) >> 4;
+    const IDiv dwi(Wi);
+    const bf16_t* xn = x + (long)n * Hi * Wi * Cin;
+    const bf16_t* gn = G ? G + (long)n * Hi * Wi * Fp : nullptr;
+    constexpr int NPF = KS1 <= 2 ? 4 : 1;
+    if constexpr (KS1 == 4) {
+      auto tile_px = [&](int t0, int& rr, int& cc) {
+        const int p = min(t0, ntl - 1) * 16 + pl;
+        const bool ok = t0 < ntl && p < npx;
+        dwi.divmod(p < npx ? p : 0, rr, cc);
+        return ok;
+      };
+      auto tile_load = [&](int rr, int cc, bf16x8 (&xfo)[KS1]) {
+        const long pix = (long)(r_lo + rr) * Wi + cc;
+#pragma unroll
+        for (int ks = 0; ks < KS1; ++ks) {
+          const int k = 32 * ks + 8 * q;
+          const bf16_t* src = (gn && k < Fp) ? gn + pix * Fp + k : xn + pix * Cin + k;
+          xfo[ks] = *reinterpret_cast<const bf16x8*>(src);
+        }
+      };
+      auto tile_mma = [&](bool pok_, int rr, int cc, const bf16x8 (&xfi)[KS1]) {
+        unsigned char* dst = tile + ((long)(r_lo + rr - iy0) * WP + cc + 1) * PS + 8 * q;
+        c1g_conv1_tile(w1r, xfi, a1, b1, nts, pok_, dst);
+      };
+      bf16x8 xa[KS1], xb[KS1];
+      int ra, ca, rb, cb;
+      bool pa = tile_px(wv, ra, ca), pb;
+      tile_load(ra, ca, xa);
+      for (int tb = wv; tb < ntl; tb += 8) {
+        pb = tile_px(tb + 4, rb, cb);
+        tile_load(rb, cb, xb);
+        tile_mma(pa, ra, ca, xa);
+        pa = tile_px(tb + 8, ra, ca);
+        tile_load(ra, ca, xa);
+        tile_mma(pb, rb, cb, xb);
+      }
+    } else
+    for (int tb = wv; tb < ntl; tb += 4 * NPF) {
+      bf16x8 xf[NPF][KS1];
+      int rrs[NPF], ccs[NPF];
+      bool poks[NPF];
+      if constexpr (BLEND) {
+        u32x4 xv[NPF][KS1];
+        C1gNb<KB> nbv[NPF];
+#pragma unroll
+        for (int g = 0; g < NPF; ++g) {
+          poks[g] = c1g_tile_px(ntl, npx, dwi, tb + 4 * g, pl, rrs[g], ccs[g]);
+          const long pix = (long)(r_lo + rrs[g]) * Wi + ccs[g];
+#pragma unroll
+          for (int ks = 0; ks < KS1; ++ks) {
+            const int k = 32 * ks + 8 * q;
+            const bool ok = poks[g] && k < Cin;
+            const unsigned off = ok ? ((unsigned)pix * (unsigned)Cin + (unsigned)k) * 2u : 0u;
+            xv[g][ks] = *reinterpret_cast<const u32x4*>(reinterpret_cast<const char*>(xn) + off);
+          }
+          c1g_blend_request<KB>(bl, (unsigned)pix, q, nbv[g]);
+        }
+#pragma unroll
+        for (int g = 0; g < NPF; ++g)
+#pragma unroll
+          for (int ks = 0; ks < KS1; ++ks) {
+            const int k = 32 * ks + 8 * q;
+            u32x4 v = xv[g][ks];
+            if (ks < KB) v = c1g_blend_chunk(bl, bfw, k, v, nbv[g].nb[min(ks, KB - 1)], nbv[g].gv);
+            const u32x4 z = {0u, 0u, 0u, 0u};
+            const u32x4 w = (poks[g] && k < Cin) ? v : z;
+            xf[g][ks] = *reinterpret_cast<const bf16x8*>(&w);
+          }
+      } else {
+#pragma unroll
+      for (int g = 0; g < NPF; ++g) {
+        poks[g] = c1g_tile_px(ntl, npx, dwi, tb + 4 * g, pl, rrs[g], ccs[g]);
+        const long pix = (long)(r_lo + rrs[g]) * Wi + ccs[g];
+#pragma unroll
+        for (int ks = 0; ks < KS1; ++ks) {
+          const int k = 32 * ks + 8 * q;
+          const bool ok = poks[g] && k < Cin;
+          const bf16_t* src = (gn && k < Fp) ? gn + pix * Fp + k : xn + pix * Cin + k;
+          const u32x4 v = *reinterpret_cast<const u32x4*>(ok ? src : xn);
+          const u32x4 z = {0u, 0u, 0u, 0u};
+          const u32x4 w = ok ? v : z;
+          xf[g][ks] = *reinterpret_cast<const bf16x8*>(&w);
+        }
+      }
+      }
+#pragma unroll
+      for (int g = 0; g < NPF; ++g) {
+        if (tb + 4 * g >= ntl) break;
+        unsigned char* dst = tile + ((long)(r_lo + rrs[g] - iy0) * WP + ccs[g] + 1) * PS + 8 * q;
+        c1g_conv1_tile(w1r, xf[g], a1, b1, nts, poks[g], dst);
+      }
+    }
+  }
+  GC_STAMP(2);
+  if constexpr (!GW_EARLY) gw_ = gconv_load_w(wfrag, slab, CSP);
+  __syncthreads();
+  GC_STAMP(3);
+  gconv_band_mma<STRIDE>(gw_, tile, red, redq, Wi, C, scale, shift, y, pooled, nullptr, Ho, Wo, nbands, CSP, PS, relu, n, bnd,
+                         slab, oy0, nrows_out, GcStat{nullptr, nullptr, nullptr, nullptr}, dbg);
+}
+
+
+template <int STRIDE, int KS1>
+__global__ __launch_bounds__(256, KS1 == 2 ? 3 : 2) void C1G_SLAB_KERNEL(const bf16_t* __restrict__ x, const bf16_t* __restrict__ G, int Fp,
+                                                            int Hi, int Wi, int Cin, int C, const bf16x8* __restrict__ w1f,
+                                                            const float* __restrict__ s1, const float* __restrict__ h1,
+                                                            const bf16x8* __restrict__ wfrag, const float* __restrict__ scale,
+                                                            const float* __restrict__ shift, bf16_t* __restrict__ y,
+                                                            float* __restrict__ pooled, int Ho, int Wo, int band, int nbands,
+                                                            int CSP, int PS, int rows_in, int relu, long long* dbg C1G_GS_PARAM) {
+  constexpr bool BLEND = C1G_BLEND;
+  C1G_GS_LOCAL
+  extern __shared__ __attribute__((aligned(16))) unsigned char tile[];
+  __shared__ float red[4][32];
+  __shared__ float redq[4][32];
+  GC_STAMP(0);
+  const long lid = xcd_logical_id(blockIdx.x, gridDim.x);
+  const int nslabs_ = (C + CSP - 1) >> 6;
+  int bnd, n;
+  td_split(lid, nbands, n, bnd);
+  const int oy0 = bnd * band;
+  const int nrows_out = min(band, Ho - oy0);
+  const int WP = Wi + 2;
+  const int iy0 = oy0 * STRIDE - 1;
+  const int nrow_used = (nrows_out - 1) * STRIDE + 3;
+  const int tid = threadIdx.x, lane = tid & 63, wv = __builtin_amdgcn_readfirstlane(tid >> 6);
+  const int pl = lane & 15, q = lane >> 4;
+  static_assert(STRIDE == 2 && (KS1 == 2 || KS1 == 5), "the slab loop exists for the stride-2 multi-slab blocks");
+  constexpr int NT = C1G_SLAB_TILES(KS1);
+  constexpr int SCSP = 64;
+  const int r_lo = max(iy0, 0), r_hi = min(iy0 + nrow_used, Hi);
+  const int npx = (r_hi - r_lo) * Wi;
+  const int ntl = (npx + 15) >> 4;
+  const IDiv dwi(Wi);
+  const bf16_t* xn = x + (long)n * Hi * Wi * Cin;
+  const bf16_t* gn = G ? G + (long)n * Hi * Wi * Fp : nullptr;
+  __shared__ __attribute__((aligned(16))) float fold[2][C1G_SLAB_MAXC];
+  float fa[C1G_SLAB_MAXC / 256], fb[C1G_SLAB_MAXC / 256];
+#pragma unroll
+  for (int j = 0; j < C1G_SLAB_MAXC / 256; ++j) {
+    const int c = min(tid + 256 * j, C - 1);
+    fa[j] = s1[c];
+    fb[j] = h1[c];
+  }
+  constexpr int KB = KS1 == 2 ? 1 : 2;
+  __shared__ __attribute__((aligned(16))) float bfw[BLEND ? 2 : 1][64];
+  [[maybe_unused]] int bt = 0;
+  [[maybe_unused]] float bsv[10], bcw = 0.f;
+  [[maybe_unused]] C1gBl bl;
+  [[maybe_unused]] C1gNb<KB> nbv[BLEND ? NT : 1];
+  if constexpr (BLEND) {
+    int bb;
+    td_split(n, gs.T_len, bb, bt);
+    c1g_blend_sums(gs, n, bt, bsv, bcw);
+    bl = c1g_blend_frame(gs, n, bt, Hi * Wi, Fp);
+  }
+  u32x4 xv[NT][KS1];
+  int dsto[NT];
+  [[maybe_unused]] unsigned dpk[(NT + 1) / 2];
+  bool poks[NT];
+#pragma unroll
+  for (int g = 0; g < NT; ++g) {
+    int rr, cc;
+    poks[g] = c1g_tile_px(ntl, npx, dwi, wv + 4 * g, pl, rr, cc);
+    const long pix = (long)(r_lo + rr) * Wi + cc;
+    dsto[g] = ((r_lo + rr - iy0) * WP + cc + 1) * PS + 8 * q;
+    if constexpr (BLEND) dpk[g >> 1] = (g & 1) ? (dpk[g >> 1] | ((unsigned)dsto[g] << 16)) : (unsigned)dsto[g];
+#pragma unroll
+    for (int ks = 0; ks < KS1; ++ks) {
+      const int k = 32 * ks + 8 * q;
+      const bool ok = poks[g] && k < Cin;
+      if constexpr (BLEND) {
+        const unsigned off = ok ? ((unsigned)pix * (unsigned)Cin + (unsigned)k) * 2u : 0u;
+        xv[g][ks] = *reinterpret_cast<const u32x4*>(reinterpret_cast<const char*>(xn) + off);
+      } else {
+      const bf16_t* src = (gn && k < Fp) ? gn + pix * Fp + k : xn + pix * Cin + k;
+      xv[g][ks] = *reinterpret_cast<const u32x4*>(ok ? src : xn);
+      }
+    }
+    if constexpr (BLEND) {
+      c1g_blend_request<KB>(bl, (unsigned)pix, q, nbv[g]);
+      __builtin_amdgcn_sched_barrier(0);
+    }
+  }
+  bf16x8 w1r[4][KS1];
+  auto load_w1 = [&](int sl, int tlo) {
+#pragma unroll
+    for (int t = tlo; t < tlo + 2; ++t)
+#pragma unroll
+      for (int ks = 0; ks < KS1; ++ks) w1r[t][ks] = w1f[((long)(sl * 4 + t) * KS1 + ks) * 64 + lane];
+  };
+  constexpr bool W1_LATE = BLEND && KS1 == 5;
+  load_w1(0, 0);
+  if constexpr (!W1_LATE) load_w1(0, 2);
+  GcW gw_;
+  if constexpr (!BLEND) gw_ = gconv_load_w(wfrag, 0, SCSP);
+  c1g_zero_halo(tile, nrow_used, Hi, Wi, PS, iy0);
+#pragma unroll
+  for (int j = 0; j < C1G_SLAB_MAXC / 256; ++j) {
+    const int c = tid + 256 * j;
+    fold[0][c] = c < C ? fa[j] : 0.f;
+    fold[1][c] = c < C ? fb[j] : 0.f;
+  }
+  if constexpr (BLEND) {
+    if (wv == 0) {
+      const float wgt = c1g_blend_weight(gs, bt, bsv, bcw);
+      bfw[0][lane] = wgt;
+      bfw[1][lane] = 1.0f - wgt;
+    }
+  }
+  __syncthreads();
+  GC_STAMP(1);
+  if constexpr (BLEND) {
+#pragma unroll
+    for (int g = 0; g < NT; ++g)
+#pragma unroll
+      for (int ks = 0; ks < KB; ++ks) {
+        xv[g][ks] = c1g_blend_chunk(bl, bfw, 32 * ks + 8 * q, xv[g][ks], nbv[g].nb[ks], nbv[g].gv);
+        asm volatile("" : "+v"(xv[g][ks]));
+        __builtin_amdgcn_sched_barrier(0);
+      }
+    if constexpr (W1_LATE) load_w1(0, 2);
+    gw_ = gconv_load_w(wfrag, 0, SCSP);
+    GC_STAMP(7);
+  }
+  bf16x8 xf[NT][KS1];
+#pragma unroll
+  for (int g = 0; g < NT; ++g)
+#pragma unroll
+    for (int ks = 0; ks < KS1; ++ks) {
+      const u32x4 z = {0u, 0u, 0u, 0u};
+      const u32x4 w = (poks[g] && 32 * ks + 8 * q < Cin) ? xv[g][ks] : z;
+      xf[g][ks] = *reinterpret_cast<const bf16x8*>(&w);
+    }
+  auto conv1_pair = [&](int sl, int tlo) {
+#pragma unroll
+    for (int t = tlo; t < tlo + 2; ++t) {
+      const f32x4 av = *reinterpret_cast<const f32x4*>(&fold[0][sl * 64 + t * 16 + 4 * q]);
+      const f32x4 bv = *reinterpret_cast<const f32x4*>(&fold[1][sl * 64 + t * 16 + 4 * q]);
+#pragma unroll
+      for (int g = 0; g < NT; ++g) {
+        if (wv + 4 * g >= ntl) break;
+        f32x4 acc = {0.f, 0.f, 0.f, 0.f};
+#pragma unroll
+        for (int ks = 0; ks < KS1; ++ks) acc = __builtin_amdgcn_mfma_f32_16x16x32_bf16(w1r[t][ks], xf[g][ks], acc, 0, 0, 0);
+        if (poks[g]) {
+          bf16x4 o;
+#pragma unroll
+          for (int e = 0; e < 4; ++e) o[e] = (bf16_t)fmaxf(acc[e] * av[e] + bv[e], 0.f);
+          if constexpr (BLEND) {
+            unsigned d = dpk[g >> 1];
+            asm volatile("" : "+v"(d));
+            *reinterpret_cast<bf16x4*>(tile + ((g & 1) ? d >> 16 : d & 0xffffu) + t * 32) = o;
+          } else
+          *reinterpret_cast<bf16x4*>(tile + dsto[g] + t * 32) = o;
+        }
+      }
+    }
+  };
+  for (int s = 0; s < nslabs_; ++s) {
+    const int sn = min(s + 1, nslabs_ - 1);
+    conv1_pair(s, 0);
+    load_w1(sn, 0);
+    conv1_pair(s, 2);
+    if (s == 0) GC_STAMP(2);
+    __syncthreads();
+    if (s == 0) GC_STAMP(3);
+    gconv_band_mma<STRIDE>(gw_, tile, red, redq, Wi, C, scale, shift, y, pooled, nullptr, Ho, Wo, nbands, SCSP, PS, relu, n,
+                           bnd, s, oy0, nrows_out);
+    if (s == 0) GC_STAMP(4);
+    load_w1(sn, 2);
+    gw_ = gconv_load_w(wfrag, sn, SCSP);
+    __syncthreads();
+  }
+  GC_STAMP(5);
+  GC_STAMP(6);
+}
diff --git a/t-deed_amd/csrc/conv.hip b/t-deed_amd/csrc/conv.hip
--- a/t-deed_amd/csrc/conv.hip
+++ b/t-deed_amd/csrc/conv.hip
@@ -589,255 +589,149 @@
     }
   }
 }
-template <int STRIDE, int KS1>
-__global__ __launch_bounds__(256, KS1 == 4 ? 3 : 1) void c1_gconv_mfma_kernel(const bf16_t* __restrict__ x, const bf16_t* __restrict__ G, int Fp,
-                                                            int Hi, int Wi, int Cin, int C, const bf16x8* __restrict__ w1f,
-                                                            const float* __restrict__ s1, const float* __restrict__ h1,
-                                                            const bf16x8* __restrict__ wfrag, const float* __restrict__ scale,
-                                                            const float* __restrict__ shift, bf16_t* __restrict__ y,
-                                                            float* __restrict__ pooled, int Ho, int Wo, int band, int nbands,
-                                                            int CSP, int PS, int rows_in, int relu, long long* dbg) {
-  extern __shared__ __attribute__((aligned(16))) unsigned char tile[];
-  __shared__ float red[4][32];
-  __shared__ float redq[4][32];
-  GC_STAMP(0);
-  const long lid = xcd_logical_id(blockIdx.x, gridDim.x);
-  const int nslabs_ = (C + CSP - 1) >> (CSP == 64 ? 6 : (CSP == 32 ? 5 : 4));
-  int slab, bnd, n, t_;
-  td_split(lid, nslabs_, t_, slab);
-  td_split(t_, nbands, n, bnd);
-  const int oy0 = bnd * band;
-  const int nrows_out = min(band, Ho - oy0);
-  const int WP = Wi + 2;
-  const int iy0 = oy0 * STRIDE - 1;
-  const int nrow_used = (nrows_out - 1) * STRIDE + 3;
-  const int tid = threadIdx.x, lane = tid & 63, wv = __builtin_amdgcn_readfirstlane(tid >> 6);
-  const int pl = lane & 15, q = lane >> 4;
-  const int nts = CSP >> 4;
-  constexpr bool GW_EARLY = KS1 <= 2;
-  GcW gw_;
-  if constexpr (GW_EARLY) gw_ = gconv_load_w(wfrag, slab, CSP);
-  bf16x8 w1r[4][KS1];
-  float a1[4][4], b1[4][4];
-#pragma unroll
-  for (int t = 0; t < 4; ++t) {
-    const int tt = slab * nts + min(t, nts - 1);
-#pragma unroll
-    for (int ks = 0; ks < KS1; ++ks) w1r[t][ks] = w1f[((long)tt * KS1 + ks) * 64 + lane];
-    const int c4 = slab * CSP + t * 16 + 4 * q;
-    const bool ok = t < nts && c4 < C;
-    const int cc4 = min(c4, C - 4);
-    const f32x4 av = *reinterpret_cast<const f32x4*>(s1 + cc4), bv = *reinterpret_cast<const f32x4*>(h1 + cc4);
-#pragma unroll
-    for (int e = 0; e < 4; ++e) {
-      a1[t][e] = ok ? av[e] : 0.f;
-      b1[t][e] = ok ? bv[e] : 0.f;
-    }
-  }
-  c1g_zero_halo(tile, nrow_used, Hi, Wi, PS, iy0);
-  GC_STAMP(1);
-  {
-    const int r_lo = max(iy0, 0), r_hi = min(iy0 + nrow_used, Hi);
-    const int npx = (r_hi - r_lo) * Wi;
-    const int ntl = (npx + 15) >> 4;
-    const IDiv dwi(Wi);
-    const bf16_t* xn = x + (long)n * Hi * Wi * Cin;
-    const bf16_t* gn = G ? G + (long)n * Hi * Wi * Fp : nullptr;
-    constexpr int NPF = KS1 <= 2 ? 4 : 1;
-    if constexpr (KS1 == 4) {
-      auto tile_px = [&](int t0, int& rr, int& cc) {
-        const int p = min(t0, ntl - 1) * 16 + pl;
-        const bool ok = t0 < ntl && p < npx;
-        dwi.divmod(p < npx ? p : 0, rr, cc);
-        return ok;
-      };
-      auto tile_load = [&](int rr, int cc, bf16x8 (&xfo)[KS1]) {
-        const long pix = (long)(r_lo + rr) * Wi + cc;
-#pragma unroll
-        for (int ks = 0; ks < KS1; ++ks) {
-          const int k = 32 * ks + 8 * q;
-          const bf16_t* src = (gn && k < Fp) ? gn + pix * Fp + k : xn + pix * Cin + k;
-          xfo[ks] = *reinterpret_cast<const bf16x8*>(src);
-        }
-      };
-      auto tile_mma = [&](bool pok_, int rr, int cc, const bf16x8 (&xfi)[KS1]) {
-        unsigned char* dst = tile + ((long)(r_lo + rr - iy0) * WP + cc + 1) * PS + 8 * q;
-        c1g_conv1_tile(w1r, xfi, a1, b1, nts, pok_, dst);
-      };
-      bf16x8 xa[KS1], xb[KS1];
-      int ra, ca, rb, cb;
-      bool pa = tile_px(wv, ra, ca), pb;
-      tile_load(ra, ca, xa);
-      for (int tb = wv; tb < ntl; tb += 8) {
-        pb = tile_px(tb + 4, rb, cb);
-        tile_load(rb, cb, xb);
-        tile_mma(pa, ra, ca, xa);
-        pa = tile_px(tb + 8, ra, ca);
-        tile_load(ra, ca, xa);
-        tile_mma(pb, rb, cb, xb);
-      }
-    } else
-    for (int tb = wv; tb < ntl; tb += 4 * NPF) {
-      bf16x8 xf[NPF][KS1];
-      int rrs[NPF], ccs[NPF];
-      bool poks[NPF];
-#pragma unroll
-      for (int g = 0; g < NPF; ++g) {
-        poks[g] = c1g_tile_px(ntl, npx, dwi, tb + 4 * g, pl, rrs[g], ccs[g]);
-        const long pix = (long)(r_lo + rrs[g]) * Wi + ccs[g];
-#pragma unroll
-        for (int ks = 0; ks < KS1; ++ks) {
-          const int k = 32 * ks + 8 * q;
-          const bool ok = poks[g] && k < Cin;
-          const bf16_t* src = (gn && k < Fp) ? gn + pix * Fp + k : xn + pix * Cin + k;
-          const u32x4 v = *reinterpret_cast<const u32x4*>(ok ? src : xn);
-          const u32x4 z = {0u, 0u, 0u, 0u};
-          const u32x4 w = ok ? v : z;
-          xf[g][ks] = *reinterpret_cast<const bf16x8*>(&w);
-        }
-      }
-#pragma unroll
-      for (int g = 0; g < NPF; ++g) {
-        if (tb + 4 * g >= ntl) break;
-        unsigned char* dst = tile + ((long)(r_lo + rrs[g] - iy0) * WP + ccs[g] + 1) * PS + 8 * q;
-        c1g_conv1_tile(w1r, xf[g], a1, b1, nts, poks[g], dst);
-      }
-    }
-  }
-  GC_STAMP(2);
-  if constexpr (!GW_EARLY) gw_ = gconv_load_w(wfrag, slab, CSP);
-  __syncthreads();
-  GC_STAMP(3);
-  gconv_band_mma<STRIDE>(gw_, tile, red, redq, Wi, C, scale, shift, y, pooled, nullptr, Ho, Wo, nbands, CSP, PS, relu, n, bnd,
-                         slab, oy0, nrows_out, GcStat{nullptr, nullptr, nullptr, nullptr}, dbg);
-}
-
+struct C1gGs {
+  const bf16_t* x; int ldx;
+  const float* gate; const float* ysum; const float* xsum;
+  const float* cw1; const float* cb1; const float* cw2; const float* cb2;
+  int T_len, F; float inv_hw;
+};
+struct C1gBl {
+  const bf16_t* xb; const float* gb;
+  unsigned oce, one, ocp, onp;
+  unsigned ldx; int F, Fh, Fp; bool has_prev, has_next;
+};
+template <int KB> struct C1gNb { unsigned nb[KB][4]; float gv; };
+__device__ __forceinline__ C1gBl c1g_blend_frame(const C1gGs& gs, int n, int t, int hw, int Fp) {
+  C1gBl bl;
+  bl.has_prev = t > 0;
+  bl.has_next = t < gs.T_len - 1;
+  const long fp = bl.has_prev ? n - 1 : n;
+  bl.xb = gs.x + fp * hw * gs.ldx;
+  bl.gb = gs.gate + fp * hw * 2;
+  bl.ldx = (unsigned)gs.ldx;
+  bl.ocp = bl.has_prev ? (unsigned)hw : 0u;
+  bl.onp = bl.ocp + (bl.has_next ? (unsigned)hw : 0u);
+  bl.oce = bl.ocp * bl.ldx;
+  bl.one = bl.onp * bl.ldx;
+  bl.F = gs.F;
+  bl.Fh = gs.F >> 1;
+  bl.Fp = Fp;
+  return bl;
+}
+__device__ __forceinline__ void c1g_blend_sums(const C1gGs& gs, int n, int t, float (&sv)[10], float& cwv) {
+  const int ci = min((int)(threadIdx.x & 63), 37);
+  cwv = *(ci < 18 ? gs.cw1 + ci : ci < 36 ? gs.cw2 + (ci - 18) : ci == 36 ? gs.cb1 : gs.cb2);
+  const unsigned c4 = (unsigned)min((int)(threadIdx.x & 63), gs.F - 1) * 4u;
+#pragma unroll
+  for (int row = 0; row < 10; ++row) {
+    const int r = row >= 5 ? row - 5 : row;
+    const int t2 = min(max(t + r - 2, 0), gs.T_len - 1);
+    const float* rowp = (row >= 5 ? gs.xsum : gs.ysum) + (long)(n - t + t2) * gs.F;
+    sv[row] = *reinterpret_cast<const float*>(reinterpret_cast<const char*>(rowp) + c4);
+  }
+}
+__device__ __forceinline__ float c1g_blend_weight(const C1gGs& gs, int t, const float (&sv)[10], float cwv) {
+  const int c = threadIdx.x & 63, F = gs.F, Fh = F >> 1;
+  float s[10];
+#pragma unroll
+  for (int row = 0; row < 10; ++row) {
+    const int t2 = t + (row >= 5 ? row - 5 : row) - 2;
+    s[row] = (t2 >= 0 && t2 < gs.T_len) ? sv[row] : 0.f;
+  }
+  const int g = c >= Fh;
+  const int cl = c - g * Fh;
+  auto cw = [&](int i) { return __builtin_bit_cast(float, __builtin_amdgcn_readlane(__builtin_bit_cast(int, cwv), i)); };
+  float a = g ? cw(37) : cw(36);
+#pragma unroll
+  for (int dc = -1; dc <= 1; ++dc) {
+    const int c2 = cl + dc;
+    const bool okc = c2 >= 0 && c2 < Fh;
+    float sc[10];
+#pragma unroll
+    for (int row = 0; row < 10; ++row) sc[row] = dc < 0 ? __shfl_up(s[row], 1) : dc > 0 ? __shfl_down(s[row], 1) : s[row];
+#pragma unroll
+    for (int dt = -1; dt <= 1; ++dt) {
+      const int t2 = t + dt;
+      const bool ok = okc && t2 >= 0 && t2 < gs.T_len;
+      const float rm = (sc[5 + dt + 2] - sc[dt + 2]) * gs.inv_hw;
+      const float sp = sc[dt + 1], sn = sc[dt + 3];
+      const float ysh = (g ? sp : sn) * gs.inv_hw;
+      const int wi = (dc + 1) * 3 + (dt + 1);
+      const float wy1 = cw(wi), wy2 = cw(18 + wi), wr1 = cw(9 + wi), wr2 = cw(27 + wi);
+      float a2 = fmaf(g ? wy2 : wy1, ysh, a);
+      a2 = fmaf(g ? wr2 : wr1, rm, a2);
+      a = ok ? a2 : a;
+    }
+  }
+  return c < F ? sigmoidf_(a) : 0.f;
+}
+template <int KB>
+__device__ __forceinline__ void c1g_blend_request(const C1gBl& bl, unsigned pu, int q, C1gNb<KB>& o) {
+  const char* gb = reinterpret_cast<const char*>(bl.gb);
+  const char* xb = reinterpret_cast<const char*>(bl.xb);
+  o.gv = *reinterpret_cast<const float*>(gb + (((q < 2 ? bl.ocp : q == 2 ? bl.onp : 0u) + pu) * 8u + (q & 1) * 4u));
+#pragma unroll
+  for (int ks = 0; ks < KB; ++ks) {
+    const unsigned kb = (unsigned)min(32 * ks + 8 * q, bl.Fp - 8);
+    const unsigned off = (pu * bl.ldx + kb) * 2u;
+#pragma unroll
+    for (int pr = 0; pr < 4; ++pr)
+      o.nb[ks][pr] = *reinterpret_cast<const unsigned*>(xb + (((int)kb + 2 * pr >= bl.Fh ? 0u : bl.one * 2u) + off + 4u * pr));
+  }
+}
+__device__ __forceinline__ u32x4 c1g_blend_chunk(const C1gBl& bl, const float (*bfw)[64], int k0, u32x4 xc,
+                                                 const unsigned (&nb)[4], float gv) {
+  const int kb = min(k0, bl.Fp - 8), pl = threadIdx.x & 15;
+  const f32x2 ga = {__shfl(gv, pl), __shfl(gv, pl + 16)};
+  const float gn = __shfl(gv, pl + 32), gp = __shfl(gv, pl + 48);
+  const f32x4 w0 = *reinterpret_cast<const f32x4*>(&bfw[0][kb]), w1 = *reinterpret_cast<const f32x4*>(&bfw[0][kb + 4]);
+  const f32x4 m0 = *reinterpret_cast<const f32x4*>(&bfw[1][kb]), m1 = *reinterpret_cast<const f32x4*>(&bfw[1][kb + 4]);
+  const float gn_ = bl.has_next ? gn : 0.f, gp_ = bl.has_prev ? gp : 0.f;
+  u32x4 o;
+#pragma unroll
+  for (int pr = 0; pr < 4; ++pr) {
+    const int ci = kb + 2 * pr;
+    const bool g = ci >= bl.Fh;
+    const unsigned xcw = xc[pr], nbw = nb[pr];
+    const f32x2 xv = {__builtin_bit_cast(float, xcw << 16), __builtin_bit_cast(float, xcw & 0xffff0000u)};
+    const f32x2 nv = {__builtin_bit_cast(float, nbw << 16), __builtin_bit_cast(float, nbw & 0xffff0000u)};
+    const float gate = g ? ga[1] : ga[0], gsh = g ? gp_ : gn_;
+    const f32x2 gate2 = {gate, gate}, gsh2 = {gsh, gsh};
+    const f32x2 wv = pr < 2 ? (f32x2){w0[2 * pr], w0[2 * pr + 1]} : (f32x2){w1[2 * pr - 4], w1[2 * pr - 3]};
+    const f32x2 om = pr < 2 ? (f32x2){m0[2 * pr], m0[2 * pr + 1]} : (f32x2){m1[2 * pr - 4], m1[2 * pr - 3]};
+    const f32x2 r = __builtin_elementwise_fma(-gate2, xv, xv);
+    const f32x2 ysh = gsh2 * nv;
+    const f32x2 tm = r * om;
+    const f32x2 ov = __builtin_elementwise_fma(ysh, wv, tm);
+    const bf16x2 ob = {(bf16_t)ov[0], (bf16_t)ov[1]};
+    o[pr] = (k0 < bl.Fp && ci < bl.F) ? __builtin_bit_cast(unsigned, ob) : xcw;
+  }
+  return o;
+}
 #define C1G_SLAB_TILES(KS1v) ((KS1v) <= 2 ? 5 : 4)
 #define C1G_SLAB_MAXC 512
-template <int STRIDE, int KS1>
-__global__ __launch_bounds__(256, KS1 == 2 ? 3 : 2) void c1_gconv_slab_loop_kernel(const bf16_t* __restrict__ x, const bf16_t* __restrict__ G, int Fp,
-                                                            int Hi, int Wi, int Cin, int C, const bf16x8* __restrict__ w1f,
-                                                            const float* __restrict__ s1, const float* __restrict__ h1,
-                                                            const bf16x8* __restrict__ wfrag, const float* __restrict__ scale,
-                                                            const float* __restrict__ shift, bf16_t* __restrict__ y,
-                                                            float* __restrict__ pooled, int Ho, int Wo, int band, int nbands,
-                                                            int CSP, int PS, int rows_in, int relu, long long* dbg) {
-  extern __shared__ __attribute__((aligned(16))) unsigned char tile[];
-  __shared__ float red[4][32];
-  __shared__ float redq[4][32];
-  GC_STAMP(0);
-  const long lid = xcd_logical_id(blockIdx.x, gridDim.x);
-  const int nslabs_ = (C + CSP - 1) >> 6;
-  int bnd, n;
-  td_split(lid, nbands, n, bnd);
-  const int oy0 = bnd * band;
-  const int nrows_out = min(band, Ho - oy0);
-  const int WP = Wi + 2;
-  const int iy0 = oy0 * STRIDE - 1;
-  const int nrow_used = (nrows_out - 1) * STRIDE + 3;
-  const int tid = threadIdx.x, lane = tid & 63, wv = __builtin_amdgcn_readfirstlane(tid >> 6);
-  const int pl = lane & 15, q = lane >> 4;
-  static_assert(STRIDE == 2 && (KS1 == 2 || KS1 == 5), "the slab loop exists for the stride-2 multi-slab blocks");
-  constexpr int NT = C1G_SLAB_TILES(KS1);
-  constexpr int SCSP = 64;
-  const int r_lo = max(iy0, 0), r_hi = min(iy0 + nrow_used, Hi);
-  const int npx = (r_hi - r_lo) * Wi;
-  const int ntl = (npx + 15) >> 4;
-  const IDiv dwi(Wi);
-  const bf16_t* xn = x + (long)n * Hi * Wi * Cin;
-  const bf16_t* gn = G ? G + (long)n * Hi * Wi * Fp : nullptr;
-  __shared__ __attribute__((aligned(16))) float fold[2][C1G_SLAB_MAXC];
-  float fa[C1G_SLAB_MAXC / 256], fb[C1G_SLAB_MAXC / 256];
-#pragma unroll
-  for (int j = 0; j < C1G_SLAB_MAXC / 256; ++j) {
-    const int c = min(tid + 256 * j, C - 1);
-    fa[j] = s1[c];
-    fb[j] = h1[c];
-  }
-  u32x4 xv[NT][KS1];
-  int dsto[NT];
-  bool poks[NT];
-#pragma unroll
-  for (int g = 0; g < NT; ++g) {
-    int rr, cc;
-    poks[g] = c1g_tile_px(ntl, npx, dwi, wv + 4 * g, pl, rr, cc);
-    const long pix = (long)(r_lo + rr) * Wi + cc;
-    dsto[g] = ((r_lo + rr - iy0) * WP + cc + 1) * PS + 8 * q;
-#pragma unroll
-    for (int ks = 0; ks < KS1; ++ks) {
-      const int k = 32 * ks + 8 * q;
-      const bool ok = poks[g] && k < Cin;
-      const bf16_t* src = (gn && k < Fp) ? gn + pix * Fp + k : xn + pix * Cin + k;
-      xv[g][ks] = *reinterpret_cast<const u32x4*>(ok ? src : xn);
-    }
-  }
-  bf16x8 w1r[4][KS1];
-  auto load_w1 = [&](int sl, int tlo) {
-#pragma unroll
-    for (int t = tlo; t < tlo + 2; ++t)
-#pragma unroll
-      for (int ks = 0; ks < KS1; ++ks) w1r[t][ks] = w1f[((long)(sl * 4 + t) * KS1 + ks) * 64 + lane];
-  };
-  load_w1(0, 0);
-  load_w1(0, 2);
-  GcW gw_ = gconv_load_w(wfrag, 0, SCSP);
-  c1g_zero_halo(tile, nrow_used, Hi, Wi, PS, iy0);
-#pragma unroll
-  for (int j = 0; j < C1G_SLAB_MAXC / 256; ++j) {
-    const int c = tid + 256 * j;
-    fold[0][c] = c < C ? fa[j] : 0.f;
-    fold[1][c] = c < C ? fb[j] : 0.f;
-  }
-  __syncthreads();
-  GC_STAMP(1);
-  bf16x8 xf[NT][KS1];
-#pragma unroll
-  for (int g = 0; g < NT; ++g)
-#pragma unroll
-    for (int ks = 0; ks < KS1; ++ks) {
-      const u32x4 z = {0u, 0u, 0u, 0u};
-      const u32x4 w = (poks[g] && 32 * ks + 8 * q < Cin) ? xv[g][ks] : z;
-      xf[g][ks] = *reinterpret_cast<const bf16x8*>(&w);
-    }
-  auto conv1_pair = [&](int sl, int tlo) {
-#pragma unroll
-    for (int t = tlo; t < tlo + 2; ++t) {
-      const f32x4 av = *reinterpret_cast<const f32x4*>(&fold[0][sl * 64 + t * 16 + 4 * q]);
-      const f32x4 bv = *reinterpret_cast<const f32x4*>(&fold[1][sl * 64 + t * 16 + 4 * q]);
-#pragma unroll
-      for (int g = 0; g < NT; ++g) {
-        if (wv + 4 * g >= ntl) break;
-        f32x4 acc = {0.f, 0.f, 0.f, 0.f};
-#pragma unroll
-        for (int ks = 0; ks < KS1; ++ks) acc = __builtin_amdgcn_mfma_f32_16x16x32_bf16(w1r[t][ks], xf[g][ks], acc, 0, 0, 0);
-        if (poks[g]) {
-          bf16x4 o;
-#pragma unroll
-          for (int e = 0; e < 4; ++e) o[e] = (bf16_t)fmaxf(acc[e] * av[e] + bv[e], 0.f);
-          *reinterpret_cast<bf16x4*>(tile + dsto[g] + t * 32) = o;
-        }
-      }
-    }
-  };
-  for (int s = 0; s < nslabs_; ++s) {
-    const int sn = min(s + 1, nslabs_ - 1);
-    conv1_pair(s, 0);
-    load_w1(sn, 0);
-    conv1_pair(s, 2);
-    if (s == 0) GC_STAMP(2);
-    __syncthreads();
-    if (s == 0) GC_STAMP(3);
-    gconv_band_mma<STRIDE>(gw_, tile, red, redq, Wi, C, scale, shift, y, pooled, nullptr, Ho, Wo, nbands, SCSP, PS, relu, n,
-                           bnd, s, oy0, nrows_out);
-    if (s == 0) GC_STAMP(4);
-    load_w1(sn, 2);
-    gw_ = gconv_load_w(wfrag, sn, SCSP);
-    __syncthreads();
-  }
-  GC_STAMP(5);
-  GC_STAMP(6);
-}
-
+#define C1G_MFMA_KERNEL c1_gconv_mfma_kernel
+#define C1G_SLAB_KERNEL c1_gconv_slab_loop_kernel
+#define C1G_BLEND false
+#define C1G_GS_PARAM
+#define C1G_GS_LOCAL [[maybe_unused]] const C1gGs gs{};
+#include "c1g_kernels.h"
+#undef C1G_MFMA_KERNEL
+#undef C1G_SLAB_KERNEL
+#undef C1G_BLEND
+#undef C1G_GS_PARAM
+#undef C1G_GS_LOCAL
+#define C1G_MFMA_KERNEL c1g_blend_mfma_kernel
+#define C1G_SLAB_KERNEL c1g_blend_slab_loop_kernel
+#define C1G_BLEND true
+#define C1G_GS_PARAM , const C1gGs gs
+#define C1G_GS_LOCAL
+#include "c1g_kernels.h"
+#undef C1G_MFMA_KERNEL
+#undef C1G_SLAB_KERNEL
+#undef C1G_BLEND
+#undef C1G_GS_PARAM
+#undef C1G_GS_LOCAL
 struct C3In {
   const bf16_t* y2p; const bf16_t* scp; const float* gate;
   const bf16x8* w3f; const float* s3; const float* h3;
@@ -1140,9 +1034,39 @@
   const GcGeom g = gc_geom(Hi, Wi, C, stride);
   return N * g.nbands * (c1g_slab_loop(Hi, Wi, Cin, C, stride) ? 1 : g.nslabs);
 }
+static int c1_gconv_launch(const void* x, const void* G, int Fp, const C1gGs* gs, int N, int Hi, int Wi, int Cin, int C, int gw,
+                           int stride, const void* w1f, const float* s1, const float* h1, const void* wfrag,
+                           const float* scale, const float* shift, void* y, float* pooled, void* stream);
 extern "C" int tdeed_c1_gconv_fwd(const void* x, const void* G, int Fp, int N, int Hi, int Wi, int Cin, int C, int gw,
                                   int stride, const void* w1f, const float* s1, const float* h1, const void* wfrag,
                                   const float* scale, const float* shift, void* y, float* pooled, void* stream) {
+  return c1_gconv_launch(x, G, Fp, nullptr, N, Hi, Wi, Cin, C, gw, stride, w1f, s1, h1, wfrag, scale, shift, y, pooled, stream);
+}
+extern "C" int tdeed_c1_gconv_gs_fits(int Hi, int Wi, int Cin, int C, int stride, int F, int Fp) {
+  if (!tdeed_c1_gconv_slab_loop_fits(Hi, Wi, Cin, C, stride)) return 0;
+  const int ks1 = (Cin + 31) / 32;
+  if (F < 4 || F % 4 != 0 || F > 64 || Fp != (F + 7) / 8 * 8 || Fp > Cin || Fp > (ks1 == 2 ? 32 : 64)) return 0;
+  return (long)Hi * Wi * Cin * 3 < (1L << 30) ? 1 : 0;
+}
+extern "C" int tdeed_c1_gconv_gs_routed(int Hi, int Wi, int Cin, int C, int stride, int F, int Fp) {
+  return tdeed_c1_gconv_gs_fits(Hi, Wi, Cin, C, stride, F, Fp) && (Cin + 31) / 32 == 5 ? 1 : 0;
+}
+extern "C" int tdeed_c1_gconv_gs_fwd(const void* x, const void* gx, int ldx, const float* gate, const float* ysum,
+                                     const float* xsum, const float* cw1, const float* cb1, const float* cw2, const float* cb2,
+                                     int T_len, int F, int Fp, int N, int Hi, int Wi, int Cin, int C, int gw, int stride,
+                                     const void* w1f, const float* s1, const float* h1, const void* wfrag, const float* scale,
+                                     const float* shift, void* y, float* pooled, void* stream) {
+  TD_CHECK(gx && gate && ysum && xsum && cw1 && cb1 && cw2 && cb2, "c1_gconv_gs: null pointer (the site's operands)");
+  TD_CHECK(tdeed_c1_gconv_gs_fits(Hi, Wi, Cin, C, stride, F, Fp), "c1_gconv_gs: Hi=%d Wi=%d Cin=%d C=%d stride=%d F=%d Fp=%d unsupported",
+           Hi, Wi, Cin, C, stride, F, Fp);
+  TD_CHECK(ldx >= Fp && ldx <= Cin && ldx % 8 == 0, "c1_gconv_gs: bad slice row stride %d", ldx);
+  TD_CHECK(T_len > 0 && N > 0 && N % T_len == 0, "c1_gconv_gs: %d frames are not clips of %d", N, T_len);
+  const C1gGs gs{(const bf16_t*)gx, ldx, gate, ysum, xsum, cw1, cb1, cw2, cb2, T_len, F, 1.0f / (float)(Hi * Wi)};
+  return c1_gconv_launch(x, nullptr, Fp, &gs, N, Hi, Wi, Cin, C, gw, stride, w1f, s1, h1, wfrag, scale, shift, y, pooled, stream);
+}
+static int c1_gconv_launch(const void* x, const void* G, int Fp, const C1gGs* gsp, int N, int Hi, int Wi, int Cin, int C, int gw,
+                           int stride, const void* w1f, const float* s1, const float* h1, const void* wfrag,
+                           const float* scale, const float* shift, void* y, float* pooled, void* stream) {
   TD_CHECK(x && w1f && s1 && h1 && wfrag && scale && shift && y && pooled, "c1_gconv: null pointer");
   TD_CHECK((gw == 8 || gw == 16) && C % gw == 0, "c1_gconv: group width %d / C %d unsupported", gw, C);
   TD_CHECK(stride == 1 || stride == 2, "c1_gconv: stride %d", stride);
@@ -1156,6 +1080,18 @@
   const size_t smem = (size_t)g.rows_in * (Wi + 2) * g.PS;
   hipStream_t st = (hipStream_t)stream;
   const int KS1 = (Cin + 31) / 32;
+  const C1gGs gs0 = gsp ? *gsp : C1gGs{};
+  if (gsp) {
+#define TD_C1G_BL(KERNEL, Kv)                                                                                                \
+  hipLaunchKernelGGL((KERNEL<2, Kv>), grid, dim3(256), smem, st, (const bf16_t*)x, (const bf16_t*)nullptr, Fp, Hi, Wi,  \
+                     Cin, C, (const bf16x8*)w1f, s1, h1, (const bf16x8*)wfrag, scale, shift, (bf16_t*)y, pooled, Ho, Wo,      \
+                     g.band, g.nbands, g.CSP, g.PS, g.rows_in, 1, g_c1g_dbg, gs0)
+    if (slabs) { if (KS1 == 2) TD_C1G_BL(c1g_blend_slab_loop_kernel, 2); else TD_C1G_BL(c1g_blend_slab_loop_kernel, 5); }
+    else { if (KS1 == 2) TD_C1G_BL(c1g_blend_mfma_kernel, 2); else TD_C1G_BL(c1g_blend_mfma_kernel, 5); }
+#undef TD_C1G_BL
+    TD_LAUNCH_CHECK("c1_gconv_gs");
+    return TDEED_OK;
+  }
 #define TD_C1G(Sv, Kv)                                                                                                       \
   hipLaunchKernelGGL((c1_gconv_mfma_kernel<Sv, Kv>), grid, dim3(256), smem, st, (const bf16_t*)x, (const bf16_t*)G,           \
                      G ? Fp : 0, Hi, Wi, Cin, C, (const bf16x8*)w1f, s1, h1, (const bf16x8*)wfrag, scale, shift, (bf16_t*)y,  \
diff --git a/t-deed_amd/engine.py b/t-deed_amd/engine.py
--- a/t-deed_amd/engine.py
+++ b/t-deed_amd/engine.py
@@ -161,10 +161,12 @@
 C1_GCONV_MAX_CIN = 160
 SC_IN_CONV3 = True
 S1_CONV3_IN_C1G = True
+C1G_BLEND = True
 
 
 BlockForm = namedtuple("BlockForm",
-                       "h w h2 w2 one_launch c1g site Fp slice_in q_given blend_in qtail slice_next sc_in_conv3 conv3_in")
+                       "h w h2 w2 one_launch c1g site Fp slice_in q_given blend_in qtail slice_next sc_in_conv3 conv3_in "
+                       "blend_c1g")
 
 
 def block_forms(blocks, h, w, act_dtype, taps, last_out_is_slice, pending=None):
@@ -192,8 +194,11 @@
                         and blk.has_downsample and act_dtype == torch.bfloat16 and pending.w3.ws
                         and pending.spec.cout == blk.cin and ("_features." + pending.spec.name) not in taps
                         and ops.c1_gconv_c3in_fits(h, w, blk.cin, blk.cout))
+        blend_c1g = bool(C1G_BLEND and c1g and not one_launch and site and act_dtype == torch.bfloat16 and bw.gs_src
+                         and bw.gs_cw1 is not None and ("_features." + blk.name + ".gs_out") not in taps
+                         and ops.c1_gconv_gs_routed(h, w, blk.cin, blk.cout, blk.stride, blk.gsf_fold, Fp))
         forms.append(BlockForm(h, w, h2, w2, one_launch, c1g, site, Fp, slice_in, q_given, blend_in, qtail, slice_next, sc_in_conv3,
-                               conv3_in))
+                               conv3_in, blend_c1g))
         h, w = h2, w2
     return forms
 
@@ -498,14 +503,15 @@
                   q=(q if f.q_given else pool.take((N, f.h, f.w, 6), torch.float32)),
                   ysum=pool.take((N, F), torch.float32),
                   xsum=pool.take((N, F), torch.float32))
-        if not f.blend_in:
+        gates_only = f.blend_in or f.blend_c1g
+        if not gates_only:
             gb["out"] = pool.take((M, Fp), self.act_dtype)
             if bw.gs_cw1 is not None:
                 gb["fw"] = pool.take((B, F, T), torch.float32)
         self.steps.append(Step(blk.name + ".gate_shift", "gate_shift", lambda: ops.gate_shift(
             xg, B, T, F, Fp, bw.gs_scale, bw.gs_shift, bw.gs_wq, bw.gs_b3d, bw.gs_cw1, bw.gs_cb1,
-            bw.gs_cw2, bw.gs_cb2, bufs=gb, wqf=bw.gs_wqf, src_order=bw.gs_src, gates_only=f.blend_in, q_given=f.q_given),
-            M * ((1 if f.blend_in else 2) * F + (0 if f.blend_in else Fp)) * _esz(self.act_dtype) + M * 16, 2 * M * F * 27))
+            bw.gs_cw2, bw.gs_cb2, bufs=gb, wqf=bw.gs_wqf, src_order=bw.gs_src, gates_only=gates_only, q_given=f.q_given),
+            M * ((1 if gates_only else 2) * F + (0 if gates_only else Fp)) * _esz(self.act_dtype) + M * 16, 2 * M * F * 27))
         tap = "_features." + blk.name + ".gs_out"
         if tap in self.taps:
             if bw.gs_src:
@@ -542,7 +548,7 @@
                                2 * M * blk.cout * (2 * blk.cout + blk.gw * 9)))
         return out, xs_next, q_next
 
-    def _chain(self, bw, f, x, y1, G, out, dead_site):
+    def _chain(self, bw, f, x, y1, G, out, dead_site, xg=None, gb=None):
         pool, steps, blk, dt = self.pool, self.steps, bw.spec, self.act_dtype
         N, es, s = self.N, _esz(dt), blk.stride
         h, w, h2, w2 = f.h, f.w, f.h2, f.w2
@@ -570,6 +576,13 @@
             for t_ in front[1:]:
                 pool.give(t_)
             x = xs2
+        elif f.blend_c1g:
+            T = self.pw.clip_len
+            steps.append(Step(blk.name + ".conv1_conv2", "c1_gconv", lambda: ops.c1_gconv_gs(
+                x, xg, gb["gate"], gb["ysum"], gb["xsum"], bw.gs_cw1, bw.gs_cb1, bw.gs_cw2, bw.gs_cb2, T, blk.gsf_fold, f.Fp,
+                bw.c1g_w1f, bw.s1, bw.h1, bw.w2frag, bw.s2, bw.h2, blk.gw, s, blk.cout, out=y2, pooled=pooled),
+                (M * blk.cin + M * f.Fp + M2 * blk.cout) * es + 8 * M + blk.cout * (blk.cin + blk.gw * 9) * es,
+                2 * M * blk.cin * blk.cout + 2 * M2 * blk.cout * blk.gw * 9))
         elif f.c1g:
             steps.append(Step(blk.name + ".conv1_conv2", "c1_gconv", lambda: ops.c1_gconv(
                 x, bw.c1g_w1f, bw.s1, bw.h1, bw.w2frag, bw.s2, bw.h2, blk.gw, s, blk.cout, G=G, out=y2, pooled=pooled),
@@ -616,7 +629,7 @@
             if f.one_launch:
                 out, xs, q = self._one_launch(bw, f, x, xg, gb, None if last else blocks[bi + 1])
             else:
-                out, xs, dead = self._chain(bw, f, x, y1, gb.get("out"), out_last if last else None, dead)
+                out, xs, dead = self._chain(bw, f, x, y1, gb.get("out"), out_last if last else None, dead, xg=xg, gb=gb)
                 q = None
             x_kept = self._block_done(bw.spec, dead, x, x_kept, out)
             x, h, w = out, f.h2, f.w2
diff --git a/t-deed_amd/ops.py b/t-deed_amd/ops.py
--- a/t-deed_amd/ops.py
+++ b/t-deed_amd/ops.py
@@ -164,7 +164,7 @@
     return _lib.load().tdeed_c1_gconv_slab_tiles(Hi, Wi, C, stride)
 
 
-def c1_gconv(x, w1f, s1, h1, wfrag, scale, shift, gw, stride, C, G=None, out=None, pooled=None):
+def c1_gconv(x, w1f, s1, h1, wfrag, scale, shift, gw, stride, C, G=None, gs=None, out=None, pooled=None):
     _chk(x, "x", torch.bfloat16); _chk(G, "G", torch.bfloat16)
     N, Hi, Wi, Cin = x.shape
     Ho, Wo = (Hi - 1) // stride + 1, (Wi - 1) // stride + 1
@@ -172,9 +172,42 @@
         out = torch.empty((N, Ho, Wo, C), dtype=x.dtype, device=x.device)
     if pooled is None:
         pooled = torch.empty((N, gconv3x3_parts(Hi, Wi, C, stride, x.dtype), C), dtype=torch.float32, device=x.device)
+    if gs is not None:
+        if G is not None:
+            raise ValueError("c1_gconv: G and gs exclude each other")
+        gx, gate, ysum, xsum, cw1, cb1, cw2, cb2, T, F, Fp = gs
+        _chk(gx, "gx", torch.bfloat16); _chk(gate, "gate", torch.float32)
+        if (tuple(gx.shape[:3]) != (N, Hi, Wi) or gate.numel() != N * Hi * Wi * 2 or ysum.numel() != N * F
+                or xsum.numel() != N * F):
+            raise ValueError(f"c1_gconv_gs: x {tuple(x.shape)}, gx {tuple(gx.shape)}, gate {tuple(gate.shape)}, "
+                             f"ysum {tuple(ysum.shape)} do not belong together")
+        call("tdeed_c1_gconv_gs_fwd", ptr(x), ptr(gx), gx.shape[-1], ptr(gate), ptr(ysum), ptr(xsum), ptr(cw1), ptr(cb1),
+             ptr(cw2), ptr(cb2), T, F, Fp, N, Hi, Wi, Cin, C, gw, stride, ptr(w1f), ptr(s1), ptr(h1), ptr(wfrag), ptr(scale),
+             ptr(shift), ptr(out), ptr(pooled), stream_ptr())
+        return out, pooled
     call("tdeed_c1_gconv_fwd", ptr(x), ptr(G), (G.shape[-1] if G is not None else 0), N, Hi, Wi, Cin, C, gw, stride, ptr(w1f),
          ptr(s1), ptr(h1), ptr(wfrag), ptr(scale), ptr(shift), ptr(out), ptr(pooled), stream_ptr())
     return out, pooled
+
+
+def c1_gconv_gs_fits(Hi, Wi, Cin, C, stride, F, Fp):
+    lib = _lib.load()
+    if not hasattr(lib, "tdeed_c1_gconv_gs_fits"):
+        return False
+    return lib.tdeed_c1_gconv_gs_fits(Hi, Wi, Cin, C, stride, F, Fp) != 0
+
+
+def c1_gconv_gs_routed(Hi, Wi, Cin, C, stride, F, Fp):
+    lib = _lib.load()
+    if not hasattr(lib, "tdeed_c1_gconv_gs_routed"):
+        return False
+    return lib.tdeed_c1_gconv_gs_routed(Hi, Wi, Cin, C, stride, F, Fp) != 0
+
+
+def c1_gconv_gs(x, gx, gate, ysum, xsum, cw1, cb1, cw2, cb2, T, F, Fp, w1f, s1, h1, wfrag, scale, shift, gw, stride, C,
+                out=None, pooled=None):
+    return c1_gconv(x, w1f, s1, h1, wfrag, scale, shift, gw, stride, C, gs=(gx, gate, ysum, xsum, cw1, cb1, cw2, cb2, T, F, Fp),
+                    out=out, pooled=pooled)
 
 
 def c1_gconv_c3in_fits(Hi, Wi, Cp, C):
```
